# zenithfang/supervised_dispnet

Measured on AMD Instinct MI355X. Metric: images/sec fwd+bwd Disp_vgg_BN 128x416 b32 @1/2/4/8 GPU, higher is better.
Workload: dtype f32 (Winograd forward / input gradient / weight gradient form each f32 product from three exact bf16 pieces per operand on the bf16 matrix cores, six partial products, f32 accumulate; error vs fp64 at or below the f32 matrix instruction's)

## Files before the change

include/dispnet_hip.h:

```cpp
#ifndef DISPNET_HIP_H_
#define DISPNET_HIP_H_

#include <stddef.h>
#include <stdint.h>

#ifdef __cplusplus
extern "C" {
#endif

typedef void* dn_stream_t;

enum dn_status {
  DN_OK = 0,
  DN_ERR_BAD_ARG = -1,
  DN_ERR_UNSUPPORTED = -2,
  DN_ERR_WORKSPACE = -3,
  DN_ERR_LAUNCH = -4
};

void dn_reload_knobs(void);
int dn_version(void);
const char* dn_last_error(void);
const char* dn_last_kernel(void);
int dn_device_arch_ok(void);
// ... 49 lines not shown
  int32_t pad_mode;
  int32_t compute;
  int32_t dilation;
  const float* bnb_y;
  const float* bnb_scale;
  const float* bnb_shift;
  const float* bnb_mean;
  const float* bnb_invstd;
  float* bnb_partial;
  void* splitk_ws;
  int64_t splitk_ws_bytes;
  float* recip_out;
  const float* bnf_gamma;
  const float* bnf_beta;
  float* bnf_running_mean;
  float* bnf_running_var;
  int64_t* bnf_num_batches_tracked;
  float bnf_momentum, bnf_eps;
  float* bnf_mean;
  float* bnf_invstd;
  float* bnf_scale;
  float* bnf_shift;
  float* bnb_dgamma;
  float* bnb_dbeta;
} dn_conv_desc;

enum { DN_COMPUTE_DEFAULT = 0, DN_COMPUTE_BF16 = 1, DN_COMPUTE_F32X3 = 2, DN_COMPUTE_F32 = 3 };

int64_t dn_conv_packed_weight_elems(const dn_conv_desc* d);
int dn_conv_pack_weights(const dn_conv_desc* d, const float* w, float* w_packed, dn_stream_t stream);
int64_t dn_pack_entry_bytes(void);
int dn_pack_entry_fill(const dn_conv_desc* d, const float* w, float* w_packed, void* entry_host);
int dn_pack_many(const void* entries_dev, int32_t n_direct, int32_t n_wino, int32_t n_wino_bf16, int32_t n_wino_x3, dn_stream_t stream);
int32_t dn_conv_weight_layout(const dn_conv_desc* d);
int32_t dn_conv_bn_partial_rows(const dn_conv_desc* d);
int64_t dn_conv_splitk_workspace_bytes(const dn_conv_desc* d);
int32_t dn_conv_fwd_folds_bn_finalize(const dn_conv_desc* d);
int32_t dn_conv_dgrad_folds_bn_sums(const dn_conv_desc* d);
int32_t dn_conv_dgrad_fuses_bn_sums(const dn_conv_desc* d);
int32_t dn_conv_fwd_fuses_reciprocal(const dn_conv_desc* d);
int dn_conv2d_fwd(const dn_conv_desc* d, dn_stream_t stream);
int dn_conv2d_dgrad(const dn_conv_desc* d, dn_stream_t stream);
int dn_convT2d_fwd(const dn_conv_desc* d, dn_stream_t stream);
int dn_convT2d_dgrad(const dn_conv_desc* d, dn_stream_t stream);

size_t dn_conv_wgrad_workspace_bytes(const dn_conv_desc* fwd);
int dn_conv2d_wgrad(const dn_conv_desc* fwd, const float* dy, float* dw, void* workspace, size_t workspace_bytes,
                    dn_stream_t stream);

int dn_bn_finalize(const float* partial, int32_t rows, int32_t C, int64_t count, const float* conv_bias,
                   const float* gamma, const float* beta, float* running_mean, float* running_var, float momentum,
                   float eps, float* mean, float* invstd, float* scale, float* shift, int64_t* num_batches_tracked,
                   dn_stream_t stream);
int dn_bn_eval_affine(int32_t C, const float* gamma, const float* beta, const float* running_mean,
                      const float* running_var, float eps, float* scale, float* shift, dn_stream_t stream);
int dn_bn_relu_pool_fwd(const float* y, const float* scale, const float* shift, int32_t N, int32_t H, int32_t W,
                        int32_t C, float* pooled, uint8_t* idx, dn_stream_t stream);
int dn_bn_relu_pool_bwd(const float* dpooled, const uint8_t* idx, const float* y, const float* mean,
                        const float* invstd, int32_t N, int32_t H, int32_t W, int32_t C, float* dz, float* partial,
                        dn_stream_t stream);
int dn_maxpool2_bwd(const float* dpooled, const uint8_t* idx, int32_t N, int32_t H, int32_t W, int32_t C, float* dx, int32_t accumulate,
                    dn_stream_t stream);
int dn_bn_relu_bwd_reduce(float* da_dz, const float* y, const float* scale, const float* shift, const float* mean,
                          const float* invstd, int64_t rows, int32_t C, float* partial, dn_stream_t stream);
int dn_bn_bwd_apply(float* dz_dy, const float* y, const float* mean, const float* invstd, const float* gamma,
                    const float* partial, int32_t partial_rows, int32_t partial_stride, int32_t partial_offset, int64_t rows,
                    int32_t C, float* dgamma, float* dbeta, dn_stream_t stream);
int dn_bn_relu_bwd_sums(const float* da, const float* y, const float* scale, const float* shift, const float* mean, const float* invstd,
                        int64_t rows, int32_t C, float* partial, dn_stream_t stream);
int dn_bn_relu_pool_bwd_sums(const float* dpooled, const uint8_t* idx, const float* y, const float* mean, const float* invstd, int32_t N,
                             int32_t H, int32_t W, int32_t C, float* partial, dn_stream_t stream);
int dn_bn_bwd_apply_relu(float* da_dy, const float* y, const float* scale, const float* shift, const float* mean, const float* invstd,
                         const float* gamma, const float* partial, int32_t partial_rows, int32_t partial_stride, int32_t partial_offset,
                         int64_t rows, int32_t C, float* dgamma, float* dbeta, dn_stream_t stream);
int dn_bn_bwd_apply_pool(const float* dpooled, const uint8_t* idx, const float* y, const float* mean, const float* invstd, const float* gamma,
                         const float* partial, int32_t partial_rows, int32_t partial_stride, int32_t partial_offset, int32_t N, int32_t H,
                         int32_t W, int32_t C, float* dy, float* dgamma, float* dbeta, dn_stream_t stream);
int32_t dn_reduce_blocks(int64_t rows, int32_t C);

int dn_bn_frozen_affine(int32_t C, const float* gamma, const float* beta, const float* running_mean, const float* running_var, float eps,
                        float* scale, float* shift, float* invstd, dn_stream_t stream);
int dn_bn_frozen_bwd(float* dz_dy, const float* y, const float* mean, const float* invstd, const float* gamma, int64_t rows, int32_t C,
                     float* partial, dn_stream_t stream);
int dn_bn_frozen_bwd_relu(float* da_dy, const float* y, const float* scale, const float* shift, const float* mean, const float* invstd,
                          const float* gamma, int64_t rows, int32_t C, float* partial, dn_stream_t stream);
int dn_bn_frozen_bwd_pool(const float* dpooled, const uint8_t* idx, const float* y, const float* mean, const float* invstd, const float* gamma,
                          int32_t N, int32_t H, int32_t W, int32_t C, float* dy, float* partial, dn_stream_t stream);
int dn_bn_frozen_add_relu_bwd(const float* gout, const float* out, const float* y, const float* mean, const float* invstd, const float* gamma,
                              const float* r, const float* r_mean, const float* r_invstd, const float* r_gamma, int64_t rows, int32_t C,
                              float* dy, float* dr, int32_t dr_accumulate, float* partial, dn_stream_t stream);
int dn_bn_frozen_finalize(const float* partial, int32_t partial_rows, int32_t partial_stride, int32_t partial_offset, int32_t C,
                          const float* gamma, const float* invstd, float* dgamma, float* dbeta, float* dbias, dn_stream_t stream);

int dn_act_bwd_reduce_from(const float* g_in, float* g_out, const float* y_post, int32_t act, float p0, float p1, int64_t rows, int32_t C,
                           float* partial, dn_stream_t stream);
int dn_act_bwd_reduce(float* g, const float* y_post, int32_t act, float p0, float p1, int64_t rows, int32_t C,
                      float* partial, dn_stream_t stream);
int dn_colsum_finalize(const float* partial, int32_t rows, int32_t C, int32_t stride, int32_t offset, float* out,
                       dn_stream_t stream);
int dn_upsample2x_nearest_bwd(const float* dfull, int32_t N, int32_t h, int32_t w, float* dlow, int32_t accumulate,
                              dn_stream_t stream);
int dn_upsample2x_nearest_bwd_nhwc(const float* dfull, int32_t N, int32_t h, int32_t w, int32_t C, float* dlow, int32_t accumulate,
                                   dn_stream_t stream);
int dn_reflect_fold(const float* dxp, int32_t N, int32_t H, int32_t W, int32_t C, int32_t pad, float* dx, int32_t accumulate,
                    dn_stream_t stream);
int dn_bn_add_relu_fwd(const float* y, const float* scale, const float* shift, const float* r, const float* r_scale, const float* r_shift,
                       int64_t rows, int32_t C, float* out, dn_stream_t stream);
int dn_bn_add_relu_bwd(const float* gout, const float* out, const float* y, const float* mean, const float* invstd, const float* r,
                       const float* r_mean, const float* r_invstd, int64_t rows, int32_t C, float* dz_y, float* dr, int32_t dr_accumulate,
                       float* partial, dn_stream_t stream);
int32_t dn_maxpool3s2_out(int32_t H, int32_t ceil_mode);
int dn_maxpool3s2_fwd(const float* x, int32_t N, int32_t H, int32_t W, int32_t C, int32_t ceil_mode, float* out, uint8_t* idx, dn_stream_t stream);
int dn_maxpool3s2_bwd(const float* dout, const uint8_t* idx, int32_t N, int32_t H, int32_t W, int32_t C, int32_t ceil_mode, float* dx,
                      int32_t accumulate, dn_stream_t stream);
int dn_sub_div(const float* x, int64_t n, float sub, float div, float* out, dn_stream_t stream);
int dn_upsample2x_bilinear_fwd(const float* low, int32_t N, int32_t h, int32_t w, int32_t OH, int32_t OW, float* out,
                               dn_stream_t stream);
int dn_upsample2x_bilinear_bwd(const float* dout, int32_t N, int32_t h, int32_t w, int32_t OH, int32_t OW, float* dlow,
                               int32_t accumulate, dn_stream_t stream);
int32_t dn_bn_stats_rows(int64_t rows);
int dn_bn_stats_partial(const float* x, int64_t rows, int32_t C, float* partial, dn_stream_t stream);
int dn_bn_apply_fwd(const float* y, const float* scale, const float* shift, int64_t rows, int32_t C, float* out, dn_stream_t stream);
int dn_phase_bias_add(float* x, int32_t N, int32_t H2, int32_t W2, int32_t C, const float* bias4, dn_stream_t stream);
size_t dn_phase_colsum_workspace_bytes(int32_t C);
int dn_phase_colsum(const float* g, int32_t N, int32_t H, int32_t W, int32_t C, float* workspace, float* out4, dn_stream_t stream);
int dn_act_fwd(const float* x, int64_t n, int32_t act, float p0, float p1, float* out, dn_stream_t stream);
int dn_resize_bilinear_fwd(const float* in, int32_t N, int32_t IH, int32_t IW, int32_t OH, int32_t OW, int32_t align_corners, float* out,
                           dn_stream_t stream);
int dn_resize_bilinear_bwd(const float* dout, int32_t N, int32_t IH, int32_t IW, int32_t OH, int32_t OW, int32_t align_corners, float* din,
                           int32_t accumulate, dn_stream_t stream);
int dn_spatial_mean_fwd(const float* x, int32_t N, int64_t HW, int32_t C, float scale, float* out, dn_stream_t stream);
// ... 189 lines not shown
```

supervised_dispnet_amd/_lib.py:

```python
import ctypes as C
import os
import pathlib

_PKG = pathlib.Path(__file__).resolve().parent
LIB_PATH = pathlib.Path(os.environ.get("DISPNET_HIP_LIB", _PKG / "libdispnet_hip.so"))

EXPECTED_ABI = 23

DN_MAX_OPERANDS = 3
ACT_NONE, ACT_RELU, ACT_LEAKY, ACT_ELU, ACT_SIGMOID_AFFINE = 0, 1, 2, 3, 4
COMPUTE_DEFAULT, COMPUTE_BF16, COMPUTE_F32X3, COMPUTE_F32 = 0, 1, 2, 3
CONV_FWD, CONV_DGRAD, CONVT_FWD, CONVT_DGRAD = 0, 1, 2, 3
LOSS_L1, LOSS_L2, LOSS_BERHU, LOSS_SCALE_INV = 0, 1, 2, 3
LOSS_STATS = 8

_f32p = C.c_void_p


class Operand(C.Structure):
    _fields_ = [("data", _f32p), ("C", C.c_int32), ("up_shift", C.c_int32),
                ("stride_n", C.c_int64), ("stride_h", C.c_int64), ("stride_w", C.c_int64), ("stride_c", C.c_int64),
                ("scale", _f32p), ("shift", _f32p)]


class Result(C.Structure):
    _fields_ = [("data", _f32p), ("C", C.c_int32), ("accumulate", C.c_int32),
                ("stride_n", C.c_int64), ("stride_h", C.c_int64), ("stride_w", C.c_int64)]


class ConvDesc(C.Structure):
    _fields_ = [("kind", C.c_int32), ("N", C.c_int32), ("IH", C.c_int32), ("IW", C.c_int32), ("OH", C.c_int32),
                ("OW", C.c_int32), ("R", C.c_int32), ("S", C.c_int32), ("stride", C.c_int32), ("pad", C.c_int32),
                ("n_in", C.c_int32), ("in_", Operand * DN_MAX_OPERANDS),
                ("n_out", C.c_int32), ("out", Result * DN_MAX_OPERANDS),
                ("w_packed", _f32p), ("bias", _f32p), ("act", C.c_int32), ("act_p0", C.c_float), ("act_p1", C.c_float),
                ("bn_partial", _f32p), ("pad_mode", C.c_int32), ("compute", C.c_int32), ("dilation", C.c_int32),
                ("bnb_y", _f32p), ("bnb_scale", _f32p), ("bnb_shift", _f32p), ("bnb_mean", _f32p), ("bnb_invstd", _f32p), ("bnb_partial", _f32p),
                ("splitk_ws", _f32p), ("splitk_ws_bytes", C.c_int64), ("recip_out", _f32p),
                ("bnf_gamma", _f32p), ("bnf_beta", _f32p), ("bnf_running_mean", _f32p), ("bnf_running_var", _f32p),
                ("bnf_num_batches_tracked", C.c_void_p), ("bnf_momentum", C.c_float), ("bnf_eps", C.c_float),
                ("bnf_mean", _f32p), ("bnf_invstd", _f32p), ("bnf_scale", _f32p), ("bnf_shift", _f32p),
                ("bnb_dgamma", _f32p), ("bnb_dbeta", _f32p)]


_P = C.POINTER
_i32, _u32, _i64, _f, _d, _vp, _sz = C.c_int32, C.c_uint32, C.c_int64, C.c_float, C.c_double, C.c_void_p, C.c_size_t

SIGNATURES = {
    "dn_version": (C.c_int, []),
    "dn_reload_knobs": (None, []),
    "dn_last_error": (C.c_char_p, []),
    "dn_last_kernel": (C.c_char_p, []),
    "dn_device_arch_ok": (C.c_int, []),
    "dn_conv_packed_weight_elems": (_i64, [_P(ConvDesc)]),
    "dn_conv_pack_weights": (C.c_int, [_P(ConvDesc), _vp, _vp, _vp]),
    "dn_pack_entry_bytes": (_i64, []),
    "dn_pack_entry_fill": (C.c_int, [_P(ConvDesc), _vp, _vp, _vp]),
    "dn_pack_many": (C.c_int, [_vp, _i32, _i32, _i32, _i32, _vp]),
    "dn_conv_weight_layout": (_i32, [_P(ConvDesc)]),
    "dn_conv_bn_partial_rows": (_i32, [_P(ConvDesc)]),
    "dn_conv_dgrad_fuses_bn_sums": (_i32, [_P(ConvDesc)]),
    "dn_conv_fwd_fuses_reciprocal": (_i32, [_P(ConvDesc)]),
    "dn_conv_splitk_workspace_bytes": (_i64, [_P(ConvDesc)]),
    "dn_conv_fwd_folds_bn_finalize": (_i32, [_P(ConvDesc)]),
    "dn_conv_dgrad_folds_bn_sums": (_i32, [_P(ConvDesc)]),
    "dn_conv2d_fwd": (C.c_int, [_P(ConvDesc), _vp]),
    "dn_conv2d_dgrad": (C.c_int, [_P(ConvDesc), _vp]),
    "dn_convT2d_fwd": (C.c_int, [_P(ConvDesc), _vp]),
    "dn_convT2d_dgrad": (C.c_int, [_P(ConvDesc), _vp]),
    "dn_conv_wgrad_workspace_bytes": (_sz, [_P(ConvDesc)]),
    "dn_conv2d_wgrad": (C.c_int, [_P(ConvDesc), _vp, _vp, _vp, _sz, _vp]),
    "dn_bn_finalize": (C.c_int, [_vp, _i32, _i32, _i64, _vp, _vp, _vp, _vp, _vp, _f, _f, _vp, _vp, _vp, _vp, _vp, _vp]),
    "dn_bn_eval_affine": (C.c_int, [_i32, _vp, _vp, _vp, _vp, _f, _vp, _vp, _vp]),
    "dn_bn_relu_pool_fwd": (C.c_int, [_vp, _vp, _vp, _i32, _i32, _i32, _i32, _vp, _vp, _vp]),
    "dn_bn_relu_bwd_sums": (C.c_int, [_vp, _vp, _vp, _vp, _vp, _vp, _i64, _i32, _vp, _vp]),
    "dn_bn_relu_pool_bwd_sums": (C.c_int, [_vp, _vp, _vp, _vp, _vp, _i32, _i32, _i32, _i32, _vp, _vp]),
    "dn_bn_bwd_apply_relu": (C.c_int, [_vp, _vp, _vp, _vp, _vp, _vp, _vp, _vp, _i32, _i32, _i32, _i64, _i32, _vp, _vp, _vp]),
    "dn_bn_bwd_apply_pool": (C.c_int, [_vp, _vp, _vp, _vp, _vp, _vp, _vp, _i32, _i32, _i32, _i32, _i32, _i32, _i32, _vp, _vp, _vp, _vp]),
    "dn_maxpool2_bwd": (C.c_int, [_vp, _vp, _i32, _i32, _i32, _i32, _vp, _i32, _vp]),
    "dn_bn_relu_pool_bwd": (C.c_int, [_vp, _vp, _vp, _vp, _vp, _i32, _i32, _i32, _i32, _vp, _vp, _vp]),
    "dn_bn_relu_bwd_reduce": (C.c_int, [_vp, _vp, _vp, _vp, _vp, _vp, _i64, _i32, _vp, _vp]),
    "dn_bn_bwd_apply": (C.c_int, [_vp, _vp, _vp, _vp, _vp, _vp, _i32, _i32, _i32, _i64, _i32, _vp, _vp, _vp]),
    "dn_reduce_blocks": (_i32, [_i64, _i32]),
    "dn_bn_frozen_affine": (C.c_int, [_i32, _vp, _vp, _vp, _vp, _f, _vp, _vp, _vp, _vp]),
    "dn_bn_frozen_bwd": (C.c_int, [_vp, _vp, _vp, _vp, _vp, _i64, _i32, _vp, _vp]),
    "dn_bn_frozen_bwd_relu": (C.c_int, [_vp, _vp, _vp, _vp, _vp, _vp, _vp, _i64, _i32, _vp, _vp]),
    "dn_bn_frozen_bwd_pool": (C.c_int, [_vp, _vp, _vp, _vp, _vp, _vp, _i32, _i32, _i32, _i32, _vp, _vp, _vp]),
    "dn_bn_frozen_add_relu_bwd": (C.c_int, [_vp, _vp, _vp, _vp, _vp, _vp, _vp, _vp, _vp, _vp, _i64, _i32, _vp, _vp, _i32, _vp, _vp]),
    "dn_bn_frozen_finalize": (C.c_int, [_vp, _i32, _i32, _i32, _i32, _vp, _vp, _vp, _vp, _vp, _vp]),
    "dn_act_bwd_reduce": (C.c_int, [_vp, _vp, _i32, _f, _f, _i64, _i32, _vp, _vp]),
    "dn_act_bwd_reduce_from": (C.c_int, [_vp, _vp, _vp, _i32, _f, _f, _i64, _i32, _vp, _vp]),
    "dn_colsum_finalize": (C.c_int, [_vp, _i32, _i32, _i32, _i32, _vp, _vp]),
    "dn_upsample2x_nearest_bwd": (C.c_int, [_vp, _i32, _i32, _i32, _vp, _i32, _vp]),
    "dn_upsample2x_nearest_bwd_nhwc": (C.c_int, [_vp, _i32, _i32, _i32, _i32, _vp, _i32, _vp]),
    "dn_reflect_fold": (C.c_int, [_vp, _i32, _i32, _i32, _i32, _i32, _vp, _i32, _vp]),
    "dn_bn_add_relu_fwd": (C.c_int, [_vp, _vp, _vp, _vp, _vp, _vp, _i64, _i32, _vp, _vp]),
    "dn_bn_add_relu_bwd": (C.c_int, [_vp, _vp, _vp, _vp, _vp, _vp, _vp, _vp, _i64, _i32, _vp, _vp, _i32, _vp, _vp]),
    "dn_maxpool3s2_out": (_i32, [_i32, _i32]),
    "dn_maxpool3s2_fwd": (C.c_int, [_vp, _i32, _i32, _i32, _i32, _i32, _vp, _vp, _vp]),
    "dn_maxpool3s2_bwd": (C.c_int, [_vp, _vp, _i32, _i32, _i32, _i32, _i32, _vp, _i32, _vp]),
    "dn_bn_stats_rows": (_i32, [_i64]),
    "dn_bn_stats_partial": (C.c_int, [_vp, _i64, _i32, _vp, _vp]),
    "dn_bn_apply_fwd": (C.c_int, [_vp, _vp, _vp, _i64, _i32, _vp, _vp]),
    "dn_act_fwd": (C.c_int, [_vp, _i64, _i32, _f, _f, _vp, _vp]),
    "dn_phase_bias_add": (C.c_int, [_vp, _i32, _i32, _i32, _i32, _vp, _vp]),
    "dn_phase_colsum_workspace_bytes": (_sz, [_i32]),
    "dn_phase_colsum": (C.c_int, [_vp, _i32, _i32, _i32, _i32, _vp, _vp, _vp]),
    "dn_resize_bilinear_fwd": (C.c_int, [_vp, _i32, _i32, _i32, _i32, _i32, _i32, _vp, _vp]),
    "dn_resize_bilinear_bwd": (C.c_int, [_vp, _i32, _i32, _i32, _i32, _i32, _i32, _vp, _i32, _vp]),
    "dn_sub_div": (C.c_int, [_vp, _i64, _f, _f, _vp, _vp]),
    "dn_spatial_mean_fwd": (C.c_int, [_vp, _i32, _i64, _i32, _f, _vp, _vp]),
    "dn_spatial_mean_bwd": (C.c_int, [_vp, _i32, _i64, _i32, _f, _vp, _vp]),
    "dn_upsample2x_bilinear_fwd": (C.c_int, [_vp, _i32, _i32, _i32, _i32, _i32, _vp, _vp]),
    "dn_upsample2x_bilinear_bwd": (C.c_int, [_vp, _i32, _i32, _i32, _i32, _i32, _vp, _i32, _vp]),
    "dn_reciprocal_fwd": (C.c_int, [_vp, _vp, _i64, _vp]),
    "dn_reciprocal_bwd": (C.c_int, [_vp, _vp, _vp, _i64, _vp]),
    "dn_masked_loss_workspace_bytes": (_sz, [_i32, _i64]),
    "dn_masked_loss_fwd": (C.c_int, [_vp, _vp, _i32, _i64, _f, _i32, _f, _i32, _vp, _vp, _sz, _vp, _vp]),
    "dn_masked_loss_fwd_fused": (C.c_int, [_vp, _vp, _i32, _i64, _f, _i32, _f, _i32, _vp, _vp, _sz, _vp, _vp, _vp]),
    "dn_masked_loss_stats": (C.c_int, [_vp, _vp, _i32, _i64, _f, _i32, _i32, _vp, _vp, _sz, _vp]),
    "dn_masked_loss_finalize": (C.c_int, [_vp, _i32, _i32, _f, _i32, _vp, _vp]),
    "dn_masked_loss_bwd": (C.c_int, [_vp, _vp, _vp, _vp, _i32, _i64, _f, _i32, _f, _vp, _vp]),
    "dn_pyramid_down2": (C.c_int, [_vp, _i32, _i32, _i32, _i32, _vp, _vp]),
    "dn_upsample_int_fwd": (C.c_int, [_vp, _i32, _i32, _i32, _i32, _i32, _vp, _vp]),
    "dn_upsample_int_bwd": (C.c_int, [_vp, _i32, _i32, _i32, _i32, _i32, _vp, _vp]),
# ... 149 lines not shown
```

supervised_dispnet_amd/csrc/dn_bn.hip:

```cpp
#include "dn_colreduce.h"
#include "dn_fold.h"

namespace dn {

constexpr int kBnTileRows = 128;
__global__ void __launch_bounds__(kThreads) bn_finalize_kernel(const float* __restrict__ partial, int rows, int C, double count,
                                                               const float* __restrict__ conv_bias, const float* __restrict__ gamma,
                                                               const float* __restrict__ beta, float* running_mean, float* running_var,
                                                               float momentum, float eps, float* mean_out, float* invstd_out, float* scale,
                                                               float* shift, long long* num_batches_tracked) {
  const int c = blockIdx.x;
  if (num_batches_tracked != nullptr && c == 0 && threadIdx.x == 0) num_batches_tracked[0] += 1;
  __shared__ double red[3][4];
  double s1 = 0.0, q = 0.0, pp = 0.0;
  const double n0 = count < (double)kBnTileRows ? count : (double)kBnTileRows;
  const double pivot = (double)partial[(long long)c * 2] / n0;
#pragma unroll 8
  for (int r = threadIdx.x; r < rows; r += kThreads) {
    const float2 v = *reinterpret_cast<const float2*>(partial + ((long long)r * C + c) * 2);
    const double left = count - (double)r * kBnTileRows;
    const double nt = left < (double)kBnTileRows ? left : (double)kBnTileRows;
    const double dm = (double)v.x / nt - pivot;
    s1 += (double)v.x;
    q += (double)v.y;
    pp += nt * dm * dm;
  }
#pragma unroll
  for (int o = 32; o > 0; o >>= 1) {
    s1 += __shfl_xor(s1, o);
    q += __shfl_xor(q, o);
    pp += __shfl_xor(pp, o);
  }
  if ((threadIdx.x & 63) == 0) {
    red[0][threadIdx.x >> 6] = s1;
    red[1][threadIdx.x >> 6] = q;
    red[2][threadIdx.x >> 6] = pp;
  }
  __syncthreads();
  double macc = 0.0, m2tot = 0.0;
  if (threadIdx.x == 0) {
    const double S = (red[0][0] + red[0][1]) + (red[0][2] + red[0][3]);
    const double Q = (red[1][0] + red[1][1]) + (red[1][2] + red[1][3]);
    const double P = (red[2][0] + red[2][1]) + (red[2][2] + red[2][3]);
    macc = S / count;
    m2tot = Q + (P - count * (macc - pivot) * (macc - pivot));
  }
  if (threadIdx.x == 0) {
    double var = m2tot / count;
    if (var < 0.0) var = 0.0;
    const float mean = (float)(macc + (conv_bias ? (double)conv_bias[c] : 0.0));
    const float invstd = (float)(1.0 / sqrt(var + (double)eps));
    const float sc = gamma[c] * invstd;
    mean_out[c] = mean;
    invstd_out[c] = invstd;
    scale[c] = sc;
    shift[c] = beta[c] - mean * sc;
    if (running_mean) {
      const double unbiased = count > 1.0 ? var * count / (count - 1.0) : var;
      running_mean[c] = (1.f - momentum) * running_mean[c] + momentum * mean;
      running_var[c] = (1.f - momentum) * running_var[c] + momentum * (float)unbiased;
    }
  }
}

__global__ void __launch_bounds__(256) bn_finalize_sliced_kernel(const float* __restrict__ partial, int rows, int C, double count, BnFinalizeArgs a) {
  __shared__ double red[3 * kFoldSlices * 64];
  const int c0 = blockIdx.x * 64;
  bn_finalize_sliced<false>(partial, rows, C, c0, C - c0 < 64 ? C - c0 : 64, count, a, red, threadIdx.x);
}

__global__ void __launch_bounds__(256) colsum2_sliced_kernel(const float* __restrict__ partial, int rows, int C, int stride, int offset,
                                                             float* __restrict__ out0, float* __restrict__ out1) {
  __shared__ double red[2 * kFoldSlices * 64];
  const int c0 = blockIdx.x * 64;
  colsum2_sliced<false>(partial, rows, C, stride, offset, c0, C - c0 < 64 ? C - c0 : 64, out0, out1, red, threadIdx.x);
}

__global__ void bn_eval_affine_kernel(int C, const float* gamma, const float* beta, const float* rm, const float* rv, float eps,
                                      float* scale, float* shift, float* invstd_out) {
  int c = blockIdx.x * blockDim.x + threadIdx.x;
  if (c < C) {
    float invstd = 1.f / sqrtf(rv[c] + eps);
    float sc = gamma[c] * invstd;
    scale[c] = sc;
    shift[c] = beta[c] - rm[c] * sc;
    if (invstd_out != nullptr) invstd_out[c] = invstd;
  }
}

__global__ void __launch_bounds__(kThreads) bn_stats_partial_kernel(const float* __restrict__ x, long long rows, int C, float* __restrict__ partial) {
  __shared__ float red[4][64];
  __shared__ float mean_s[64];
  const int c = blockIdx.y * 64 + (threadIdx.x & 63), q = threadIdx.x >> 6;
  const long long r0 = (long long)blockIdx.x * kBnTileRows;
  const long long left = rows - r0;
  const int n = left < kBnTileRows ? (int)left : kBnTileRows;
  float s = 0.f;
  if (c < C)
    for (int r = q; r < n; r += 4) s += x[(r0 + r) * C + c];
  red[q][threadIdx.x & 63] = s;
  __syncthreads();
  float tot = 0.f;
  if (q == 0) {
    tot = red[0][threadIdx.x] + red[1][threadIdx.x] + red[2][threadIdx.x] + red[3][threadIdx.x];
    mean_s[threadIdx.x] = tot / (float)n;
  }
  __syncthreads();
  const float mu = mean_s[threadIdx.x & 63];
  float m2 = 0.f;
  if (c < C)
    for (int r = q; r < n; r += 4) {
      const float d = x[(r0 + r) * C + c] - mu;
      m2 += d * d;
    }
  __syncthreads();
  red[q][threadIdx.x & 63] = m2;
  __syncthreads();
  if (q == 0 && c < C) {
    float* dst = partial + ((long long)blockIdx.x * C + c) * 2;
    dst[0] = tot;
    dst[1] = red[0][threadIdx.x] + red[1][threadIdx.x] + red[2][threadIdx.x] + red[3][threadIdx.x];
  }
}

__global__ void __launch_bounds__(kThreads) bn_apply_kernel(const float* __restrict__ y, const float* __restrict__ scale, const float* __restrict__ shift,
                                                            long long rows, int C, float* __restrict__ out) {
  const int G = C / 4;
  const long long total = rows * G;
// ... 443 lines not shown
  float* dr;
  int dr_accumulate;
  int C;
  template <int V>
  __device__ __forceinline__ void apply(long long row, int c0, float (&acc)[V][4]) const {
    const long long o = row * C + c0;
    const Vec<V> g = ldv<V>(gout + o), ov = ldv<V>(out + o), yv = ldv_stream<V>(y + o);
    const Vec<V> mu = ldv<V>(mean + c0), is = ldv<V>(invstd + c0), ga = ldv<V>(gamma + c0);
    Vec<V> m, d;
#pragma unroll
    for (int e = 0; e < V; ++e) {
      m.v[e] = ov.v[e] > 0.f ? g.v[e] : 0.f;
      float term;
      d.v[e] = bn_frozen_bwd_value(m.v[e], yv.v[e], mu.v[e], is.v[e], ga.v[e], term);
      acc[e][0] += m.v[e];
      acc[e][1] += term;
    }
    stv<V>(dy + o, d);
    if (r_mean != nullptr) {
      const Vec<V> rv = ldv_stream<V>(r + o), rm = ldv<V>(r_mean + c0), ri = ldv<V>(r_invstd + c0), rg = ldv<V>(r_gamma + c0);
#pragma unroll
      for (int e = 0; e < V; ++e) {
        float term;
        d.v[e] = bn_frozen_bwd_value(m.v[e], rv.v[e], rm.v[e], ri.v[e], rg.v[e], term);
        acc[e][2] += m.v[e];
        acc[e][3] += term;
      }
      stv<V>(dr + o, d);
    } else if (dr != nullptr) {
      if (dr_accumulate) {
        Vec<V> a = ldv<V>(dr + o);
#pragma unroll
        for (int e = 0; e < V; ++e) a.v[e] += m.v[e];
        stv<V>(dr + o, a);
      } else {
        stv<V>(dr + o, m);
      }
    }
  }
};

__device__ __forceinline__ float bn_frozen_dbias(float ga, float is, float db) {
#pragma clang fp contract(off)
  return (ga * is) * db;
}

__global__ void __launch_bounds__(256) bn_frozen_finalize_sliced_kernel(const float* __restrict__ partial, int rows, int C, int stride, int offset,
                                                                        const float* __restrict__ gamma, const float* __restrict__ invstd,
                                                                        float* __restrict__ dgamma, float* __restrict__ dbeta,
                                                                        float* __restrict__ dbias) {
  __shared__ double red[2 * kFoldSlices * 64];
  const int c0 = blockIdx.x * 64;
  const int nlive = C - c0 < 64 ? C - c0 : 64;
  colsum2_sliced<false>(partial, rows, C, stride, offset, c0, nlive, dbeta, dgamma, red, threadIdx.x);
  const int cl = threadIdx.x & 63;
  if (dbias != nullptr && (threadIdx.x >> 6) == 0 && cl < nlive) dbias[c0 + cl] = bn_frozen_dbias(gamma[c0 + cl], invstd[c0 + cl], dbeta[c0 + cl]);
}

__global__ void __launch_bounds__(256) bn_frozen_finalize_kernel(const float* __restrict__ partial, int rows, int C, int stride, int offset,
                                                                 const float* __restrict__ gamma, const float* __restrict__ invstd,
                                                                 float* __restrict__ dgamma, float* __restrict__ dbeta, float* __restrict__ dbias) {
  const int c = blockIdx.x;
  double s0 = 0.0, s1 = 0.0;
#pragma unroll 4
  for (int r = threadIdx.x; r < rows; r += 256) {
    const float* q = partial + ((long long)r * C + c) * stride + offset;
    s0 += (double)q[0];
    s1 += (double)q[1];
  }
#pragma unroll
  for (int o = 32; o > 0; o >>= 1) {
    s0 += __shfl_xor(s0, o);
    s1 += __shfl_xor(s1, o);
  }
  __shared__ double red[2][4];
  if ((threadIdx.x & 63) == 0) {
    red[0][threadIdx.x >> 6] = s0;
    red[1][threadIdx.x >> 6] = s1;
  }
  __syncthreads();
  if (threadIdx.x == 0) {
    const float db = (float)((red[0][0] + red[0][1]) + (red[0][2] + red[0][3]));
    dbeta[c] = db;
    dgamma[c] = (float)((red[1][0] + red[1][1]) + (red[1][2] + red[1][3]));
    if (dbias != nullptr) dbias[c] = bn_frozen_dbias(gamma[c], invstd[c], db);
  }
}

template <bool RELU>
static int launch_bn_bwd_apply(float* g_dy, const float* y, const float* scale, const float* shift, const float* mean, const float* invstd,
                               const float* gamma, const float* dgamma, const float* dbeta, int64_t rows, int32_t C, hipStream_t s,
                               const char* what) {
  const int G = C / 4;
  int blocks = ew_blocks((rows * (long long)G + 3) / 4);
  int ga = G, gb = kThreads;
  while (gb != 0) {
    const int t = ga % gb;
    ga = gb;
    gb = t;
  }
  const int per = G / ga;
  if (per <= 64) {
    blocks = (blocks + per - 1) / per * per;
    set_last_kernel(RELU ? "dn::bn_bwd_apply_hoisted_kernel<true>" : "dn::bn_bwd_apply_hoisted_kernel<false>");
    DN_LAUNCH(bn_bwd_apply_hoisted_kernel<RELU>, dim3(blocks), dim3(kThreads), 0, s, g_dy, y, scale, shift, mean, invstd, gamma, dgamma, dbeta,
              (long long)rows, C, (float)(1.0 / (double)rows));
  } else {
    set_last_kernel(RELU ? "dn::bn_bwd_apply_kernel<true>" : "dn::bn_bwd_apply_kernel<false>");
    DN_LAUNCH(bn_bwd_apply_kernel<RELU>, dim3(ew_blocks(rows * (C / 4))), dim3(kThreads), 0, s, g_dy, y, scale, shift, mean, invstd, gamma, dgamma,
              dbeta, (long long)rows, C, (float)(1.0 / (double)rows));
  }
  return check_launch(what);
}

}

using namespace dn;

extern "C" {

int dn_bn_finalize(const float* partial, int32_t rows, int32_t C, int64_t count, const float* conv_bias, const float* gamma,
                   const float* beta, float* running_mean, float* running_var, float momentum, float eps, float* mean, float* invstd,
                   float* scale, float* shift, int64_t* num_batches_tracked, dn_stream_t stream) {
  DN_REQUIRE(partial && gamma && beta && mean && invstd && scale && shift && rows > 0 && C > 0 && count > 0, DN_ERR_BAD_ARG,
             "dn_bn_finalize: bad argument");
  if (rows <= kFoldMaxRows) {
    const BnFinalizeArgs a{conv_bias, gamma, beta, running_mean, running_var, reinterpret_cast<long long*>(num_batches_tracked), momentum, eps,
                           mean, invstd, scale, shift};
    DN_LAUNCH(bn_finalize_sliced_kernel, dim3((C + 63) / 64), dim3(256), 0, as_stream(stream), partial, rows, C, (double)count, a);
    return check_launch("bn_finalize_sliced_kernel");
  }
  DN_LAUNCH(bn_finalize_kernel, dim3(C), dim3(kThreads), 0, as_stream(stream), partial, rows, C, (double)count, conv_bias, gamma,
                     beta, running_mean, running_var, momentum, eps, mean, invstd, scale, shift,
                     reinterpret_cast<long long*>(num_batches_tracked));
  return check_launch("bn_finalize_kernel");
}

int dn_bn_eval_affine(int32_t C, const float* gamma, const float* beta, const float* running_mean, const float* running_var, float eps,
                      float* scale, float* shift, dn_stream_t stream) {
  DN_REQUIRE(C > 0 && gamma && beta && running_mean && running_var && scale && shift, DN_ERR_BAD_ARG, "dn_bn_eval_affine: bad argument");
  DN_LAUNCH(bn_eval_affine_kernel, dim3((C + 255) / 256), dim3(256), 0, as_stream(stream), C, gamma, beta, running_mean,
                     running_var, eps, scale, shift, (float*)nullptr);
  return check_launch("bn_eval_affine_kernel");
}

int dn_bn_frozen_affine(int32_t C, const float* gamma, const float* beta, const float* running_mean, const float* running_var, float eps,
                        float* scale, float* shift, float* invstd, dn_stream_t stream) {
  DN_REQUIRE(C > 0 && gamma && beta && running_mean && running_var && scale && shift && invstd, DN_ERR_BAD_ARG,
             "dn_bn_frozen_affine: bad argument");
  DN_LAUNCH(bn_eval_affine_kernel, dim3((C + 255) / 256), dim3(256), 0, as_stream(stream), C, gamma, beta, running_mean,
                     running_var, eps, scale, shift, invstd);
  return check_launch("bn_eval_affine_kernel");
}

int dn_bn_frozen_bwd(float* dz_dy, const float* y, const float* mean, const float* invstd, const float* gamma, int64_t rows, int32_t C,
                     float* partial, dn_stream_t stream) {
  DN_REQUIRE(dz_dy && y && mean && invstd && gamma && partial && rows > 0 && C > 0, DN_ERR_BAD_ARG, "dn_bn_frozen_bwd: bad argument");
  DN_REQUIRE(C % 4 == 0, DN_ERR_UNSUPPORTED, "dn_bn_frozen_bwd: need C%%4==0");
  BnFrozenBwdOp<false> op{dz_dy, y, nullptr, nullptr, mean, invstd, gamma, C};
  return launch_colreduce(op, rows, C, partial, as_stream(stream), "bn_frozen_bwd");
}

int dn_bn_frozen_bwd_relu(float* da_dy, const float* y, const float* scale, const float* shift, const float* mean, const float* invstd,
                          const float* gamma, int64_t rows, int32_t C, float* partial, dn_stream_t stream) {
  DN_REQUIRE(da_dy && y && scale && shift && mean && invstd && gamma && partial && rows > 0 && C > 0, DN_ERR_BAD_ARG,
             "dn_bn_frozen_bwd_relu: bad argument");
  DN_REQUIRE(C % 4 == 0, DN_ERR_UNSUPPORTED, "dn_bn_frozen_bwd_relu: need C%%4==0");
  BnFrozenBwdOp<true> op{da_dy, y, scale, shift, mean, invstd, gamma, C};
  return launch_colreduce(op, rows, C, partial, as_stream(stream), "bn_frozen_bwd_relu");
}

int dn_bn_frozen_bwd_pool(const float* dpooled, const uint8_t* idx, const float* y, const float* mean, const float* invstd, const float* gamma,
                          int32_t N, int32_t H, int32_t W, int32_t C, float* dy, float* partial, dn_stream_t stream) {
  DN_REQUIRE(dpooled && idx && y && mean && invstd && gamma && dy && partial && N > 0 && H > 0 && W > 0 && C > 0, DN_ERR_BAD_ARG,
             "dn_bn_frozen_bwd_pool: bad argument");
  DN_REQUIRE(C % 4 == 0 && H % 2 == 0 && W % 2 == 0, DN_ERR_UNSUPPORTED, "dn_bn_frozen_bwd_pool: need C%%4==0 and even H,W");
  BnFrozenPoolBwdOp op{dpooled, idx, y, mean, invstd, gamma, dy, H / 2, W / 2, H, W, C};
  return launch_colreduce(op, (long long)N * (H / 2) * (W / 2), C, partial, as_stream(stream), "bn_frozen_bwd_pool");
}

int dn_bn_frozen_add_relu_bwd(const float* gout, const float* out, const float* y, const float* mean, const float* invstd, const float* gamma,
                              const float* r, const float* r_mean, const float* r_invstd, const float* r_gamma, int64_t rows, int32_t C,
                              float* dy, float* dr, int32_t dr_accumulate, float* partial, dn_stream_t stream) {
  DN_REQUIRE(gout && out && y && mean && invstd && gamma && dy && partial && rows > 0 && C > 0, DN_ERR_BAD_ARG,
             "dn_bn_frozen_add_relu_bwd: bad argument");
  DN_REQUIRE(C % 4 == 0, DN_ERR_UNSUPPORTED, "dn_bn_frozen_add_relu_bwd: need C%%4==0");
  DN_REQUIRE((r_mean == nullptr) == (r_invstd == nullptr) && (r_mean == nullptr) == (r_gamma == nullptr), DN_ERR_BAD_ARG,
             "dn_bn_frozen_add_relu_bwd: r_mean / r_invstd / r_gamma go together");
// ... 11 lines not shown
  hipStream_t s = as_stream(stream);
  if (partial_rows <= kFoldMaxRows && (partial_stride & 1) == 0 && (partial_offset & 1) == 0 && (reinterpret_cast<uintptr_t>(partial) & 7) == 0)
    DN_LAUNCH(bn_frozen_finalize_sliced_kernel, dim3((C + 63) / 64), dim3(256), 0, s, partial, partial_rows, C, partial_stride, partial_offset, gamma,
              invstd, dgamma, dbeta, dbias);
  else
    DN_LAUNCH(bn_frozen_finalize_kernel, dim3(C), dim3(256), 0, s, partial, partial_rows, C, partial_stride, partial_offset, gamma, invstd, dgamma,
              dbeta, dbias);
  return check_launch("bn_frozen_finalize");
}

int32_t dn_bn_stats_rows(int64_t rows) { return (int32_t)((rows + kBnTileRows - 1) / kBnTileRows); }

int dn_bn_stats_partial(const float* x, int64_t rows, int32_t C, float* partial, dn_stream_t stream) {
  DN_REQUIRE(x && partial && rows > 0 && C > 0, DN_ERR_BAD_ARG, "dn_bn_stats_partial: bad argument");
  DN_REQUIRE((rows + kBnTileRows - 1) / kBnTileRows < 65536ll * 32768ll, DN_ERR_UNSUPPORTED, "dn_bn_stats_partial: too many rows");
  DN_LAUNCH(bn_stats_partial_kernel, dim3((unsigned)((rows + kBnTileRows - 1) / kBnTileRows), (C + 63) / 64), dim3(kThreads), 0, as_stream(stream), x,
                     (long long)rows, C, partial);
  return check_launch("bn_stats_partial_kernel");
}

int dn_bn_apply_fwd(const float* y, const float* scale, const float* shift, int64_t rows, int32_t C, float* out, dn_stream_t stream) {
  DN_REQUIRE(y && scale && shift && out && rows > 0 && C > 0, DN_ERR_BAD_ARG, "dn_bn_apply_fwd: bad argument");
  DN_REQUIRE(C % 4 == 0, DN_ERR_UNSUPPORTED, "dn_bn_apply_fwd: need C%%4==0");
  DN_LAUNCH(bn_apply_kernel, dim3(ew_blocks(rows * (C / 4))), dim3(kThreads), 0, as_stream(stream), y, scale, shift, (long long)rows, C, out);
  return check_launch("bn_apply_kernel");
}

int dn_bn_relu_pool_fwd(const float* y, const float* scale, const float* shift, int32_t N, int32_t H, int32_t W, int32_t C, float* pooled,
                        uint8_t* idx, dn_stream_t stream) {
  DN_REQUIRE(y && pooled && idx && ((scale == nullptr) == (shift == nullptr)), DN_ERR_BAD_ARG, "dn_bn_relu_pool_fwd: null pointer");
  DN_REQUIRE(C % 4 == 0 && H % 2 == 0 && W % 2 == 0 && N > 0, DN_ERR_UNSUPPORTED, "dn_bn_relu_pool_fwd: need C%%4==0 and even H,W");
  const long long total = (long long)N * (H / 2) * (W / 2) * (C / 4);
  DN_LAUNCH(bn_relu_pool_fwd_kernel, dim3(ew_blocks(total)), dim3(kThreads), 0, as_stream(stream), y, scale, shift, N, H, W, C,
                     pooled, idx);
  return check_launch("bn_relu_pool_fwd_kernel");
}

int dn_bn_relu_pool_bwd(const float* dpooled, const uint8_t* idx, const float* y, const float* mean, const float* invstd, int32_t N,
                        int32_t H, int32_t W, int32_t C, float* dz, float* partial, dn_stream_t stream) {
  DN_REQUIRE(dpooled && idx && y && mean && invstd && dz && partial, DN_ERR_BAD_ARG, "dn_bn_relu_pool_bwd: null pointer");
  DN_REQUIRE(C % 4 == 0 && H % 2 == 0 && W % 2 == 0, DN_ERR_UNSUPPORTED, "dn_bn_relu_pool_bwd: need C%%4==0 and even H,W");
  PoolBwdOp op{dpooled, idx, y, mean, invstd, dz, H / 2, W / 2, H, W, C};
  return launch_colreduce(op, (long long)N * (H / 2) * (W / 2), C, partial, as_stream(stream), "bn_relu_pool_bwd");
}

int dn_bn_relu_pool_bwd_sums(const float* dpooled, const uint8_t* idx, const float* y, const float* mean, const float* invstd, int32_t N,
                             int32_t H, int32_t W, int32_t C, float* partial, dn_stream_t stream) {
  DN_REQUIRE(dpooled && idx && y && mean && invstd && partial, DN_ERR_BAD_ARG, "dn_bn_relu_pool_bwd_sums: null pointer");
  DN_REQUIRE(C % 4 == 0 && H % 2 == 0 && W % 2 == 0, DN_ERR_UNSUPPORTED, "dn_bn_relu_pool_bwd_sums: need C%%4==0 and even H,W");
  PoolBwdOp op{dpooled, idx, y, mean, invstd, nullptr, H / 2, W / 2, H, W, C};
  return launch_colreduce(op, (long long)N * (H / 2) * (W / 2), C, partial, as_stream(stream), "bn_relu_pool_bwd_sums");
}

int dn_bn_relu_bwd_reduce(float* da_dz, const float* y, const float* scale, const float* shift, const float* mean, const float* invstd,
                          int64_t rows, int32_t C, float* partial, dn_stream_t stream) {
  DN_REQUIRE(da_dz && y && scale && shift && mean && invstd && partial && rows > 0 && C > 0, DN_ERR_BAD_ARG,
             "dn_bn_relu_bwd_reduce: bad argument");
  BnReluBwdOp op{1, da_dz, y, scale, shift, mean, invstd, C};
  return launch_colreduce(op, rows, C, partial, as_stream(stream), "bn_relu_bwd_reduce");
}

int dn_bn_relu_bwd_sums(const float* da, const float* y, const float* scale, const float* shift, const float* mean, const float* invstd,
                        int64_t rows, int32_t C, float* partial, dn_stream_t stream) {
  DN_REQUIRE(da && y && scale && shift && mean && invstd && partial && rows > 0 && C > 0, DN_ERR_BAD_ARG, "dn_bn_relu_bwd_sums: bad argument");
  BnReluBwdOp op{0, const_cast<float*>(da), y, scale, shift, mean, invstd, C};
  return launch_colreduce(op, rows, C, partial, as_stream(stream), "bn_relu_bwd_sums");
}

static void launch_colsum2(const float* partial, int32_t partial_rows, int32_t C, int32_t partial_stride, int32_t partial_offset, float* out0,
                           float* out1, hipStream_t s) {
  if (partial_rows <= kFoldMaxRows && (partial_stride & 1) == 0 && (partial_offset & 1) == 0 && (reinterpret_cast<uintptr_t>(partial) & 7) == 0)
    DN_LAUNCH(colsum2_sliced_kernel, dim3((C + 63) / 64), dim3(256), 0, s, partial, partial_rows, C, partial_stride, partial_offset, out0, out1);
  else
    DN_LAUNCH(colsum2_finalize_kernel, dim3(C), dim3(256), 0, s, partial, partial_rows, C, partial_stride, partial_offset, out0, out1);
}

static int bn_bwd_sums_to_params(const float* partial, int32_t partial_rows, int32_t partial_stride, int32_t partial_offset, int32_t C,
                                 float* dgamma, float* dbeta, hipStream_t s, const char* who) {
  DN_REQUIRE(dgamma && dbeta, DN_ERR_BAD_ARG, "%s: bad argument", who);
  DN_REQUIRE(C % 4 == 0, DN_ERR_UNSUPPORTED, "%s: need C%%4==0", who);
  if (partial == nullptr) return DN_OK;
  DN_REQUIRE(partial_rows > 0, DN_ERR_BAD_ARG, "%s: bad argument", who);
  DN_REQUIRE(partial_stride >= 2 && partial_offset >= 0 && partial_offset + 1 < partial_stride, DN_ERR_BAD_ARG, "%s: partial layout", who);
  launch_colsum2(partial, partial_rows, C, partial_stride, partial_offset, dbeta, dgamma, s);
  return DN_OK;
}

int dn_bn_bwd_apply_relu(float* da_dy, const float* y, const float* scale, const float* shift, const float* mean, const float* invstd,
                         const float* gamma, const float* partial, int32_t partial_rows, int32_t partial_stride, int32_t partial_offset,
                         int64_t rows, int32_t C, float* dgamma, float* dbeta, dn_stream_t stream) {
  DN_REQUIRE(da_dy && y && scale && shift && mean && invstd && gamma && rows > 0, DN_ERR_BAD_ARG, "dn_bn_bwd_apply_relu: bad argument");
  hipStream_t s = as_stream(stream);
  int rc = bn_bwd_sums_to_params(partial, partial_rows, partial_stride, partial_offset, C, dgamma, dbeta, s, "dn_bn_bwd_apply_relu");
  if (rc != DN_OK) return rc;
  return launch_bn_bwd_apply<true>(da_dy, y, scale, shift, mean, invstd, gamma, dgamma, dbeta, rows, C, s, "bn_bwd_apply_relu");
}

int dn_bn_bwd_apply_pool(const float* dpooled, const uint8_t* idx, const float* y, const float* mean, const float* invstd, const float* gamma,
                         const float* partial, int32_t partial_rows, int32_t partial_stride, int32_t partial_offset, int32_t N, int32_t H,
                         int32_t W, int32_t C, float* dy, float* dgamma, float* dbeta, dn_stream_t stream) {
  DN_REQUIRE(dpooled && idx && y && mean && invstd && gamma && dy && N > 0, DN_ERR_BAD_ARG, "dn_bn_bwd_apply_pool: bad argument");
  DN_REQUIRE(H % 2 == 0 && W % 2 == 0, DN_ERR_UNSUPPORTED, "dn_bn_bwd_apply_pool: need even H, W");
  hipStream_t s = as_stream(stream);
  int rc = bn_bwd_sums_to_params(partial, partial_rows, partial_stride, partial_offset, C, dgamma, dbeta, s, "dn_bn_bwd_apply_pool");
  if (rc != DN_OK) return rc;
  const long long total = (long long)N * (H / 2) * (W / 2) * (C / 4);
  DN_LAUNCH(bn_bwd_apply_pool_kernel, dim3(ew_blocks(total)), dim3(kThreads), 0, s, dpooled, idx, y, mean, invstd, gamma, dgamma, dbeta, N,
                     H, W, C, (float)(1.0 / ((double)N * H * W)), dy);
  return check_launch("bn_bwd_apply_pool");
}

int dn_bn_bwd_apply(float* dz_dy, const float* y, const float* mean, const float* invstd, const float* gamma, const float* partial,
                    int32_t partial_rows, int32_t partial_stride, int32_t partial_offset, int64_t rows, int32_t C, float* dgamma,
                    float* dbeta, dn_stream_t stream) {
  DN_REQUIRE(dz_dy && y && mean && invstd && gamma && partial && dgamma && dbeta && rows > 0, DN_ERR_BAD_ARG, "dn_bn_bwd_apply: bad argument");
  DN_REQUIRE(C % 4 == 0, DN_ERR_UNSUPPORTED, "dn_bn_bwd_apply: need C%%4==0");
  DN_REQUIRE(partial_stride >= 2 && partial_offset >= 0 && partial_offset + 1 < partial_stride, DN_ERR_BAD_ARG, "dn_bn_bwd_apply: partial layout");
  hipStream_t s = as_stream(stream);
  launch_colsum2(partial, partial_rows, C, partial_stride, partial_offset, dbeta, dgamma, s);
  return launch_bn_bwd_apply<false>(dz_dy, y, nullptr, nullptr, mean, invstd, gamma, dgamma, dbeta, rows, C, s, "bn_bwd_apply");
}

int dn_bn_add_relu_fwd(const float* y, const float* scale, const float* shift, const float* r, const float* r_scale, const float* r_shift,
                       int64_t rows, int32_t C, float* out, dn_stream_t stream) {
  DN_REQUIRE(y && scale && shift && out && rows > 0 && C > 0 && ((r_scale == nullptr) == (r_shift == nullptr)) && (r || !r_scale),
             DN_ERR_BAD_ARG, "dn_bn_add_relu_fwd: bad argument");
  DN_REQUIRE(C % 4 == 0, DN_ERR_UNSUPPORTED, "dn_bn_add_relu_fwd: need C%%4==0");
  DN_LAUNCH(bn_add_relu_fwd_kernel, dim3(ew_blocks(rows * (C / 4))), dim3(kThreads), 0, as_stream(stream), y, scale, shift, r, r_scale,
                     r_shift, (long long)rows, C, out);
  return check_launch("bn_add_relu_fwd_kernel");
}

int dn_bn_add_relu_bwd(const float* gout, const float* out, const float* y, const float* mean, const float* invstd, const float* r,
                       const float* r_mean, const float* r_invstd, int64_t rows, int32_t C, float* dz_y, float* dr, int32_t dr_accumulate,
                       float* partial, dn_stream_t stream) {
  DN_REQUIRE(gout && out && y && mean && invstd && dz_y && partial && rows > 0 && C > 0, DN_ERR_BAD_ARG, "dn_bn_add_relu_bwd: bad argument");
  DN_REQUIRE((r_mean == nullptr) == (r_invstd == nullptr), DN_ERR_BAD_ARG, "dn_bn_add_relu_bwd: r_mean / r_invstd go together");
  DN_REQUIRE(r_mean == nullptr || (r && dr), DN_ERR_BAD_ARG, "dn_bn_add_relu_bwd: the downsample branch needs r and dr");
  AddReluBwdOp op{gout, out, y, mean, invstd, r, r_mean, r_invstd, dz_y, dr, dr_accumulate, C};
  return launch_colreduce(op, rows, C, partial, as_stream(stream), "bn_add_relu_bwd");
}

}
```

supervised_dispnet_amd/csrc/dn_colreduce.h:

```cpp
#pragma once
#include "dn_device.h"

namespace dn {

constexpr int kThreads = 256;
constexpr int kMaxReduceBlocks = 4096;

static inline int ew_blocks(long long n_items) {
  long long b = (n_items + kThreads - 1) / kThreads;
  if (b > 4096) b = 4096;
  if (b < 1) b = 1;
  return (int)b;
}

static inline int reduce_blocks(long long rows, int C) {
  int V = (C % 4 == 0) ? 4 : 1;
  int groups = C / V;
  int tpr = 1;
  while (tpr < groups && tpr < kThreads) tpr <<= 1;
  int rpi = kThreads / tpr;
  const int rpt = 2;
  long long b = (rows + (long long)rpi * rpt - 1) / ((long long)rpi * rpt);
  const int cap = 1024 < kMaxReduceBlocks ? 1024 : kMaxReduceBlocks;
  if (b > cap) b = cap;
  if (b < 1) b = 1;
  return (int)b;
}

template <class Op, int V>
__global__ void __launch_bounds__(kThreads) colreduce_kernel(Op op, long long rows, int C, float* __restrict__ partial) {
  constexpr int NACC = Op::NACC;
  const int groups = C / V;
  int tpr = 1;
  while (tpr < groups && tpr < kThreads) tpr <<= 1;
  const int rpi = kThreads / tpr;
  const int rl = threadIdx.x / tpr, gi = threadIdx.x % tpr;
  const long long per = (rows + gridDim.x - 1) / gridDim.x;
  const long long rbeg = blockIdx.x * per;
  const long long rend = (rbeg + per < rows) ? rbeg + per : rows;
  __shared__ float red[kThreads * V * NACC];
  for (int g0 = 0; g0 < groups; g0 += tpr) {
    const int grp = g0 + gi;
    float acc[V][NACC];
#pragma unroll
    for (int v = 0; v < V; ++v)
#pragma unroll
      for (int a = 0; a < NACC; ++a) acc[v][a] = 0.f;
    if (grp < groups)
      for (long long r = rbeg + rl; r < rend; r += rpi) op.template apply<V>(r, grp * V, acc);
#pragma unroll
    for (int v = 0; v < V; ++v)
#pragma unroll
      for (int a = 0; a < NACC; ++a) red[(threadIdx.x * V + v) * NACC + a] = acc[v][a];
    __syncthreads();
    if (rl == 0 && grp < groups) {
#pragma unroll
      for (int v = 0; v < V; ++v)
#pragma unroll
        for (int a = 0; a < NACC; ++a) {
          float s = 0.f;
          for (int q = 0; q < rpi; ++q) s += red[((q * tpr + gi) * V + v) * NACC + a];
          partial[((long long)blockIdx.x * C + grp * V + v) * NACC + a] = s;
        }
    }
    __syncthreads();
  }
}

template <class Op>
static int launch_colreduce(const Op& op, long long rows, int C, float* partial, hipStream_t s, const char* what) {
  const int blocks = reduce_blocks(rows, C);
  if (C % 4 == 0)
    DN_LAUNCH((colreduce_kernel<Op, 4>), dim3(blocks), dim3(kThreads), 0, s, op, rows, C, partial);
  else
    DN_LAUNCH((colreduce_kernel<Op, 1>), dim3(blocks), dim3(kThreads), 0, s, op, rows, C, partial);
  return check_launch(what);
}

template <int V>
struct Vec {
  float v[V];
};
template <int V>
__device__ __forceinline__ Vec<V> ldv(const float* p) {
  Vec<V> r;
  if constexpr (V == 4) {
    f32x4 t = *reinterpret_cast<const f32x4*>(p);
#pragma unroll
    for (int i = 0; i < 4; ++i) r.v[i] = t[i];
  } else {
#pragma unroll
    for (int i = 0; i < V; ++i) r.v[i] = p[i];
  }
  return r;
}
template <int V>
__device__ __forceinline__ void stv(float* p, const Vec<V>& r) {
  if constexpr (V == 4) {
    *reinterpret_cast<f32x4*>(p) = f32x4{r.v[0], r.v[1], r.v[2], r.v[3]};
  } else {
#pragma unroll
    for (int i = 0; i < V; ++i) p[i] = r.v[i];
  }
}

}
```

supervised_dispnet_amd/csrc/dn_conv.hip:

```cpp
#include <stdlib.h>

#include "dn_internal.h"

namespace dn {

template <auto Launch> static int plan_only(const dn_conv_desc*, IgemmParams& p, hipStream_t s) { return Launch(p, s); }
template <auto Launch> static int with_desc(const dn_conv_desc* d, IgemmParams& p, hipStream_t s) { return Launch(d, p, s); }
static bool heads_off() { return knobs().no_direct; }
constexpr auto x3_upper = conv_x3_splitk_workspace_upper_bytes;
static const ConvFamily kConvFamilies[] = {
    {"head_fwd", head_fwd_eligible, heads_off, plan_only<launch_head_fwd>, nullptr, x3_upper, head_fwd_fuses_reciprocal},
    {"head_dgrad", head_dgrad_eligible, heads_off, plan_only<launch_head_dgrad>, nullptr, x3_upper},
    {"winograd", wino_eligible, nullptr, plan_only<launch_wino_conv>, wino_layout,
     [](const IgemmParams& p) { return wino_layout(p) == 3 ? wino_splitk_workspace_bytes(p) : (size_t)0; }, nullptr,
     [](const dn_conv_desc* d) {
       const dn_result& r = d->out[0];
       return d->kind == DN_CONV_DGRAD && d->n_out == 1 && !r.accumulate && (r.C & 3) == 0 && r.stride_w == r.C &&
              r.stride_h == (int64_t)d->OW * r.C && r.stride_n == (int64_t)d->OH * d->OW * r.C && d->bias == nullptr && d->act == DN_ACT_NONE;
     },
     [](IgemmParams& p) { wino_prepare(p); return wino_folds_bn_finalize(p); }, [](IgemmParams& p) { wino_prepare(p); return wino_folds_bn_sums(p); }},
    {"stem3", stem3_conv_eligible, nullptr, plan_only<launch_stem3_conv>, nullptr, x3_upper},
    {"stemk", stemk_conv_eligible, nullptr, with_desc<launch_stemk_conv>, nullptr, x3_upper},
    {"stem", stem_eligible, nullptr, plan_only<launch_stem>, nullptr, x3_upper},
    {"lds3", lds3_conv_eligible, nullptr, with_desc<launch_lds3_conv>, nullptr, x3_upper},
    {"lds3k", lds3k_conv_eligible, nullptr, with_desc<launch_lds3k_conv>, nullptr, x3_upper},
    {"thin", thin_conv_eligible, nullptr, plan_only<launch_thin_conv>, nullptr, x3_upper},
    {"tiled", [](const dn_conv_desc*, const IgemmParams&) { return true; }, nullptr, plan_only<launch_tiled_conv>, nullptr, x3_upper},
};

const ConvFamily* conv_route(const dn_conv_desc* d, const IgemmParams& p) {
  const ConvFamily* f = kConvFamilies;
  while (!f->eligible(d, p) || (f->switched_off && f->switched_off())) ++f;
  return f;
}

static int run_conv(const dn_conv_desc* d, int expect_kind, dn_stream_t stream) {
  DN_REQUIRE(d != nullptr && d->kind == expect_kind, DN_ERR_BAD_ARG, "descriptor kind mismatch (want %d)", expect_kind);
  IgemmParams p;
  int rc = build_plan(d, false, &p);
  if (rc != DN_OK) return rc;
  DN_REQUIRE(p.w != nullptr, DN_ERR_BAD_ARG, "w_packed is null");
  for (int i = 0; i < p.n_in; ++i) DN_REQUIRE(p.in[i].p != nullptr, DN_ERR_BAD_ARG, "operand %d has no data", i);
  for (int i = 0; i < p.n_out; ++i) {
    const dn_result& o = d->out[i];
    DN_REQUIRE(o.stride_h == (int64_t)d->OW * o.stride_w && o.stride_n == (int64_t)d->OH * o.stride_h, DN_ERR_UNSUPPORTED,
               "result %d must be pixel-dense (NHWC with a channel stride)", i);
  }
  return conv_route(d, p)->launch(d, p, as_stream(stream));
}

}

using namespace dn;

static bool wgrad_split_plans(const dn_conv_desc* fwd, dn_conv_desc* d1, dn_conv_desc* d2, IgemmParams* p1, IgemmParams* p2, size_t* w1,
                              size_t* w2) {
  if (fwd->kind != DN_CONV_FWD || fwd->n_in < 2 || fwd->in[fwd->n_in - 1].C != 1) return false;
  *d1 = *fwd;
  d1->n_in = fwd->n_in - 1;
  *d2 = *fwd;
  d2->n_in = 1;
  d2->in[0] = fwd->in[fwd->n_in - 1];
  if (build_plan(d1, true, p1) != DN_OK || build_plan(d2, true, p2) != DN_OK) return false;
  int cin_total = 0;
  for (int i = 0; i < fwd->n_in; ++i) cin_total += fwd->in[i].C;
  if (wino_wgrad_eligible(d1, *p1)) {
    p1->dw_cin_total = cin_total;
    *w1 = (wino_wgrad_workspace_bytes(*p1) + 255) / 256 * 256;
  } else {
    return false;
  }
  p2->in[0].ch_off = cin_total - 1;
  p2->D1 = cin_total;
  choose_splits(p2);
// ... 185 lines not shown
```

supervised_dispnet_amd/csrc/dn_fold.h:

```cpp
#pragma once
#if defined(__HIP_DEVICE_COMPILE__) && !defined(__gfx950__)
#error "dn_fold.h relies on gfx950 behaviour (write-through sc1 stores + s_waitcnt vmcnt(0), relaxed agent-scope atomics served by the L2): probe before porting (dn_last_arrival_probe)"
#endif
#include "dn_internal.h"

namespace dn {

constexpr int kFoldMaxRows = 128;
constexpr int kFoldSlices = 4;
constexpr int kFoldCounters = 64;

__device__ __forceinline__ void fold_store(float* p, float v) { __hip_atomic_store(p, v, __ATOMIC_RELAXED, __HIP_MEMORY_SCOPE_AGENT); }

template <bool AGENT>
__device__ __forceinline__ float2 fold_load2(const float* p) {
  float2 r;
  if constexpr (AGENT) {
    const unsigned long long u = __hip_atomic_load(reinterpret_cast<const unsigned long long*>(p), __ATOMIC_RELAXED, __HIP_MEMORY_SCOPE_AGENT);
    r.x = __builtin_bit_cast(float, (unsigned)(u & 0xffffffffull));
    r.y = __builtin_bit_cast(float, (unsigned)(u >> 32));
  } else {
    r = *reinterpret_cast<const float2*>(p);
  }
  return r;
}

__device__ __forceinline__ bool fold_last_arrival(int* counter, int expected, int* flag) {
  asm volatile("s_waitcnt vmcnt(0)" ::: "memory");
  __syncthreads();
  if (threadIdx.x == 0) {
    const int prev = __hip_atomic_fetch_add(counter, 1, __ATOMIC_RELAXED, __HIP_MEMORY_SCOPE_AGENT);
    *flag = (prev == expected - 1) ? 1 : 0;
    if (prev == expected - 1) __hip_atomic_store(counter, 0, __ATOMIC_RELAXED, __HIP_MEMORY_SCOPE_AGENT);
  }
  __syncthreads();
  return *flag != 0;
}

template <bool AGENT>
__device__ __forceinline__ void bn_finalize_sliced(const float* partial, int rows, int C, int c0, int nlive, double count, const BnFinalizeArgs& a,
                                                   double* red, int tid) {
  constexpr double kTile = 128.0;
  const int cl = tid & 63, sl = tid >> 6;
  const int c = c0 + cl;
  const bool live = tid < 64 * kFoldSlices && cl < nlive;
  double pivot = 0.0;
  if (live) {
    double s1 = 0.0, q = 0.0, pp = 0.0;
    const double n0 = count < kTile ? count : kTile;
    pivot = (double)fold_load2<AGENT>(partial + (long long)c * 2).x / n0;
#pragma unroll 8
    for (int r = sl; r < rows; r += kFoldSlices) {
      const float2 v = fold_load2<AGENT>(partial + ((long long)r * C + c) * 2);
      const double left = count - (double)r * kTile;
      const double nt = left < kTile ? left : kTile;
      const double dm = (double)v.x / nt - pivot;
      s1 += (double)v.x;
      q += (double)v.y;
      pp += nt * dm * dm;
    }
    red[(0 * kFoldSlices + sl) * 64 + cl] = s1;
    red[(1 * kFoldSlices + sl) * 64 + cl] = q;
    red[(2 * kFoldSlices + sl) * 64 + cl] = pp;
  }
  __syncthreads();
  if (live && sl == 0) {
    double t[3];
#pragma unroll
    for (int k = 0; k < 3; ++k)
      t[k] = ((red[(k * kFoldSlices + 0) * 64 + cl] + red[(k * kFoldSlices + 1) * 64 + cl]) + red[(k * kFoldSlices + 2) * 64 + cl]) +
             red[(k * kFoldSlices + 3) * 64 + cl];
    const double macc = t[0] / count;
    const double m2tot = t[1] + (t[2] - count * (macc - pivot) * (macc - pivot));
    double var = m2tot / count;
    if (var < 0.0) var = 0.0;
    const float mean = (float)(macc + (a.conv_bias ? (double)a.conv_bias[c] : 0.0));
    const float invstd = (float)(1.0 / sqrt(var + (double)a.eps));
    const float sc = a.gamma[c] * invstd;
    a.mean[c] = mean;
    a.invstd[c] = invstd;
    a.scale[c] = sc;
    a.shift[c] = a.beta[c] - mean * sc;
    if (a.running_mean) {
      const double unbiased = count > 1.0 ? var * count / (count - 1.0) : var;
      a.running_mean[c] = (1.f - a.momentum) * a.running_mean[c] + a.momentum * mean;
      a.running_var[c] = (1.f - a.momentum) * a.running_var[c] + a.momentum * (float)unbiased;
    }
  }
  if (tid == 0 && c0 == 0 && a.num_batches_tracked != nullptr) a.num_batches_tracked[0] += 1;
}

template <bool AGENT>
__device__ __forceinline__ void colsum2_sliced(const float* partial, int rows, int C, int stride, int offset, int c0, int nlive, float* out0,
                                               float* out1, double* red, int tid) {
  const int cl = tid & 63, sl = tid >> 6;
  const int c = c0 + cl;
  const bool live = tid < 64 * kFoldSlices && cl < nlive;
  if (live) {
    double s0 = 0.0, s1 = 0.0;
#pragma unroll 8
    for (int r = sl; r < rows; r += kFoldSlices) {
      const float2 v = fold_load2<AGENT>(partial + ((long long)r * C + c) * stride + offset);
      s0 += (double)v.x;
      s1 += (double)v.y;
    }
    red[(0 * kFoldSlices + sl) * 64 + cl] = s0;
    red[(1 * kFoldSlices + sl) * 64 + cl] = s1;
  }
  __syncthreads();
  if (live && sl == 0) {
    out0[c] = (float)(((red[(0 * kFoldSlices + 0) * 64 + cl] + red[(0 * kFoldSlices + 1) * 64 + cl]) + red[(0 * kFoldSlices + 2) * 64 + cl]) +
                      red[(0 * kFoldSlices + 3) * 64 + cl]);
    out1[c] = (float)(((red[(1 * kFoldSlices + 0) * 64 + cl] + red[(1 * kFoldSlices + 1) * 64 + cl]) + red[(1 * kFoldSlices + 2) * 64 + cl]) +
                      red[(1 * kFoldSlices + 3) * 64 + cl]);
  }
}

}
```

supervised_dispnet_amd/csrc/dn_internal.h:

```cpp
#pragma once
#include <hip/hip_runtime.h>
#include <hip/hip_ext.h>
#include <stdint.h>
#include <stdio.h>

#include <atomic>
#include <functional>
#include <tuple>
#include <type_traits>

#include "dispnet_hip.h"

namespace dn {

void set_error(const char* fmt, ...);
void set_last_kernel(const char* fmt, ...);
int check_launch(const char* what);

static inline hipStream_t as_stream(dn_stream_t s) { return reinterpret_cast<hipStream_t>(s); }

struct LaunchTape;
extern std::atomic<LaunchTape*> g_tape_rec;
void tape_push(LaunchTape* t, std::function<void(hipEvent_t)>&& op, const void* kernel, hipStream_t stream);

// ... 33 lines not shown
  int wino_splitk_target, wino_splitk_maxblocks;
  int pack_blocks;
  bool no_riding_fences;
  int wino_nmajor;
  int wino_wg_target;
  int wino8;
};
const Knobs& knobs();

inline int norm_compute(int c) {
  return c == DN_COMPUTE_BF16 ? DN_COMPUTE_BF16 : ((c == DN_COMPUTE_F32X3 || c == DN_COMPUTE_DEFAULT) ? DN_COMPUTE_F32X3 : DN_COMPUTE_F32);
}

#define DN_REQUIRE(cond, code, ...)      \
  do {                                   \
    if (!(cond)) {                       \
      ::dn::set_error(__VA_ARGS__);      \
      return (code);                     \
    }                                    \
  } while (0)

constexpr int kMaxTaps = 64;
constexpr int kMaxPhases = 4;
constexpr int kChunk = 32;

struct KOperand {
  const float* p;
  const float* scale;
  const float* shift;
  long long sn, sh, sw, sc;
  int C;
  int up;
  int vec;
  int ch_off;
  unsigned mC;
  int small;
};

struct KResult {
  float* p;
  long long sn, sh, sw;
  int C;
  int n_begin;
  int accumulate;
  int linear;
};

struct KPhase {
  int ntaps;
  int tap0;
  int ooy, oox;
  int nchunks;
  long long w_off;
};

struct BnFinalizeArgs {
  const float* conv_bias;
  const float* gamma;
  const float* beta;
  float* running_mean;
  float* running_var;
  long long* num_batches_tracked;
  float momentum, eps;
  float* mean;
  float* invstd;
  float* scale;
  float* shift;
};

struct IgemmParams {
  KOperand in[DN_MAX_OPERANDS];
  KResult out[DN_MAX_OPERANDS];
  KPhase ph[kMaxPhases];
  int8_t tdy[kMaxTaps], tdx[kMaxTaps], tr[kMaxTaps], ts[kMaxTaps];
  int n_in, n_out, nphases;
  int N, GH, GW, M;
  int sy, sx;
  int osy, osx;
  int IH, IW, OH, OW;
  int Ntot, Npad;
  int BN;
  int R, S;
  int n_is_dim0;
  int D0, D1;
  const float* w;
  const float* bias;
  float* bn_partial;
  int act;
  float act_p0, act_p1;
  const float* g;
  float* ws;
  int splits, m_per_split;
  unsigned mGW, mGH;
  int allvec;
  int uni32;
  int wg_uniform;
  int any_affine;
  int reflect;
  int compute;
  int tile_store;
  const float *bnb_y, *bnb_scale, *bnb_shift, *bnb_mean, *bnb_invstd;
  float* bnb_partial;
  int ksplit, ks_chunks, ks_cnt_floats;
  int dw_cin_total;
  int ks_reg, ks_tail;
  float* recip_out;
  float* ks_ws;
  size_t ks_ws_bytes;
  int T, TH, TW;
  unsigned mTW, mTH;
  BnFinalizeArgs bnf;
  float *bnb_dgamma, *bnb_dbeta;
  int* fold_cnt;
  int fold_bn, fold_bnb;
  int nmajor;
};

static inline unsigned fastdiv_magic(unsigned d) { return d <= 1 ? 0xFFFFFFFFu : (unsigned)(0x100000000ull / d); }

int build_plan(const dn_conv_desc* d, bool for_wgrad, IgemmParams* p);

inline long long direct_packed_elems(const IgemmParams& p) {
  const KPhase& last = p.ph[p.nphases - 1];
  return last.w_off + (long long)p.Npad * last.nchunks * kChunk;
}

struct PackEntry {
  IgemmParams p;
  const float* w;
  float* wp;
  long long total;
  int wino;
  int NS;
};
int launch_wino_pack_many(const PackEntry* tab_dev, int first, int n, hipStream_t stream);
int launch_wino_pack16_many(const PackEntry* tab_dev, int first, int n, int pieces, hipStream_t stream);
int launch_wino_pack16(const IgemmParams& p, const float* w, float* wp, int pieces, hipStream_t stream);
long long wino_packed_floats(const IgemmParams& p, int layout);
int wino_layout(const IgemmParams& p);

struct ConvFamily {
  const char* name;
  bool (*eligible)(const dn_conv_desc* d, const IgemmParams& p);
  bool (*switched_off)();
  int (*launch)(const dn_conv_desc* d, IgemmParams& p, hipStream_t s);
  int (*weight_layout)(const IgemmParams& p);
  size_t (*splitk_workspace_bytes)(const IgemmParams& p);
  bool (*fuses_reciprocal)(const IgemmParams& p);
  bool (*takes_bn_sums)(const dn_conv_desc* d);
  bool (*folds_bn_finalize)(IgemmParams& p);
  bool (*folds_bn_sums)(IgemmParams& p);
};
const ConvFamily* conv_route(const dn_conv_desc* d, const IgemmParams& p);

bool stem_eligible(const dn_conv_desc* d, const IgemmParams& p);
int launch_stem(const IgemmParams& p, hipStream_t stream);
int launch_tiled_conv(const IgemmParams& p, hipStream_t stream);
void choose_splits(IgemmParams* p);
size_t generic_wgrad_workspace_bytes(const IgemmParams& p);
int generic_wgrad(const dn_conv_desc* fwd, IgemmParams& p, const float* dy, float* dw, void* workspace, size_t workspace_bytes, hipStream_t s);
int launch_direct_pack(const IgemmParams& p, const float* w, float* wp, hipStream_t stream);
int launch_direct_pack_many(const PackEntry* tab_dev, int n, hipStream_t stream);

bool head_fwd_eligible(const dn_conv_desc* d, const IgemmParams& p);
int launch_head_fwd(const IgemmParams& p, hipStream_t stream);
bool head_fwd_fuses_reciprocal(const IgemmParams& p);
bool head_dgrad_eligible(const dn_conv_desc* d, const IgemmParams& p);
int launch_head_dgrad(const IgemmParams& p, hipStream_t stream);
bool head_wgrad_eligible(const dn_conv_desc* fwd, const IgemmParams& p);
size_t head_wgrad_workspace_bytes(const IgemmParams& p);
int launch_head_wgrad(const IgemmParams& p, float* dw, float* workspace, hipStream_t stream);

bool wino_eligible(const dn_conv_desc* d, const IgemmParams& p);
long long wino_packed_elems(const IgemmParams& p);
int launch_wino_pack(const IgemmParams& p, const float* w, float* wp, hipStream_t stream);
int launch_wino_conv(IgemmParams& p, hipStream_t stream);
void wino_prepare(IgemmParams& p);
bool wino_folds_bn_finalize(const IgemmParams& p);
bool wino_folds_bn_sums(const IgemmParams& p);
int wino_splitk_choice(const IgemmParams& p);
size_t conv_x3_splitk_workspace_upper_bytes(const IgemmParams& p);
size_t wino_splitk_workspace_bytes(const IgemmParams& p);
bool wino_wgrad_eligible(const dn_conv_desc* fwd, const IgemmParams& p);
size_t wino_wgrad_workspace_bytes(const IgemmParams& p);
int launch_wino_wgrad(IgemmParams& p, float* dw, hipStream_t stream);

bool thin_wgrad_eligible(const dn_conv_desc* fwd, const IgemmParams& p);
size_t thin_wgrad_workspace_bytes(const IgemmParams& p);
int launch_thin_wgrad(IgemmParams& p, float* dw, hipStream_t stream);
bool thin_conv_eligible(const dn_conv_desc* d, const IgemmParams& p);
int launch_thin_conv(const IgemmParams& p, hipStream_t stream);

bool lds3_conv_eligible(const dn_conv_desc* d, const IgemmParams& p);
int launch_lds3_conv(const dn_conv_desc* d, const IgemmParams& p, hipStream_t stream);
bool lds3_wgrad_eligible(const dn_conv_desc* fwd, const IgemmParams& p);
size_t lds3_wgrad_workspace_bytes(const IgemmParams& p);
int launch_lds3_wgrad(const dn_conv_desc* fwd, IgemmParams& p, float* dw, hipStream_t stream);
bool lds3k_wgrad_eligible(const dn_conv_desc* fwd, const IgemmParams& p);
size_t lds3k_wgrad_workspace_bytes(const IgemmParams& p);
int launch_lds3k_wgrad(const dn_conv_desc* fwd, IgemmParams& p, float* dw, hipStream_t stream);
int launch_wgrad_reduce(const IgemmParams& p, float* dw, hipStream_t stream);
bool wgrad_x3_eligible(const IgemmParams& p);
int launch_wgrad_x3(const IgemmParams& p, hipStream_t stream);
bool lds3k_conv_eligible(const dn_conv_desc* d, const IgemmParams& p);
int launch_lds3k_conv(const dn_conv_desc* d, const IgemmParams& p, hipStream_t stream);
bool stem3_conv_eligible(const dn_conv_desc* d, const IgemmParams& p);
bool stemk_conv_eligible(const dn_conv_desc* d, const IgemmParams& p);
int launch_stemk_conv(const dn_conv_desc* d, const IgemmParams& p, hipStream_t stream);
bool stemk_wgrad_eligible(const dn_conv_desc* d, const IgemmParams& p);
size_t stemk_wgrad_workspace_bytes(const dn_conv_desc* d, const IgemmParams& p);
int launch_stemk_wgrad(const dn_conv_desc* d, IgemmParams& p, float* dw, hipStream_t stream);
int launch_stem3_conv(const IgemmParams& p, hipStream_t stream);

}
```

supervised_dispnet_amd/csrc/dn_lds3.hip:

```cpp
#include <stdlib.h>

#include "dn_device.h"

namespace dn {

struct Lds3Geo {
  int tilesX, tilesY, ntiles;
  int dy0, dx0;
  int per_xcd;
};

template <int CG, int NKS, bool HAS1, int ROLES, int STRIDE, int TH, int TW, int ROWS, int COLS>
struct Lds3Cfg {
  static constexpr int HALFC = (COLS + 1) / 2;
  static constexpr int COLSP = STRIDE == 2 ? 2 * HALFC : COLS;
  static constexpr int PLANE = ROWS * COLSP * 16;
  static constexpr int CGSTRIDE = ((PLANE + 255) / 256) * 256 + 256 / CG;
  static constexpr int PSTRIDE = CG * CGSTRIDE;
  static constexpr int DPLANE = HAS1 ? ROWS * COLS * 4 : 0;
  static constexpr size_t LDS = (size_t)3 * PSTRIDE + DPLANE;
  static constexpr int PTB = TH * TW / 16;
  static constexpr int WAVES_PER_ROLE = 4 / ROLES;
  static constexpr int PT_PER_WAVE = PTB / WAVES_PER_ROLE;
  static_assert(TW % 16 == 0 && PT_PER_WAVE % 2 == 0, "pixel tiles are processed in pairs");
};

template <int CG, int NKS, bool HAS1, int ROLES, int STRIDE, int TH, int TW, int ROWS, int COLS, int PIPE>
__global__ void __launch_bounds__(256, 2) lds3_conv_kernel(const IgemmParams p, const Lds3Geo geo) {
  using Cfg = Lds3Cfg<CG, NKS, HAS1, ROLES, STRIDE, TH, TW, ROWS, COLS>;
  constexpr int C = 8 * CG;
  extern __shared__ __align__(16) char lds[];
  const int tid = threadIdx.x, lane = tid & 63, wave = tid >> 6;
  const int j = lane & 15, g = lane >> 4;
  const int role = ROLES == 1 ? 0 : (ROLES == 2 ? (wave >> 1) : wave);
  const int sub = ROLES == 1 ? wave : (ROLES == 2 ? (wave & 1) : 0);
  const int z = ROLES == 4 ? role : 0;
  const int mt = ROLES == 2 ? role : 0;
  const KPhase ph = p.ph[z];
  const int ntaps = ph.ntaps, Kp = ph.nchunks * kChunk;
  const int nslots = ntaps * CG;
  const int kbase1 = ((ntaps * C + kChunk - 1) / kChunk) * kChunk;

  bf16x8 wa[NKS][3];
  int boff[NKS];
  {
    const int n = 16 * mt + j;
    const float* wrow = p.w + ph.w_off + (long long)n * Kp;
#pragma unroll
    for (int ks = 0; ks < NKS; ++ks) {
      const int s = 4 * ks + g;
      float v[8];
#pragma unroll
      for (int e = 0; e < 8; ++e) v[e] = 0.f;
      int off = 0;
      if (s < nslots) {
// ... 341 lines not shown
        for (int u = 0; u < 2; ++u)
#pragma unroll
          for (int m = 0; m < 4; ++m) acc[u][m] = __builtin_amdgcn_mfma_f32_16x16x32_bf16(wa[m][AS[q]], b[u][BS[q]], acc[u][m], 0, 0, 0);
      if (p.bn_partial != nullptr) {
        if (i == 0) {
#pragma unroll
          for (int m = 0; m < 4; ++m)
#pragma unroll
            for (int e = 0; e < 4; ++e) {
              pv[m][e] = __shfl(acc[0][m][e], lane & 48);
              sv[m][e] = 0.f;
              qv[m][e] = 0.f;
            }
        }
#pragma unroll
        for (int u = 0; u < 2; ++u)
#pragma unroll
          for (int m = 0; m < 4; ++m)
#pragma unroll
            for (int e = 0; e < 4; ++e) {
              const float dlt = acc[u][m][e] - pv[m][e];
              sv[m][e] += dlt;
              qv[m][e] = fmaf(dlt, dlt, qv[m][e]);
            }
      }
#pragma unroll
      for (int u = 0; u < 2; ++u) {
        const int pt = i + u;
        const int gy = gy0 + 2 * wave + (pt >> 1), gx = gx0 + (pt & 1) * 16 + j;
        float* o = R.p + (long long)n * R.sn + (long long)gy * R.sh + (long long)gx * R.sw + 4 * g;
#pragma unroll
        for (int m = 0; m < 4; ++m) {
          f32x4 w4;
#pragma unroll
          for (int e = 0; e < 4; ++e) w4[e] = apply_act(acc[u][m][e] + bias[m][e], p.act, p.act_p0, p.act_p1);
          *reinterpret_cast<f32x4*>(o + 16 * m) = w4;
        }
      }
    }
    if (p.bn_partial != nullptr) {
#pragma unroll
      for (int m = 0; m < 4; ++m)
#pragma unroll
        for (int e = 0; e < 4; ++e) {
          const float s1 = row16_sum(sv[m][e]), q1 = row16_sum(qv[m][e]);
          if (j == 0) *reinterpret_cast<f32x2*>(&wstat[wave][16 * m + 4 * g + e][0]) = f32x2{fmaf(64.f, pv[m][e], s1), q1 - s1 * s1 * (1.f / 64.f)};
        }
    }
    __syncthreads();
    if (p.bn_partial != nullptr && tid < 128) {
      const int h = tid >> 6, c = tid & 63;
      const f32x2 a = *reinterpret_cast<const f32x2*>(&wstat[2 * h][c][0]), b2 = *reinterpret_cast<const f32x2*>(&wstat[2 * h + 1][c][0]);
      const float dm = (b2[0] - a[0]) * (1.f / 64.f);
      *reinterpret_cast<f32x2*>(p.bn_partial + ((long long)(2 * t + h) * p.Ntot + c) * 2) = f32x2{a[0] + b2[0], a[1] + b2[1] + dm * dm * 32.f};
    }
  }
}

static bool stem3_eligible(const dn_conv_desc* d, const IgemmParams& p) {
  if (knobs().no_lds3 || p.compute != DN_COMPUTE_F32X3) return false;
  if (d->kind != DN_CONV_FWD || d->R != 3 || d->S != 3 || d->stride != 1 || d->pad != 1 || d->pad_mode != 0 || d->dilation > 1) return false;
  if (p.n_in != 1 || p.n_out != 1 || p.Ntot != 64 || p.nphases != 1) return false;
  const KOperand& o = p.in[0];
  const KResult& r = p.out[0];
  if (!(o.C >= 1 && o.C <= 3 && o.up == 0 && o.scale == nullptr && o.small)) return false;
  if (!(r.linear && !r.accumulate && (r.sw & 3) == 0 && (reinterpret_cast<uintptr_t>(r.p) & 15) == 0)) return false;
  return p.GH % STEM_TH == 0 && p.GW % STEM_TW == 0;
}

bool stem3_conv_eligible(const dn_conv_desc* d, const IgemmParams& p) { return stem3_eligible(d, p); }

int launch_stem3_conv(const IgemmParams& p, hipStream_t stream) {
  Lds3Geo geo;
  geo.tilesX = p.GW / STEM_TW;
  geo.tilesY = p.GH / STEM_TH;
  geo.ntiles = p.N * geo.tilesX * geo.tilesY;
  geo.dy0 = -1;
  geo.dx0 = -1;
  geo.per_xcd = (geo.ntiles + 7) / 8;
  int blocks = geo.ntiles < 512 ? geo.ntiles : 512;
  blocks = (blocks + 7) / 8 * 8;
  DN_LAUNCH(stem3_conv_kernel, dim3(blocks), dim3(256), 0, stream, p, geo);
  set_last_kernel("dn::stem3_conv_kernel");
  return check_launch("stem3_conv_kernel");
}

struct Lds3Pick {
  int cfg;
  Lds3Geo geo;
};

static Lds3Pick lds3_pick(const dn_conv_desc* d, const IgemmParams& p) {
  Lds3Pick r;
  r.cfg = 0;
  if (knobs().no_lds3 || p.compute != DN_COMPUTE_F32X3) return r;
  if (p.reflect || p.bn_partial != nullptr || p.bnb_y != nullptr || p.Ntot > 32 || p.n_in > 2 || p.n_out < 1) return r;
  if (d->dilation > 1) return r;
  if (!(p.nphases == 1 || (p.nphases == 4 && p.Ntot <= 16))) return r;
  const KOperand& a = p.in[0];
  if (!(a.vec && a.small && a.up == 0 && a.scale == nullptr && (a.C == 16 || a.C == 32))) return r;
  const bool has1 = p.n_in == 2;
  if (has1) {
    const KOperand& b = p.in[1];
    if (!(b.C == 1 && b.small && b.scale == nullptr)) return r;
  }
  if (p.sy != p.sx || (p.sy != 1 && p.sy != 2)) return r;
  if (has1 && (p.sy != 1 || p.nphases != 1 || p.Ntot > 16)) return r;
  for (int i = 0; i < p.n_out; ++i)
    if (p.out[i].C < 1) return r;
  int dy0 = 127, dy1 = -127, dx0 = 127, dx1 = -127, maxtaps = 0;
  for (int z = 0; z < p.nphases; ++z) {
    const KPhase& ph = p.ph[z];
    if (ph.ntaps < 1) return r;
    if (ph.ntaps > maxtaps) maxtaps = ph.ntaps;
    for (int t = 0; t < ph.ntaps; ++t) {
      const int dy = p.tdy[ph.tap0 + t], dx = p.tdx[ph.tap0 + t];
      dy0 = dy < dy0 ? dy : dy0; dy1 = dy > dy1 ? dy : dy1;
      dx0 = dx < dx0 ? dx : dx0; dx1 = dx > dx1 ? dx : dx1;
    }
  }
  const int spanY = dy1 - dy0 + 1, spanX = dx1 - dx0 + 1;
  const int cg = a.C / 8, slots = maxtaps * cg + (has1 ? 2 : 0);
  if (has1 && maxtaps > 16) return r;
  const int roles = p.nphases == 4 ? 4 : (p.Ntot > 16 ? 2 : 1);
  int cfg = 0, TH = 8, TW = 32;
// ... 52 lines not shown
```

supervised_dispnet_amd/csrc/dn_plan.hip:

```cpp
#include <stdarg.h>
#include <stdlib.h>
#include <string.h>

#include <atomic>
#include <mutex>

#include "dn_internal.h"

namespace dn {

static thread_local char g_err[512] = "";

void set_error(const char* fmt, ...) {
  va_list ap;
  va_start(ap, fmt);
  vsnprintf(g_err, sizeof(g_err), fmt, ap);
  va_end(ap);
}

static thread_local char g_kernel[160] = "";

void set_last_kernel(const char* fmt, ...) {
  va_list ap;
  va_start(ap, fmt);
  vsnprintf(g_kernel, sizeof(g_kernel), fmt, ap);
  va_end(ap);
}

int check_launch(const char* what) {
  hipError_t e = hipGetLastError();
  if (e != hipSuccess) {
    set_error("%s: %s", what, hipGetErrorString(e));
    return DN_ERR_LAUNCH;
  }
  return DN_OK;
}

static int pick_bn(int ntot) { return ntot <= 32 ? 32 : (ntot <= 64 ? 64 : 128); }

static int ceil_div(int a, int b) { return (a + b - 1) / b; }

static int floor_div(int a, int b) {
  int q = a / b, r = a % b;
  return (r != 0 && ((r < 0) != (b < 0))) ? q - 1 : q;
}

static void fill_operand(KOperand* k, const dn_operand* o, int ch_off) {
  k->p = o->data;
  k->scale = o->scale;
  k->shift = o->shift;
  k->sn = o->stride_n;
  k->sh = o->stride_h;
  k->sw = o->stride_w;
  k->sc = o->stride_c;
  k->C = o->C;
  k->up = o->up_shift;
  bool aligned = ((reinterpret_cast<uintptr_t>(o->data) & 15) == 0) && (o->stride_n % 4 == 0) &&
                 (o->stride_h % 4 == 0) && (o->stride_w % 4 == 0);
  k->vec = (o->C % 4 == 0 && o->stride_c == 1 && aligned) ? 1 : 0;
// ... 35 lines not shown
  k->no_tap_windows = on("DN_NO_TAP_WINDOWS");
  k->wino_wg_target = num("DN_WINO_WG_TARGET", 0);
  k->wino_nmajor = num("DN_WINO_NMAJOR", 1);
  k->no_riding_fences = on("DN_NO_RIDING_FENCES");
  k->wino8 = num("DN_WINO8", -1);
}

const Knobs& knobs() {
  if (g_knobs_state.load(std::memory_order_acquire) == 0) {
    std::lock_guard<std::mutex> lock(g_knobs_mu);
    if (g_knobs_state.load(std::memory_order_relaxed) == 0) {
      read_knobs(&g_knobs);
      g_knobs_state.store(1, std::memory_order_release);
    }
  }
  return g_knobs;
}

int build_plan(const dn_conv_desc* d, bool for_wgrad, IgemmParams* p) {
  memset(p, 0, sizeof(*p));
  DN_REQUIRE(d != nullptr, DN_ERR_BAD_ARG, "null conv descriptor");
  DN_REQUIRE(d->kind >= DN_CONV_FWD && d->kind <= DN_CONVT_DGRAD, DN_ERR_BAD_ARG, "bad conv kind %d", d->kind);
  DN_REQUIRE(d->R >= 1 && d->S >= 1 && d->R * d->S <= 49, DN_ERR_UNSUPPORTED, "kernel %dx%d unsupported", d->R, d->S);
  DN_REQUIRE(d->stride >= 1 && d->stride <= 2, DN_ERR_UNSUPPORTED, "stride %d unsupported", d->stride);
  DN_REQUIRE(d->n_in >= 1 && d->n_in <= DN_MAX_OPERANDS, DN_ERR_BAD_ARG, "n_in %d", d->n_in);
  DN_REQUIRE(d->N > 0 && d->IH > 0 && d->IW > 0 && d->OH > 0 && d->OW > 0, DN_ERR_BAD_ARG, "bad sizes");
  int cin_total = 0;
  for (int i = 0; i < d->n_in; ++i) {
    DN_REQUIRE(d->in[i].C > 0 && (d->in[i].up_shift == 0 || d->in[i].up_shift == 1), DN_ERR_BAD_ARG, "operand %d", i);
    cin_total += d->in[i].C;
  }
  p->N = d->N;
  p->R = d->R;
  p->S = d->S;
  p->act = d->act;
  p->act_p0 = d->act_p0;
  p->act_p1 = d->act_p1;
  p->bias = d->bias;
  p->w = d->w_packed;
  p->bn_partial = d->bn_partial;
  if (d->kind == DN_CONV_DGRAD && !for_wgrad && d->bnb_y != nullptr && d->bnb_partial != nullptr) {
    DN_REQUIRE(d->bnb_scale && d->bnb_shift && d->bnb_mean && d->bnb_invstd, DN_ERR_BAD_ARG, "bnb_y needs scale / shift / mean / invstd");
    p->bnb_y = d->bnb_y;
    p->bnb_scale = d->bnb_scale;
    p->bnb_shift = d->bnb_shift;
    p->bnb_mean = d->bnb_mean;
    p->bnb_invstd = d->bnb_invstd;
    p->bnb_partial = d->bnb_partial;
  }
  if (!for_wgrad && d->kind == DN_CONV_FWD) p->recip_out = d->recip_out;
  if (!for_wgrad && d->splitk_ws != nullptr && d->splitk_ws_bytes > 0) {
    p->ks_ws = reinterpret_cast<float*>(d->splitk_ws);
    p->ks_ws_bytes = (size_t)d->splitk_ws_bytes;
    if (d->splitk_ws_bytes >= 8192 && (d->splitk_ws_bytes & 3) == 0) {
      p->ks_ws_bytes -= 256;
      p->fold_cnt = reinterpret_cast<int*>(reinterpret_cast<char*>(d->splitk_ws) + d->splitk_ws_bytes - 256);
    }
  }
  if (!for_wgrad && d->kind == DN_CONV_FWD && d->bn_partial != nullptr && d->bnf_scale != nullptr) {
    DN_REQUIRE(d->bnf_gamma && d->bnf_beta && d->bnf_mean && d->bnf_invstd && d->bnf_shift, DN_ERR_BAD_ARG,
               "bnf_scale needs gamma / beta / mean / invstd / shift");
    DN_REQUIRE((d->bnf_running_mean == nullptr) == (d->bnf_running_var == nullptr), DN_ERR_BAD_ARG, "bnf_running_mean and bnf_running_var go together");
    p->bnf.conv_bias = d->bias;
    p->bnf.gamma = d->bnf_gamma;
    p->bnf.beta = d->bnf_beta;
    p->bnf.running_mean = d->bnf_running_mean;
    p->bnf.running_var = d->bnf_running_var;
    p->bnf.num_batches_tracked = reinterpret_cast<long long*>(d->bnf_num_batches_tracked);
    p->bnf.momentum = d->bnf_momentum;
    p->bnf.eps = d->bnf_eps;
    p->bnf.mean = d->bnf_mean;
    p->bnf.invstd = d->bnf_invstd;
    p->bnf.scale = d->bnf_scale;
    p->bnf.shift = d->bnf_shift;
  }
  if (!for_wgrad && d->kind == DN_CONV_DGRAD && p->bnb_y != nullptr && d->bnb_dgamma != nullptr && d->bnb_dbeta != nullptr) {
    p->bnb_dgamma = d->bnb_dgamma;
    p->bnb_dbeta = d->bnb_dbeta;
  }
  const int st = d->stride, pad = d->pad;
  const int dil = d->dilation > 1 ? d->dilation : 1;
  DN_REQUIRE(d->pad_mode == 0 || d->pad_mode == 1, DN_ERR_BAD_ARG, "bad pad_mode %d", d->pad_mode);
  if (dil > 1) {
    DN_REQUIRE(st == 1 && d->pad_mode == 0 && (d->kind == DN_CONV_FWD || d->kind == DN_CONV_DGRAD), DN_ERR_UNSUPPORTED,
               "dilation %d: stride-1 zero-padded conv forward / input gradient / weight gradient only", dil);
    DN_REQUIRE((d->R - 1) * dil - pad <= 127 && (d->S - 1) * dil - pad <= 127 && pad <= 127, DN_ERR_UNSUPPORTED, "dilation %d: tap offsets beyond +-127", dil);
  }
  if (d->pad_mode == 1) {
    DN_REQUIRE(for_wgrad ? d->kind == DN_CONV_FWD : d->kind == DN_CONV_FWD, DN_ERR_UNSUPPORTED,
               "reflection padding is supported by the conv forward and its weight gradient only");
    DN_REQUIRE(pad < d->IH && pad < d->IW, DN_ERR_BAD_ARG, "reflection pad %d needs a larger input than %dx%d", pad, d->IH, d->IW);
    p->reflect = 1;
  }

  if (for_wgrad) {
    DN_REQUIRE(d->kind == DN_CONV_FWD || d->kind == DN_CONVT_FWD, DN_ERR_BAD_ARG, "wgrad needs a forward descriptor");
    p->nphases = 1;
    p->osy = p->osx = 1;
    p->sy = p->sx = st;
    p->n_is_dim0 = 1;
    int nt = 0;
    for (int r = 0; r < d->R; ++r)
      for (int s = 0; s < d->S; ++s) {
        p->tdy[nt] = (int8_t)(r * dil - pad);
        p->tdx[nt] = (int8_t)(s * dil - pad);
        p->tr[nt] = (int8_t)r;
        p->ts[nt] = (int8_t)s;
        ++nt;
      }
    p->ph[0].ntaps = nt;
// ... 116 lines not shown
  }
  long long m = (long long)p->N * p->GH * p->GW;
  DN_REQUIRE(m > 0 && m < (1ll << 31), DN_ERR_UNSUPPORTED, "grid too large");
  p->M = (int)m;
  p->mGW = fastdiv_magic((unsigned)p->GW);
  p->mGH = fastdiv_magic((unsigned)p->GH);
  p->allvec = 1;
  p->uni32 = 1;
  p->any_affine = 0;
  for (int z = 0; z < p->nphases; ++z)
    if (p->ph[z].ntaps > 32) p->uni32 = 0;
  int n_fast = 0, n_uniform = 0;
  for (int i = 0; i < p->n_in; ++i) {
    const KOperand& o = p->in[i];
    if (o.scale != nullptr) p->any_affine = 1;
    p->in[i].small = offsets_fit_int32(p->in[i], p->N, p->IH, p->IW) && ((long long)p->N * (o.sn < 0 ? -o.sn : o.sn) + 16) * 4 < (1ll << 31) ? 1 : 0;
    if (!(p->in[i].vec && p->in[i].small)) p->allvec = 0;
    if (p->in[i].vec && p->in[i].small && o.up == 0 && (o.C % 32 == 0 || o.C == 4 || o.C == 8 || o.C == 16)) ++n_fast;
    if (p->in[i].vec && p->in[i].small && o.up == 0 && o.C % 32 == 0) ++n_uniform;
  }
  (void)n_fast;
  if (p->reflect) p->uni32 = 0;
  for (int i = 0; i < p->n_in; ++i)
    if (!p->in[i].small) p->uni32 = 0;
  p->wg_uniform = (!p->reflect && p->ph[0].ntaps <= 32) ? 1 : 0;
  for (int i = 0; i < p->n_in; ++i) {
    const KOperand& o = p->in[i];
    if (!o.small || (!o.vec && o.scale != nullptr) || o.C >= 32768) p->wg_uniform = 0;
  }
  (void)n_uniform;
  p->tile_store = false ? 0 : (false ? 1 : 2);
  p->compute = norm_compute(d->compute);
  p->BN = pick_bn(p->Ntot);
  p->Npad = ceil_div(p->Ntot, p->BN) * p->BN;
  long long woff = 0;
  for (int z = 0; z < p->nphases; ++z) {
    int nch = 0;
    for (int i = 0; i < p->n_in; ++i) nch += ceil_div(p->ph[z].ntaps * p->in[i].C, kChunk);
    p->ph[z].nchunks = nch;
    p->ph[z].w_off = woff;
    woff += (long long)p->Npad * nch * kChunk;
  }
  return DN_OK;
}

static const ConvFamily* plan_route(const dn_conv_desc* d, IgemmParams* p) {
  return build_plan(d, false, p) == DN_OK ? conv_route(d, *p) : nullptr;
}

}

extern "C" {

int dn_version(void) { return 23; }

void dn_reload_knobs(void) {
  std::lock_guard<std::mutex> lock(dn::g_knobs_mu);
  dn::read_knobs(&dn::g_knobs);
  dn::g_knobs_state.store(1, std::memory_order_release);
}

const char* dn_last_error(void) { return dn::g_err; }

const char* dn_last_kernel(void) { return dn::g_kernel; }

int dn_device_arch_ok(void) {
  int dev = 0;
  if (hipGetDevice(&dev) != hipSuccess) {
    dn::set_error("hipGetDevice failed (no HIP device?)");
    return DN_ERR_LAUNCH;
  }
  hipDeviceProp_t prop;
  if (hipGetDeviceProperties(&prop, dev) != hipSuccess) {
    dn::set_error("hipGetDeviceProperties failed");
    return DN_ERR_LAUNCH;
  }
  return strncmp(prop.gcnArchName, "gfx950", 6) == 0 ? 1 : 0;
}

int64_t dn_conv_packed_weight_elems(const dn_conv_desc* d) {
  dn::IgemmParams p;
  const dn::ConvFamily* f = dn::plan_route(d, &p);
  if (f == nullptr) return -1;
  return f->weight_layout ? dn::wino_packed_floats(p, f->weight_layout(p)) : dn::direct_packed_elems(p);
}

int32_t dn_conv_weight_layout(const dn_conv_desc* d) {
  dn::IgemmParams p;
  const dn::ConvFamily* f = dn::plan_route(d, &p);
  return f == nullptr ? -1 : (f->weight_layout ? f->weight_layout(p) : 0);
}

int32_t dn_conv_bn_partial_rows(const dn_conv_desc* d) {
  dn::IgemmParams p;
  if (dn::build_plan(d, false, &p) != DN_OK) return -1;
  return (p.M + 127) / 128;
}

int32_t dn_conv_fwd_fuses_reciprocal(const dn_conv_desc* d) {
  dn::IgemmParams p;
  const dn::ConvFamily* f = dn::plan_route(d, &p);
  return (f != nullptr && f->fuses_reciprocal && f->fuses_reciprocal(p)) ? 1 : 0;
}

int32_t dn_conv_dgrad_fuses_bn_sums(const dn_conv_desc* d) {
  dn::IgemmParams p;
  const dn::ConvFamily* f = dn::plan_route(d, &p);
// ... 50 lines not shown
```

supervised_dispnet_amd/csrc/dn_wino_common.h:

```cpp
#pragma once
#include "dn_device.h"
#include "dn_fold.h"

namespace dn {

constexpr int WBT = 64;
constexpr int WBN = 64;
constexpr int WKC = 16;
constexpr int WZLD = 72;

template <int MTW>
struct WinoCfg {
  static constexpr int BT = 32 * MTW;
  static constexpr int HALFB = BT * 16 + 32;
  static constexpr int POSB = 2 * HALFB;
  static constexpr int SUBB = 16 * POSB + 64;
  static constexpr int BUFB = 2 * SUBB;
  static constexpr size_t LDS = (size_t)2 * BUFB;
};

constexpr int W16_ROWB = 48;

template <int NK, int TSTEP, int NWAVES, int GROUPS>
__device__ __forceinline__ void wino_bn_bwd_sums(const IgemmParams& p, const f32x4 (&Y)[NK][2][2], int mb, int tg, int c4, int wave, int lane, int tid,
// ... 15 lines not shown
        const int n = (int)fastdiv_dev(r, (unsigned)p.TH, p.mTH, &ty);
        const float* y00 = p.bnb_y + (((long long)n * p.OH + 2 * (int)ty) * p.OW + 2 * (int)tx) * C + n_first;
        const f32x4 yv[2][2] = {{*reinterpret_cast<const f32x4*>(y00), *reinterpret_cast<const f32x4*>(y00 + C)},
                                {*reinterpret_cast<const f32x4*>(y00 + rowB), *reinterpret_cast<const f32x4*>(y00 + rowB + C)}};
#pragma unroll
        for (int a = 0; a < 2; ++a)
#pragma unroll
          for (int b = 0; b < 2; ++b)
#pragma unroll
            for (int e = 0; e < 4; ++e) {
              const float yy = yv[a][b][e];
              const float dz = (yy * sc[e] + sh[e] > 0.f) ? Y[k][a][b][e] : 0.f;
              s1[(k * TSTEP) / 32][e] += dz;
              s2[(k * TSTEP) / 32][e] += dz * (yy - mu[e]) * is[e];
            }
      }
    }
  }
#pragma unroll
  for (int g = 0; g < GROUPS; ++g)
#pragma unroll
    for (int e = 0; e < 4; ++e) {
      s1[g][e] += __shfl_xor(s1[g][e], 16);
      s1[g][e] += __shfl_xor(s1[g][e], 32);
      s2[g][e] += __shfl_xor(s2[g][e], 16);
      s2[g][e] += __shfl_xor(s2[g][e], 32);
    }
  __syncthreads();
  if (lane < 16) {
#pragma unroll
    for (int g = 0; g < GROUPS; ++g) {
      *reinterpret_cast<f32x4*>(red + ((g * NWAVES + wave) * 2 + 0) * 64 + 4 * c4) = s1[g];
      *reinterpret_cast<f32x4*>(red + ((g * NWAVES + wave) * 2 + 1) * 64 + 4 * c4) = s2[g];
    }
  }
  __syncthreads();
  if (tid < 64 * GROUPS) {
    const int g = tid >> 6, col = tid & 63;
    float a1 = 0.f, a2 = 0.f;
#pragma unroll
    for (int w = 0; w < NWAVES; ++w) {
      a1 += red[((g * NWAVES + w) * 2 + 0) * 64 + col];
      a2 += red[((g * NWAVES + w) * 2 + 1) * 64 + col];
    }
    const int n = (n_first - 4 * c4) + col;
    if (n < p.Ntot && mb * BT + 32 * g < p.T) {
      float* dst = p.bnb_partial + ((long long)(GROUPS * mb + g) * p.Ntot + n) * 2;
      fold_store(dst, a1);
      fold_store(dst + 1, a2);
    }
  }
}

__device__ __forceinline__ void wino_fold_tail(const IgemmParams& p, int nb, int mblocks, float* lds, int tid) {
  if (!(p.fold_bn | p.fold_bnb)) return;
  __shared__ int fold_flag;
  if (!fold_last_arrival(p.fold_cnt + nb, mblocks, &fold_flag)) return;
  const int rows = (p.T + 31) / 32, c0 = nb * WBN;
  const int nlive = p.Ntot - c0 < WBN ? p.Ntot - c0 : WBN;
  double* red = reinterpret_cast<double*>(lds);
  if (p.fold_bn) bn_finalize_sliced<true>(p.bn_partial, rows, p.Ntot, c0, nlive, (double)p.M, p.bnf, red, tid);
  if (p.fold_bnb) colsum2_sliced<true>(p.bnb_partial, rows, p.Ntot, 2, 0, c0, nlive, p.bnb_dbeta, p.bnb_dgamma, red, tid);
}

bool wino8_wanted(const IgemmParams& p);
int launch_wino_conv8(const IgemmParams& p, hipStream_t stream);

}
```

supervised_dispnet_amd/csrc/dn_winograd.hip:

```cpp
#include <stdlib.h>
#include <type_traits>
#include <utility>

#include "dn_device.h"
#include "dn_wino_common.h"

namespace dn {

bool wino_eligible(const dn_conv_desc* d, const IgemmParams& p) {
  if (knobs().no_winograd) return false;
  if (!(d->kind == DN_CONV_FWD || d->kind == DN_CONV_DGRAD)) return false;
  if (d->R != 3 || d->S != 3 || d->stride != 1 || d->pad != 1 || d->pad_mode != 0 || d->dilation > 1) return false;
  if (d->IH != d->OH || d->IW != d->OW || (d->OH & 1) || (d->OW & 1)) return false;
  if (p.nphases != 1 || p.ph[0].ntaps != 9) return false;
  if (p.Ntot < 64) return false;
  if ((long long)p.M * 4 >= (1ll << 31)) return false;
  {
    const long long T = p.M / 4, Tpad = (T + 31) / 32 * 32, Npad = (p.Ntot + WBN - 1) / WBN * WBN;
    if (T * p.Ntot * 100 < Tpad * Npad * 60) return false;
    if (T < knobs().wino_min_tiles) return false;
  }
  for (int i = 0; i < p.n_in; ++i) {
    const KOperand& o = p.in[i];
    const bool scalar1 = o.C == 1 && o.small && o.scale == nullptr;
// ... 826 lines not shown
          if (accumulate) {
            const f32x4 g00 = *reinterpret_cast<const f32x4*>(o00), g01 = *reinterpret_cast<const f32x4*>(o00 + sw);
            const f32x4 g10 = *reinterpret_cast<const f32x4*>(o00 + rowB), g11 = *reinterpret_cast<const f32x4*>(o00 + rowB + sw);
            v[0][0] += g00;
            v[0][1] += g01;
            v[1][0] += g10;
            v[1][1] += g11;
          }
          *reinterpret_cast<f32x4*>(o00) = v[0][0];
          *reinterpret_cast<f32x4*>(o00 + sw) = v[0][1];
          *reinterpret_cast<f32x4*>(o00 + rowB) = v[1][0];
          *reinterpret_cast<f32x4*>(o00 + rowB + sw) = v[1][1];
        }
      }
    } else {
#pragma unroll
      for (int k = 0; k < NK; ++k) {
        const int t = mb * BT + tg + 16 * k;
        if (t < p.T) {
          unsigned tx, ty;
          const unsigned r = fastdiv_dev((unsigned)t, (unsigned)p.TW, p.mTW, &tx);
          const int n = (int)fastdiv_dev(r, (unsigned)p.TH, p.mTH, &ty);
          const long long pix0 = ((long long)n * p.OH + 2 * (int)ty) * p.OW + 2 * (int)tx;
#pragma unroll
          for (int a = 0; a < 2; ++a)
#pragma unroll
            for (int b = 0; b < 2; ++b) {
              const long long pix = pix0 + (long long)a * p.OW + b;
#pragma unroll
              for (int e = 0; e < 4; ++e) {
                const int col = n_first + e;
                if (col < p.Ntot) {
                  const float val = apply_act(Y[k][a][b][e] + bias[e], p.act, p.act_p0, p.act_p1);
                  int sg = 0;
                  if (p.n_out > 1 && col >= p.out[1].n_begin) sg = 1;
                  if (p.n_out > 2 && col >= p.out[2].n_begin) sg = 2;
                  const KResult& Q = p.out[sg];
                  float* o = Q.p + pix * Q.sw + (col - Q.n_begin);
                  *o = Q.accumulate ? *o + val : val;
                }
              }
            }
        }
      }
    }
  }
  if (p.fold_bn | p.fold_bnb) {
    __syncthreads();
    unsigned bx = blockIdx.x;
    asm volatile("" : "+s"(bx));
    const int MT2 = (p.T + BT - 1) / BT, NT2 = p.Npad / WBN;
    const int per2 = (MT2 * NT2 + 7) >> 3;
    const int q2 = (int)(bx & 7u) * per2 + (int)(bx >> 3);
    wino_fold_tail(p, p.nmajor ? q2 / MT2 : q2 % NT2, MT2, smem, (int)threadIdx.x);
  }
}

bool wino_folds_bn_finalize(const IgemmParams& p) {
  return p.bnf.scale != nullptr && p.bn_partial != nullptr && p.fold_cnt != nullptr && (p.T + 31) / 32 <= kFoldMaxRows &&
         wino_npad(p) / WBN <= kFoldCounters;
}
bool wino_folds_bn_sums(const IgemmParams& p) {
  return p.bnb_dgamma != nullptr && p.bnb_dbeta != nullptr && p.bnb_partial != nullptr && p.fold_cnt != nullptr && (p.T + 31) / 32 <= kFoldMaxRows &&
         wino_npad(p) / WBN <= kFoldCounters;
}

template <int MTW, bool HA, int PREC = 0>
static int launch_wino_variant(const IgemmParams& p, hipStream_t stream) {
  using Cfg = WinoCfg<MTW>;
  auto kernel = wino_conv_kernel<MTW, HA, PREC>;
  constexpr size_t lds16a = (size_t)2 * 16 * Cfg::BT * W16_ROWB;
  constexpr size_t lds16b = (size_t)(4 * Cfg::BT * WZLD + MTW * 8 * 64) * sizeof(float);
  constexpr size_t lds = PREC == 1 ? (lds16a > lds16b ? lds16a : lds16b) : Cfg::LDS;
  hipError_t e = hipFuncSetAttribute(reinterpret_cast<const void*>(kernel), hipFuncAttributeMaxDynamicSharedMemorySize, (int)lds);
  if (e != hipSuccess) {
    set_error("hipFuncSetAttribute(wino_conv_kernel, %zu): %s", lds, hipGetErrorString(e));
    return DN_ERR_LAUNCH;
  }
  const int tiles = ((p.T + Cfg::BT - 1) / Cfg::BT) * (p.Npad / WBN);
  dim3 grid((tiles + 7) / 8 * 8, (PREC == 3 && MTW == 1 && p.ksplit > 1) ? p.ksplit : 1);
  DN_LAUNCH(kernel, grid, dim3(256), lds, stream, p);
  set_last_kernel("dn::wino_conv_kernel<%d, %s, %d>", MTW, HA ? "true" : "false", PREC);
  return check_launch("wino_conv_kernel");
}

void wino_prepare(IgemmParams& p) {
  const int wl = wino_layout(p);
  p.compute = wl == 2 ? DN_COMPUTE_BF16 : (wl == 3 ? DN_COMPUTE_F32X3 : DN_COMPUTE_F32);
  p.Npad = wino_npad(p);
  p.T = p.M / 4;
  p.TH = p.OH / 2;
  p.TW = p.OW / 2;
  p.mTW = fastdiv_magic((unsigned)p.TW);
  p.mTH = fastdiv_magic((unsigned)p.TH);
}

int launch_wino_conv(IgemmParams& p, hipStream_t stream) {
  wino_prepare(p);
  {
    const int nm = knobs().wino_nmajor, nt = p.Npad / WBN;
    p.nmajor = p.compute == DN_COMPUTE_F32X3 && (nm == 1 || (nm == 2 && nt >= 4) || (nm == 3 && nt >= 8));
  }
  p.fold_bn = wino_folds_bn_finalize(p) ? 1 : 0;
  p.fold_bnb = wino_folds_bn_sums(p) ? 1 : 0;
  if (p.compute == DN_COMPUTE_BF16)
    return p.any_affine ? launch_wino_variant<1, true, 1>(p, stream) : launch_wino_variant<1, false, 1>(p, stream);
  p.ksplit = 1;
  if (p.compute == DN_COMPUTE_F32X3) {
    if (wino8_wanted(p)) return launch_wino_conv8(p, stream);
    const int ks = wino_splitk_choice(p);
    if (ks > 1 && p.ks_ws != nullptr && p.ks_ws_bytes >= wino_splitk_workspace_bytes(p)) {
      p.ksplit = ks;
      p.ks_chunks = wino_ktot(p) / WKC;
      p.ks_cnt_floats = kSplitKCounterBytes / 4;
    }
    return p.any_affine ? launch_wino_variant<1, true, 3>(p, stream) : launch_wino_variant<1, false, 3>(p, stream);
  }
// ... 5 lines not shown
```

supervised_dispnet_amd/csrc/dn_winograd8.hip:

```cpp
#include <stdlib.h>

#include "dn_device.h"
#include "dn_wino_common.h"

namespace dn {

namespace {
constexpr int BT8 = 64;
constexpr size_t kXchgBytes = (size_t)8 * BT8 * WZLD * sizeof(float);
constexpr size_t kStatBytes = (size_t)(2 * 8 * 2 * 64) * sizeof(float);
constexpr size_t kLds8 = kXchgBytes + kStatBytes;
static_assert(kLds8 >= WinoCfg<2>::LDS, "the epilogue's exchange area must cover the main loop's two chunk buffers");
static_assert(kLds8 <= 160 * 1024, "one CU has 160 KB of LDS");
}

template <bool HA>
__global__ void __launch_bounds__(512, 1) wino_conv8_kernel(const IgemmParams p) {
  using Cfg = WinoCfg<2>;
  constexpr int BT = BT8, HALFB = Cfg::HALFB, POSB = Cfg::POSB, SUBB = Cfg::SUBB, BUFB = Cfg::BUFB;
  extern __shared__ __align__(16) float smem[];
  char* smemB = reinterpret_cast<char*>(smem);
  const int tid = threadIdx.x, lane = tid & 63, wave = __builtin_amdgcn_readfirstlane(tid >> 6);
  const int wi = wave >> 1, jh = wave & 1;
  const int MT = (p.T + BT - 1) / BT, NT = p.Npad / WBN;
// ... 455 lines not shown
              v[a][b] = Y[k][a][b] + bias;
              if (!plain) {
#pragma unroll
                for (int e = 0; e < 4; ++e) v[a][b][e] = apply_act(v[a][b][e], p.act, p.act_p0, p.act_p1);
              }
            }
          if (accumulate) {
            const f32x4 g00 = *reinterpret_cast<const f32x4*>(o00), g01 = *reinterpret_cast<const f32x4*>(o00 + sw);
            const f32x4 g10 = *reinterpret_cast<const f32x4*>(o00 + rowB), g11 = *reinterpret_cast<const f32x4*>(o00 + rowB + sw);
            v[0][0] += g00;
            v[0][1] += g01;
            v[1][0] += g10;
            v[1][1] += g11;
          }
          *reinterpret_cast<f32x4*>(o00) = v[0][0];
          *reinterpret_cast<f32x4*>(o00 + sw) = v[0][1];
          *reinterpret_cast<f32x4*>(o00 + rowB) = v[1][0];
          *reinterpret_cast<f32x4*>(o00 + rowB + sw) = v[1][1];
        }
      }
    } else {
#pragma unroll
      for (int k = 0; k < NK; ++k) {
        const int t = mb * BT + tg + 32 * k;
        if (t < p.T) {
          unsigned tx, ty;
          const unsigned r = fastdiv_dev((unsigned)t, (unsigned)p.TW, p.mTW, &tx);
          const int n = (int)fastdiv_dev(r, (unsigned)p.TH, p.mTH, &ty);
          const long long pix0 = ((long long)n * p.OH + 2 * (int)ty) * p.OW + 2 * (int)tx;
#pragma unroll
          for (int a = 0; a < 2; ++a)
#pragma unroll
            for (int b = 0; b < 2; ++b) {
              const long long pix = pix0 + (long long)a * p.OW + b;
#pragma unroll
              for (int e = 0; e < 4; ++e) {
                const int col = n_first + e;
                if (col < p.Ntot) {
                  const float val = apply_act(Y[k][a][b][e] + bias[e], p.act, p.act_p0, p.act_p1);
                  int sg = 0;
                  if (p.n_out > 1 && col >= p.out[1].n_begin) sg = 1;
                  if (p.n_out > 2 && col >= p.out[2].n_begin) sg = 2;
                  const KResult& Q = p.out[sg];
                  float* o = Q.p + pix * Q.sw + (col - Q.n_begin);
                  *o = Q.accumulate ? *o + val : val;
                }
              }
            }
        }
      }
    }
  }
  __syncthreads();
  wino_fold_tail(p, nb, MT, smem, tid);
}

template <bool HA>
static int launch_wino8(const IgemmParams& p, hipStream_t stream) {
  auto kernel = wino_conv8_kernel<HA>;
  hipError_t e = hipFuncSetAttribute(reinterpret_cast<const void*>(kernel), hipFuncAttributeMaxDynamicSharedMemorySize, (int)kLds8);
  if (e != hipSuccess) {
    set_error("hipFuncSetAttribute(wino_conv8_kernel, %zu): %s", kLds8, hipGetErrorString(e));
    return DN_ERR_LAUNCH;
  }
  const int tiles = ((p.T + BT8 - 1) / BT8) * (p.Npad / WBN);
  IgemmParams q = p;
  q.ksplit = 1;
  int blocks = (tiles + 7) / 8 * 8;
  if (!knobs().no_wino8_tail && p.ks_ws != nullptr) {
    const int cus = 256, reg = tiles / cus * cus, tail = tiles - reg;
    int chunks = 0;
    for (int i = 0; i < p.n_in; ++i) chunks += (p.in[i].C + WKC - 1) / WKC;
    int ks = tail > 0 ? cus / tail : 1;
    if (ks > chunks / 8) ks = chunks / 8;
    if (ks > 8) ks = 8;
    const size_t need = 4096 + (size_t)tail * ks * 32 * 512 * 16;
    if (reg > 0 && reg <= 3 * cus && tail > 0 && tail % 8 == 0 && tail <= 64 && ks >= 2 && p.ks_ws_bytes >= need) {
      q.ksplit = ks;
      q.ks_chunks = chunks;
      q.ks_cnt_floats = 4096 / 4;
      q.ks_reg = reg;
      q.ks_tail = tail;
      blocks = reg + tail * ks;
    }
  }
  dim3 grid(blocks);
  DN_LAUNCH(kernel, grid, dim3(512), kLds8, stream, q);
  set_last_kernel("dn::wino_conv8_kernel<%s>", HA ? "true" : "false");
  return check_launch("wino_conv8_kernel");
}

bool wino8_wanted(const IgemmParams& p) {
  if (p.compute != DN_COMPUTE_F32X3) return false;
  const int mode = knobs().wino8;
  if (mode == 0) return false;
  if (mode == 1) return true;
  int k = 0;
  for (int i = 0; i < p.n_in; ++i) k += (p.in[i].C + WKC - 1) / WKC * WKC;
  const long long blocks = (long long)((p.M / 4 + BT8 - 1) / BT8) * ((p.Ntot + WBN - 1) / WBN);
  return k >= 128 && blocks >= 192;
}

int launch_wino_conv8(const IgemmParams& p, hipStream_t stream) {
  return p.any_affine ? launch_wino8<true>(p, stream) : launch_wino8<false>(p, stream);
}

}
// ... 1 lines not shown
```

supervised_dispnet_amd/engine.py:

```python
import ctypes as C
import math
import os
import threading
import weakref

import torch

from . import _lib
from ._lib import (ACT_LEAKY, ACT_NONE, ACT_RELU, ACT_SIGMOID_AFFINE, CONV_DGRAD, CONV_FWD, CONVT_DGRAD, CONVT_FWD,
                   ConvDesc)

BN_EPS = 1e-5
BN_MOMENTUM = 0.1

PARAM_EPOCH = 0


PROFILE = None

SPLITK = True
PACK_ON_SIDE_STREAM = True
PACK_LATE_MIN_ELEMS = 400000
BN_SUMS_FUSION = True
FOLD_FINALIZE = True
# ... 146 lines not shown
    if pause:
        _lib.call("dn_tape_pause", TAPE["handle"], 1)
        TAPE["paused"] = True
    try:
        with torch.cuda.device(device), outside_tape_pool():
            props = torch.cuda.get_device_properties(device)
            if "gfx950" not in getattr(props, "gcnArchName", "gfx950") or props.multi_processor_count % 8:
                ok = False
            shapes = ((8, 16, 1), (104, 4, 1), (32, 2, 4))
            side = side_stream()["sides"][0]
            outs = []
            for st in (torch.cuda.current_stream(device), side):
                for gx, gy, gz in shapes:
                    o = torch.full((gx * gy * gz,), -1, dtype=torch.int32, device=device)
                    side.wait_stream(torch.cuda.current_stream(device))
                    _lib.call("dn_xcd_probe", o.data_ptr(), gx, gy, gz, st.cuda_stream)
                    outs.append((o, gx))
            torch.cuda.synchronize(device)
            for o, gx in outs:
                ids = o.cpu().view(-1, gx)
                if int(ids.min()) < 0 or int(ids.max()) > 7 or not bool((ids == ids[0:1]).all()):
                    ok = False
    except Exception:
        ok = False
    finally:
        if pause:
            TAPE["paused"] = False
            _lib.call("dn_tape_pause", TAPE["handle"], 0)
    if not ok:
        import warnings
        warnings.warn("supervised_dispnet_amd: block -> XCD placement on this device is not blockIdx.x % 8; K split of small grids disabled")
    _XCD_OK[device.index] = ok
    return ok


def _splitk_workspace(d, device):
    if not SPLITK or device.type != "cuda" or not xcd_placement_ok(device):
        return
    h = _stream()
    cur = _SPLITK.get((device.index, h))
    if cur is None:
        with torch.cuda.device(device):
            sides = side_stream()["handles"]
        if h in sides:
            _SPLITK[(device.index, h)] = cur = (None, 0, None, None)
        else:
            with outside_tape_pool():
                buf = torch.zeros(_SPLITK_BYTES // 4, dtype=torch.float32, device=device)
            cur = _SPLITK[(device.index, h)] = (buf, _SPLITK_BYTES, None, buf.data_ptr())
    if cur[0] is None:
        return
    d.splitk_ws = cur[3]
    d.splitk_ws_bytes = cur[1]


def _pick_bn(ntot):
    return 32 if ntot <= 32 else (64 if ntot <= 64 else 128)


class _Timed(object):

    def __init__(self, name, flops, tag="", abytes=0):
        self.name, self.flops, self.tag, self.abytes = name, flops, tag, abytes

    def __enter__(self):
        if PROFILE is not None:
            self.e0 = torch.cuda.Event(enable_timing=True)
            self.e1 = torch.cuda.Event(enable_timing=True)
            self.e0.record()
        return self

    def __exit__(self, *exc):
        if PROFILE is not None:
            self.e1.record()
            launched = _lib.load().dn_last_kernel().decode(errors="replace")
            PROFILE.append((launched or self.name, self.flops, self.e0, self.e1, self.tag, 0, int(self.abytes)))
        return False


def hbm_call(kernel, nbytes, entry, *args):
    if PROFILE is None:
        return _lib.call(entry, *args)
    e0 = torch.cuda.Event(enable_timing=True)
    e1 = torch.cuda.Event(enable_timing=True)
    e0.record()
    _lib.call(entry, *args)
    e1.record()
    if kernel is None:
        kernel = _lib.load().dn_last_kernel().decode(errors="replace")
    PROFILE.append((kernel, 0, e0, e1, entry, int(nbytes), int(nbytes)))


def bump_param_epoch():
    global PARAM_EPOCH
    PARAM_EPOCH += 1


_TLS = threading.local()


def _stream():
    h = getattr(_TLS, "handle", None)
    return h if h is not None else torch.cuda.current_stream().cuda_stream


class stream_scope(object):
# ... 643 lines not shown
                         y.t.data_ptr(), y.scale.data_ptr(), y.shift.data_ptr(), mean.data_ptr(), invstd.data_ptr(), gamma, y.rows, Cn,
                         sums.partial.data_ptr(), _stream())
    y.bn_sums = None
    dgamma, dbeta = sink.dest_or_new(bn.weight), sink.dest_or_new(bn.bias)
    dbias = sink.dest_or_new(conv_bias) if conv_bias is not None else None
    home = _stream()

    def finish():
        h = _stream()
        _lib.call("dn_bn_frozen_finalize", sums.partial.data_ptr(), sums.rows, sums.stride, sums.offset, Cn, bn.weight.data_ptr(),
                  invstd.data_ptr(), dgamma.data_ptr(), dbeta.data_ptr(), _ptr(dbias), h)
        if h != home:
            cur = torch.cuda.current_stream()
            cross_stream_use(invstd, cur)
            for prm, t in ((bn.weight, dgamma), (bn.bias, dbeta), (conv_bias, dbias)):
                if t is not None and sink.dest(prm) is None:
                    cross_stream_use(t, cur)
        sink.put(bn.weight, dgamma)
        sink.put(bn.bias, dbeta)
        if dbias is not None:
            sink.put(conv_bias, dbias)

    if defer is not None:
        defer.append((finish, sums.partial))
    else:
        finish()
    return g


def bn_backward(y, bn, sink, conv_bias=None, defer=None):
    g, y_t, Cn, dev = y.grad, y.t, y.C, y.t.device
    if y.frozen is not None:
        return _bn_backward_frozen(y, bn, sink, conv_bias, defer)
    if y.mean is None:
        raise RuntimeError("bn_backward: the forward of this BatchNorm was not recorded (neither batch statistics nor a frozen state on it)")
    relu_pending = not y.grad_is_dz
    sums = y.bn_sums
    if relu_pending and (sums is None or BN_MATERIALIZE_DZ):
        if y.no_relu:
            raise RuntimeError("a ReLU-less BatchNorm output must be consumed by block_bn_add_relu / block_bn_plain")
        nblk = _lib.load().dn_reduce_blocks(y.rows, Cn)
        sums = BnSums(torch.empty((nblk, Cn, 2), dtype=torch.float32, device=dev), nblk)
        if BN_MATERIALIZE_DZ:
            hbm_call("dn::colreduce_kernel<dn::BnReluBwdOp, 4>", y.rows * Cn * 12, "dn_bn_relu_bwd_reduce", g.data_ptr(),
                     y_t.data_ptr(), y.scale.data_ptr(), y.shift.data_ptr(), y.mean.data_ptr(), y.invstd.data_ptr(), y.rows, Cn,
                     sums.partial.data_ptr(), _stream())
        else:
            hbm_call("dn::colreduce_kernel<dn::BnReluBwdOp, 4>", y.rows * Cn * 8, "dn_bn_relu_bwd_sums", g.data_ptr(),
                     y_t.data_ptr(), y.scale.data_ptr(), y.shift.data_ptr(), y.mean.data_ptr(), y.invstd.data_ptr(), y.rows, Cn,
                     sums.partial.data_ptr(), _stream())
    elif sums is None:
        raise RuntimeError("bn_backward: the column sums of this dz are gone (a second consumer added to the gradient after they were taken)")
    dgamma, dbeta = sums.final if sums.final is not None else (sink.dest_or_new(bn.weight), sink.dest_or_new(bn.bias))
    if y.pool_src is not None:
        dpooled, pidx = y.pool_src
        hbm_call("dn::bn_bwd_apply_pool_kernel", y.rows * Cn * 8 + y.rows * Cn * 5 // 4, "dn_bn_bwd_apply_pool", dpooled.data_ptr(),
                 pidx.data_ptr(), y_t.data_ptr(), y.mean.data_ptr(), y.invstd.data_ptr(), bn.weight.data_ptr(), sums.partial.data_ptr(),
                 sums.rows, sums.stride, sums.offset, y.N, y.H, y.W, Cn, g.data_ptr(), dgamma.data_ptr(),
                 dbeta.data_ptr(), _stream())
        y.pool_src = None
    elif relu_pending and not BN_MATERIALIZE_DZ:
        hbm_call(None, y.rows * Cn * 12, "dn_bn_bwd_apply_relu", g.data_ptr(), y_t.data_ptr(),
                 y.scale.data_ptr(), y.shift.data_ptr(), y.mean.data_ptr(), y.invstd.data_ptr(), bn.weight.data_ptr(),
                 None if sums.final is not None else sums.partial.data_ptr(), sums.rows, sums.stride, sums.offset, y.rows, Cn,
                 dgamma.data_ptr(), dbeta.data_ptr(), _stream())
    else:
        hbm_call(None, y.rows * Cn * 12, "dn_bn_bwd_apply", g.data_ptr(), y_t.data_ptr(), y.mean.data_ptr(),
                 y.invstd.data_ptr(), bn.weight.data_ptr(), sums.partial.data_ptr(), sums.rows, sums.stride,
                 sums.offset, y.rows, Cn, dgamma.data_ptr(), dbeta.data_ptr(), _stream())
    y.bn_sums = None
    sink.put(bn.weight, dgamma)
    sink.put(bn.bias, dbeta)
    return g


def _bn_finalize(bn, partial, prow, count, conv_bias, mean, invstd, scale, shift, nbt):
    _lib.call("dn_bn_finalize", partial.data_ptr(), prow, scale.numel(), count, _ptr(conv_bias.detach()) if conv_bias is not None else None,
              bn.weight.data_ptr(), bn.bias.data_ptr(), bn.running_mean.data_ptr(), bn.running_var.data_ptr(),
              bn.momentum if bn.momentum is not None else BN_MOMENTUM, bn.eps, mean.data_ptr(), invstd.data_ptr(),
              scale.data_ptr(), shift.data_ptr(), nbt, _stream())


def _bn_pending(y, bn, partial, prow, training, conv_bias=None, record=False):
    Cn, dev = y.C, y.t.device
    if not training:
        _bn_frozen_affine(y, bn, record)
        return
    y.scale = torch.empty(Cn, dtype=torch.float32, device=dev)
    y.shift = torch.empty(Cn, dtype=torch.float32, device=dev)
    y.mean = torch.empty(Cn, dtype=torch.float32, device=dev)
    y.invstd = torch.empty(Cn, dtype=torch.float32, device=dev)
    _bn_finalize(bn, partial, prow, y.rows, conv_bias, y.mean, y.invstd, y.scale, y.shift, _nbt_ptr(bn))


def block_conv_bn(tape, sink, x_piece, layer, bn, training, relu=True):
    xa = x_piece.act
    dev = xa.t.device
    Cn = layer.Cout
    if not bn.training:
        y_t, _, _ = conv_forward(layer, [x_piece], ACT_NONE)
        OH, OW = y_t.shape[1], y_t.shape[2]
        y = Act(y_t, xa.N, OH, OW, Cn)
        y.no_relu = not relu
        _bn_frozen_affine(y, bn, tape.recording)

        def backward_frozen():
            if y.grad is None:
                return
            fin = []
            g = bn_backward(y, bn, sink, conv_bias=layer.m.bias, defer=fin)
            conv_wgrad(layer, [x_piece], g, (OH, OW), out=sink.dest(layer.m.weight), sink=sink, first=fin[0])
            conv_dgrad(layer, g, xa.N, OH, OW, [x_piece], (xa.H, xa.W))
            y.grad = None

        tape.push(backward_frozen)
        return y
    scale = torch.empty(Cn, dtype=torch.float32, device=dev)
    shift = torch.empty(Cn, dtype=torch.float32, device=dev)
    mean = torch.empty(Cn, dtype=torch.float32, device=dev)
    invstd = torch.empty(Cn, dtype=torch.float32, device=dev)
    nbt = _nbt_ptr(bn)
    fold = [bn, mean, invstd, scale, shift, nbt]
    y_t, partial, prow = conv_forward(layer, [x_piece], ACT_NONE, bn_stats=True, bn_fold=fold)
    OH, OW = y_t.shape[1], y_t.shape[2]
    y = Act(y_t, xa.N, OH, OW, Cn)
    y.no_relu = not relu
    y.scale, y.shift, y.mean, y.invstd = scale, shift, mean, invstd
    y.bn_owner = (bn, sink)
    if fold[0] is not True:
        _bn_finalize(bn, partial, prow, y.rows, layer.m.bias, mean, invstd, scale, shift, nbt)

    def backward():
        if y.grad is None:
            return
        g = bn_backward(y, bn, sink)
        if layer.m.bias is not None:
            sink.put_zero(layer.m.bias)
        conv_wgrad(layer, [x_piece], g, (OH, OW), out=sink.dest(layer.m.weight), sink=sink)
        conv_dgrad(layer, g, xa.N, OH, OW, [x_piece], (xa.H, xa.W))
        y.grad = None

    tape.push(backward)
    return y


def block_pool(tape, y):
    dev = y.t.device
    p_t = torch.empty((y.N, y.H // 2, y.W // 2, y.C), dtype=torch.float32, device=dev)
    idx = torch.empty((y.N, y.H // 2, y.W // 2, y.C), dtype=torch.uint8, device=dev)
    hbm_call("dn::bn_relu_pool_fwd_kernel", y.rows * y.C * 4 * 1.25 + y.rows * y.C // 4, "dn_bn_relu_pool_fwd", y.t.data_ptr(),
             y.scale.data_ptr(), y.shift.data_ptr(), y.N, y.H, y.W, y.C, p_t.data_ptr(), idx.data_ptr(), _stream())
    p = Act(p_t, y.N, y.H // 2, y.W // 2, y.C)

    def backward():
        if p.grad is None:
            return
        if y.frozen is not None:
            y.grad = y.new_like()
            y.grad_is_dz = True
            y.pool_src = (p.grad, idx)
            p.grad = None
            return
        nblk = _lib.load().dn_reduce_blocks(p.rows, y.C)
        sums = y.bn_sums = BnSums(torch.empty((nblk, y.C, 2), dtype=torch.float32, device=dev), nblk)
        y.grad = y.new_like()
        y.grad_is_dz = True
        if BN_MATERIALIZE_DZ:
            hbm_call("dn::colreduce_kernel<dn::PoolBwdOp, 4>", y.rows * y.C * 4 * 2.25 + y.rows * y.C // 4, "dn_bn_relu_pool_bwd",
                     p.grad.data_ptr(), idx.data_ptr(), y.t.data_ptr(), y.mean.data_ptr(), y.invstd.data_ptr(), y.N, y.H, y.W, y.C,
                     y.grad.data_ptr(), sums.partial.data_ptr(), _stream())
        else:
            hbm_call("dn::colreduce_kernel<dn::PoolBwdOp, 4>", y.rows * y.C * 4 * 1.25 + y.rows * y.C // 4, "dn_bn_relu_pool_bwd_sums",
                     p.grad.data_ptr(), idx.data_ptr(), y.t.data_ptr(), y.mean.data_ptr(), y.invstd.data_ptr(), y.N, y.H, y.W, y.C,
                     sums.partial.data_ptr(), _stream())
            y.pool_src = (p.grad, idx)
        p.grad = None

    tape.push(backward)
    return p


def block_conv_act(tape, sink, pieces, layer, act, p0=0.0, p1=0.0, out_hw=None, stat_bn=None):
    if stat_bn is not None and not stat_bn.training:
        stat_bn = None
    a0 = pieces[0].act
    in_hw = (a0.H * (2 if pieces[0].up else 1), a0.W * (2 if pieces[0].up else 1))
    want_recip = [] if (FUSE_RECIP and act == ACT_SIGMOID_AFFINE and layer.Cout == 1 and stat_bn is None and p1 > 0) else None
    y_t, partial, prow = conv_forward(layer, pieces, act, p0, p1, out_hw=out_hw, bn_stats=stat_bn is not None, recip=want_recip)
    OH, OW = y_t.shape[1], y_t.shape[2]
    y = Act(y_t, a0.N, OH, OW, layer.Cout)
    if want_recip:
        y.recip_t = want_recip[0]
    if stat_bn is not None:
        scratch = torch.empty((4, layer.Cout), dtype=torch.float32, device=y_t.device)
        _bn_finalize(stat_bn, partial, prow, y.rows, layer.m.bias, *scratch, _nbt_ptr(stat_bn))

    def backward():
        if y.grad is None:
            sink.put_none(layer.m.weight)
            if layer.m.bias is not None:
                sink.put_none(layer.m.bias)
            return
        g, g_src = y.grad, None
        if y.grad_borrowed:
            g_src, g, y.grad_borrowed = g, torch.empty_like(y.grad), False
        finish_db, db_partial = act_bwd(g, y_t, act, p0, p1, y.rows, layer.Cout,
                                        out=sink.dest(layer.m.bias) if layer.m.bias is not None else None, defer=True, src=g_src)

        def bias_grad():
            db = finish_db()
            if layer.m.bias is not None:
                sink.put(layer.m.bias, db)
            return db if (layer.m.bias is None or sink.dest(layer.m.bias) is None) else None

        conv_wgrad(layer, pieces, g, (OH, OW), out=sink.dest(layer.m.weight), sink=sink, first=(bias_grad, db_partial))
        conv_dgrad(layer, g, a0.N, OH, OW, pieces, in_hw)
        y.grad = None

    tape.push(backward, out=y)
    return y


def _not_on_tape(what):
    if TAPE is not None and not TAPE.get("paused"):
        raise RuntimeError("launch tape: %s runs outside libdispnet_hip and would be missing from the replay" % what)


# ... 403 lines not shown
```

Before: 2003.

## Fold BN column-sum finalize into producer kernels via multi-level group counters

Replaces the single-block-per-channel BN finalize and colsum kernels with a two-level fold. Row groups are reduced in parallel, and the last-arriving block merges the group records using workspace counters. The winograd fold tail and the pool-backward sums reduce are extended so that large row counts can also fold the finalize into the producing kernel, which drops the separate finalize launches and their serial reductions. This adds atomic counter and workspace complexity, and a serial fallback is kept for when the workspace is too small.

```diff
diff --git a/include/dispnet_hip.h b/include/dispnet_hip.h
--- a/include/dispnet_hip.h
+++ b/include/dispnet_hip.h
@@ -125,6 +125,10 @@
                    const float* gamma, const float* beta, float* running_mean, float* running_var, float momentum,
                    float eps, float* mean, float* invstd, float* scale, float* shift, int64_t* num_batches_tracked,
                    dn_stream_t stream);
+int dn_bn_finalize_ws(const float* partial, int32_t rows, int32_t C, int64_t count, const float* conv_bias,
+                      const float* gamma, const float* beta, float* running_mean, float* running_var, float momentum,
+                      float eps, float* mean, float* invstd, float* scale, float* shift, int64_t* num_batches_tracked,
+                      void* ws, int64_t ws_bytes, dn_stream_t stream);
 int dn_bn_eval_affine(int32_t C, const float* gamma, const float* beta, const float* running_mean,
                       const float* running_var, float eps, float* scale, float* shift, dn_stream_t stream);
 int dn_bn_relu_pool_fwd(const float* y, const float* scale, const float* shift, int32_t N, int32_t H, int32_t W,
@@ -150,6 +154,11 @@
                          const float* partial, int32_t partial_rows, int32_t partial_stride, int32_t partial_offset, int32_t N, int32_t H,
                          int32_t W, int32_t C, float* dy, float* dgamma, float* dbeta, dn_stream_t stream);
 int32_t dn_reduce_blocks(int64_t rows, int32_t C);
+int dn_bn_bwd_sums_finish(const float* partial, int32_t partial_rows, int32_t partial_stride, int32_t partial_offset, int32_t C,
+                          float* dgamma, float* dbeta, void* ws, int64_t ws_bytes, dn_stream_t stream);
+int dn_bn_relu_pool_bwd_sums_finish(const float* dpooled, const uint8_t* idx, const float* y, const float* mean, const float* invstd,
+                                    int32_t N, int32_t H, int32_t W, int32_t C, float* partial, float* dgamma, float* dbeta, void* ws,
+                                    int64_t ws_bytes, dn_stream_t stream);
 
 int dn_bn_frozen_affine(int32_t C, const float* gamma, const float* beta, const float* running_mean, const float* running_var, float eps,
                         float* scale, float* shift, float* invstd, dn_stream_t stream);
diff --git a/supervised_dispnet_amd/_lib.py b/supervised_dispnet_amd/_lib.py
--- a/supervised_dispnet_amd/_lib.py
+++ b/supervised_dispnet_amd/_lib.py
@@ -5,7 +5,7 @@
 _PKG = pathlib.Path(__file__).resolve().parent
 LIB_PATH = pathlib.Path(os.environ.get("DISPNET_HIP_LIB", _PKG / "libdispnet_hip.so"))
 
-EXPECTED_ABI = 23
+EXPECTED_ABI = 24
 
 DN_MAX_OPERANDS = 3
 ACT_NONE, ACT_RELU, ACT_LEAKY, ACT_ELU, ACT_SIGMOID_AFFINE = 0, 1, 2, 3, 4
@@ -71,6 +71,9 @@
     "dn_conv_wgrad_workspace_bytes": (_sz, [_P(ConvDesc)]),
     "dn_conv2d_wgrad": (C.c_int, [_P(ConvDesc), _vp, _vp, _vp, _sz, _vp]),
     "dn_bn_finalize": (C.c_int, [_vp, _i32, _i32, _i64, _vp, _vp, _vp, _vp, _vp, _f, _f, _vp, _vp, _vp, _vp, _vp, _vp]),
+    "dn_bn_finalize_ws": (C.c_int, [_vp, _i32, _i32, _i64, _vp, _vp, _vp, _vp, _vp, _f, _f, _vp, _vp, _vp, _vp, _vp, _vp, _i64, _vp]),
+    "dn_bn_bwd_sums_finish": (C.c_int, [_vp, _i32, _i32, _i32, _i32, _vp, _vp, _vp, _i64, _vp]),
+    "dn_bn_relu_pool_bwd_sums_finish": (C.c_int, [_vp, _vp, _vp, _vp, _vp, _i32, _i32, _i32, _i32, _vp, _vp, _vp, _vp, _i64, _vp]),
     "dn_bn_eval_affine": (C.c_int, [_i32, _vp, _vp, _vp, _vp, _f, _vp, _vp, _vp]),
     "dn_bn_relu_pool_fwd": (C.c_int, [_vp, _vp, _vp, _i32, _i32, _i32, _i32, _vp, _vp, _vp]),
     "dn_bn_relu_bwd_sums": (C.c_int, [_vp, _vp, _vp, _vp, _vp, _vp, _i64, _i32, _vp, _vp]),
diff --git a/supervised_dispnet_amd/csrc/dn_bn.hip b/supervised_dispnet_amd/csrc/dn_bn.hip
--- a/supervised_dispnet_amd/csrc/dn_bn.hip
+++ b/supervised_dispnet_amd/csrc/dn_bn.hip
@@ -4,76 +4,77 @@
 namespace dn {
 
 constexpr int kBnTileRows = 128;
-__global__ void __launch_bounds__(kThreads) bn_finalize_kernel(const float* __restrict__ partial, int rows, int C, double count,
-                                                               const float* __restrict__ conv_bias, const float* __restrict__ gamma,
-                                                               const float* __restrict__ beta, float* running_mean, float* running_var,
-                                                               float momentum, float eps, float* mean_out, float* invstd_out, float* scale,
-                                                               float* shift, long long* num_batches_tracked) {
-  const int c = blockIdx.x;
-  if (num_batches_tracked != nullptr && c == 0 && threadIdx.x == 0) num_batches_tracked[0] += 1;
-  __shared__ double red[3][4];
-  double s1 = 0.0, q = 0.0, pp = 0.0;
-  const double n0 = count < (double)kBnTileRows ? count : (double)kBnTileRows;
-  const double pivot = (double)partial[(long long)c * 2] / n0;
-#pragma unroll 8
-  for (int r = threadIdx.x; r < rows; r += kThreads) {
-    const float2 v = *reinterpret_cast<const float2*>(partial + ((long long)r * C + c) * 2);
-    const double left = count - (double)r * kBnTileRows;
-    const double nt = left < (double)kBnTileRows ? left : (double)kBnTileRows;
-    const double dm = (double)v.x / nt - pivot;
-    s1 += (double)v.x;
-    q += (double)v.y;
-    pp += nt * dm * dm;
-  }
-#pragma unroll
-  for (int o = 32; o > 0; o >>= 1) {
-    s1 += __shfl_xor(s1, o);
-    q += __shfl_xor(q, o);
-    pp += __shfl_xor(pp, o);
-  }
-  if ((threadIdx.x & 63) == 0) {
-    red[0][threadIdx.x >> 6] = s1;
-    red[1][threadIdx.x >> 6] = q;
-    red[2][threadIdx.x >> 6] = pp;
-  }
-  __syncthreads();
-  double macc = 0.0, m2tot = 0.0;
-  if (threadIdx.x == 0) {
-    const double S = (red[0][0] + red[0][1]) + (red[0][2] + red[0][3]);
-    const double Q = (red[1][0] + red[1][1]) + (red[1][2] + red[1][3]);
-    const double P = (red[2][0] + red[2][1]) + (red[2][2] + red[2][3]);
-    macc = S / count;
-    m2tot = Q + (P - count * (macc - pivot) * (macc - pivot));
-  }
-  if (threadIdx.x == 0) {
-    double var = m2tot / count;
-    if (var < 0.0) var = 0.0;
-    const float mean = (float)(macc + (conv_bias ? (double)conv_bias[c] : 0.0));
-    const float invstd = (float)(1.0 / sqrt(var + (double)eps));
-    const float sc = gamma[c] * invstd;
-    mean_out[c] = mean;
-    invstd_out[c] = invstd;
-    scale[c] = sc;
-    shift[c] = beta[c] - mean * sc;
-    if (running_mean) {
-      const double unbiased = count > 1.0 ? var * count / (count - 1.0) : var;
-      running_mean[c] = (1.f - momentum) * running_mean[c] + momentum * mean;
-      running_var[c] = (1.f - momentum) * running_var[c] + momentum * (float)unbiased;
-    }
-  }
-}
-
-__global__ void __launch_bounds__(256) bn_finalize_sliced_kernel(const float* __restrict__ partial, int rows, int C, double count, BnFinalizeArgs a) {
+
+__global__ void __launch_bounds__(256) bn_finalize_levels_kernel(const float* __restrict__ partial, int rows, int C, double count, BnFinalizeArgs a,
+                                                                 FoldWs ws) {
   __shared__ double red[3 * kFoldSlices * 64];
-  const int c0 = blockIdx.x * 64;
-  bn_finalize_sliced<false>(partial, rows, C, c0, C - c0 < 64 ? C - c0 : 64, count, a, red, threadIdx.x);
-}
-
-__global__ void __launch_bounds__(256) colsum2_sliced_kernel(const float* __restrict__ partial, int rows, int C, int stride, int offset,
+  __shared__ int flag;
+  fold_bn_levels<false>(partial, rows, C, (int)blockIdx.x, (int)blockIdx.y, count, a, ws.cnt, ws.rec, red, &flag, threadIdx.x);
+}
+
+__global__ void __launch_bounds__(256) bn_finalize_serial_kernel(const float* __restrict__ partial, int rows, int C, double count, BnFinalizeArgs a) {
+  __shared__ double red[3 * kFoldSlices * 64];
+  __shared__ double lrec[3][64];
+  const int tid = threadIdx.x, cl = tid & 63, sl = tid >> 6, c0 = blockIdx.x * 64;
+  const int nlive = C - c0 < 64 ? C - c0 : 64;
+  const bool live = cl < nlive;
+  const int groups = (rows + kFoldMaxRows - 1) / kFoldMaxRows;
+  double A[3] = {0.0, 0.0, 0.0}, rec[3];
+  for (int g = 0; g < groups; ++g) {
+    const int r0 = g * kFoldMaxRows;
+    bn_group_sliced<false>(partial, r0, r0 + kFoldMaxRows < rows ? r0 + kFoldMaxRows : rows, C, c0, nlive, count, red, tid, rec);
+    if (live && sl == 0) {
+      lrec[0][cl] = rec[0];
+      lrec[1][cl] = rec[1];
+      lrec[2][cl] = rec[2];
+    }
+    __syncthreads();
+    if (live && sl == (g & (kFoldSlices - 1))) {
+      const double B[3] = {lrec[0][cl], lrec[1][cl], lrec[2][cl]};
+      bn_chan_merge(A, B);
+    }
+    __syncthreads();
+  }
+  bn_merge_slices(A, live, red, tid);
+  if (live && sl == 0) bn_finalize_record(A, c0 + cl, count, a);
+  if (tid == 0 && c0 == 0 && a.num_batches_tracked != nullptr) a.num_batches_tracked[0] += 1;
+}
+
+__global__ void __launch_bounds__(256) colsum2_levels_kernel(const float* __restrict__ partial, int rows, int C, int stride, int offset,
+                                                             float* __restrict__ out0, float* __restrict__ out1, FoldWs ws) {
+  __shared__ double red[2 * kFoldSlices * 64];
+  __shared__ int flag;
+  fold_colsum2_levels<false>(partial, rows, C, stride, offset, (int)blockIdx.x, (int)blockIdx.y, out0, out1, ws.cnt, ws.rec, red, &flag, threadIdx.x);
+}
+
+__global__ void __launch_bounds__(256) colsum2_serial_kernel(const float* __restrict__ partial, int rows, int C, int stride, int offset,
                                                              float* __restrict__ out0, float* __restrict__ out1) {
   __shared__ double red[2 * kFoldSlices * 64];
-  const int c0 = blockIdx.x * 64;
-  colsum2_sliced<false>(partial, rows, C, stride, offset, c0, C - c0 < 64 ? C - c0 : 64, out0, out1, red, threadIdx.x);
+  __shared__ double lrec[2][64];
+  const int tid = threadIdx.x, cl = tid & 63, sl = tid >> 6, c0 = blockIdx.x * 64;
+  const int nlive = C - c0 < 64 ? C - c0 : 64;
+  const bool live = cl < nlive;
+  const int groups = (rows + kFoldMaxRows - 1) / kFoldMaxRows;
+  double A[2] = {0.0, 0.0}, s[2];
+  for (int g = 0; g < groups; ++g) {
+    const int r0 = g * kFoldMaxRows;
+    colsum2_group_sliced<false>(partial, r0, r0 + kFoldMaxRows < rows ? r0 + kFoldMaxRows : rows, C, stride, offset, c0, nlive, red, tid, s);
+    if (live && sl == 0) {
+      lrec[0][cl] = s[0];
+      lrec[1][cl] = s[1];
+    }
+    __syncthreads();
+    if (live && sl == (g & (kFoldSlices - 1))) {
+      A[0] += lrec[0][cl];
+      A[1] += lrec[1][cl];
+    }
+    __syncthreads();
+  }
+  colsum2_merge_slices(A, live, red, tid);
+  if (live && sl == 0) {
+    out0[c0 + cl] = (float)A[0];
+    out1[c0 + cl] = (float)A[1];
+  }
 }
 
 __global__ void bn_eval_affine_kernel(int C, const float* gamma, const float* beta, const float* rm, const float* rv, float eps,
@@ -623,9 +624,15 @@
   __shared__ double red[2 * kFoldSlices * 64];
   const int c0 = blockIdx.x * 64;
   const int nlive = C - c0 < 64 ? C - c0 : 64;
-  colsum2_sliced<false>(partial, rows, C, stride, offset, c0, nlive, dbeta, dgamma, red, threadIdx.x);
+  double s[2];
+  colsum2_group_sliced<false>(partial, 0, rows, C, stride, offset, c0, nlive, red, threadIdx.x, s);
   const int cl = threadIdx.x & 63;
-  if (dbias != nullptr && (threadIdx.x >> 6) == 0 && cl < nlive) dbias[c0 + cl] = bn_frozen_dbias(gamma[c0 + cl], invstd[c0 + cl], dbeta[c0 + cl]);
+  if ((threadIdx.x >> 6) == 0 && cl < nlive) {
+    const float db = (float)s[0];
+    dbeta[c0 + cl] = db;
+    dgamma[c0 + cl] = (float)s[1];
+    if (dbias != nullptr) dbias[c0 + cl] = bn_frozen_dbias(gamma[c0 + cl], invstd[c0 + cl], db);
+  }
 }
 
 __global__ void __launch_bounds__(256) bn_frozen_finalize_kernel(const float* __restrict__ partial, int rows, int C, int stride, int offset,
@@ -684,27 +691,49 @@
   return check_launch(what);
 }
 
+static void launch_colsum2(const float* partial, int32_t partial_rows, int32_t C, int32_t partial_stride, int32_t partial_offset, float* out0,
+                           float* out1, hipStream_t s, const FoldWs* ws = nullptr) {
+  const FoldWs none{nullptr, nullptr, nullptr};
+  const FoldWs& f = ws != nullptr ? *ws : none;
+  const int groups = (partial_rows + kFoldMaxRows - 1) / kFoldMaxRows;
+  if ((partial_stride & 1) != 0 || (partial_offset & 1) != 0 || (reinterpret_cast<uintptr_t>(partial) & 7) != 0)
+    DN_LAUNCH(colsum2_finalize_kernel, dim3(C), dim3(256), 0, s, partial, partial_rows, C, partial_stride, partial_offset, out0, out1);
+  else if (groups == 1 || fold_levels_fit(f, partial_rows, C))
+    DN_LAUNCH(colsum2_levels_kernel, dim3((C + 63) / 64, groups), dim3(256), 0, s, partial, partial_rows, C, partial_stride, partial_offset, out0,
+              out1, f);
+  else
+    DN_LAUNCH(colsum2_serial_kernel, dim3((C + 63) / 64), dim3(256), 0, s, partial, partial_rows, C, partial_stride, partial_offset, out0, out1);
+}
+
 }
 
 using namespace dn;
 
 extern "C" {
+
+int dn_bn_finalize_ws(const float* partial, int32_t rows, int32_t C, int64_t count, const float* conv_bias, const float* gamma,
+                      const float* beta, float* running_mean, float* running_var, float momentum, float eps, float* mean, float* invstd,
+                      float* scale, float* shift, int64_t* num_batches_tracked, void* ws, int64_t ws_bytes, dn_stream_t stream) {
+  DN_REQUIRE(partial && gamma && beta && mean && invstd && scale && shift && rows > 0 && C > 0 && count > 0, DN_ERR_BAD_ARG,
+             "dn_bn_finalize: bad argument");
+  const BnFinalizeArgs a{conv_bias, gamma, beta, running_mean, running_var, reinterpret_cast<long long*>(num_batches_tracked), momentum, eps,
+                         mean, invstd, scale, shift};
+  FoldWs f;
+  fold_ws_of(ws, ws_bytes, &f);
+  const int groups = (rows + kFoldMaxRows - 1) / kFoldMaxRows;
+  if (groups == 1 || fold_levels_fit(f, rows, C)) {
+    DN_LAUNCH(bn_finalize_levels_kernel, dim3((C + 63) / 64, groups), dim3(256), 0, as_stream(stream), partial, rows, C, (double)count, a, f);
+    return check_launch("bn_finalize_levels_kernel");
+  }
+  DN_LAUNCH(bn_finalize_serial_kernel, dim3((C + 63) / 64), dim3(256), 0, as_stream(stream), partial, rows, C, (double)count, a);
+  return check_launch("bn_finalize_serial_kernel");
+}
 
 int dn_bn_finalize(const float* partial, int32_t rows, int32_t C, int64_t count, const float* conv_bias, const float* gamma,
                    const float* beta, float* running_mean, float* running_var, float momentum, float eps, float* mean, float* invstd,
                    float* scale, float* shift, int64_t* num_batches_tracked, dn_stream_t stream) {
-  DN_REQUIRE(partial && gamma && beta && mean && invstd && scale && shift && rows > 0 && C > 0 && count > 0, DN_ERR_BAD_ARG,
-             "dn_bn_finalize: bad argument");
-  if (rows <= kFoldMaxRows) {
-    const BnFinalizeArgs a{conv_bias, gamma, beta, running_mean, running_var, reinterpret_cast<long long*>(num_batches_tracked), momentum, eps,
-                           mean, invstd, scale, shift};
-    DN_LAUNCH(bn_finalize_sliced_kernel, dim3((C + 63) / 64), dim3(256), 0, as_stream(stream), partial, rows, C, (double)count, a);
-    return check_launch("bn_finalize_sliced_kernel");
-  }
-  DN_LAUNCH(bn_finalize_kernel, dim3(C), dim3(kThreads), 0, as_stream(stream), partial, rows, C, (double)count, conv_bias, gamma,
-                     beta, running_mean, running_var, momentum, eps, mean, invstd, scale, shift,
-                     reinterpret_cast<long long*>(num_batches_tracked));
-  return check_launch("bn_finalize_kernel");
+  return dn_bn_finalize_ws(partial, rows, C, count, conv_bias, gamma, beta, running_mean, running_var, momentum, eps, mean, invstd, scale, shift,
+                           num_batches_tracked, nullptr, 0, stream);
 }
 
 int dn_bn_eval_affine(int32_t C, const float* gamma, const float* beta, const float* running_mean, const float* running_var, float eps,
@@ -822,6 +851,36 @@
   return launch_colreduce(op, (long long)N * (H / 2) * (W / 2), C, partial, as_stream(stream), "bn_relu_pool_bwd_sums");
 }
 
+int dn_bn_relu_pool_bwd_sums_finish(const float* dpooled, const uint8_t* idx, const float* y, const float* mean, const float* invstd, int32_t N,
+                                    int32_t H, int32_t W, int32_t C, float* partial, float* dgamma, float* dbeta, void* ws, int64_t ws_bytes,
+                                    dn_stream_t stream) {
+  DN_REQUIRE(dpooled && idx && y && mean && invstd && partial && dgamma && dbeta, DN_ERR_BAD_ARG, "dn_bn_relu_pool_bwd_sums_finish: null pointer");
+  DN_REQUIRE(C % 4 == 0 && H % 2 == 0 && W % 2 == 0, DN_ERR_UNSUPPORTED, "dn_bn_relu_pool_bwd_sums_finish: need C%%4==0 and even H,W");
+  PoolBwdOp op{dpooled, idx, y, mean, invstd, nullptr, H / 2, W / 2, H, W, C};
+  const long long rows = (long long)N * (H / 2) * (W / 2);
+  hipStream_t s = as_stream(stream);
+  FoldWs f;
+  fold_ws_of(ws, ws_bytes, &f);
+  if (launch_colreduce_finish(op, rows, C, partial, f, dbeta, dgamma, s)) {
+    set_last_kernel("dn::colreduce_finish_kernel<dn::PoolBwdOp, 4>");
+    return check_launch("bn_relu_pool_bwd_sums_finish");
+  }
+  int rc = launch_colreduce(op, rows, C, partial, s, "bn_relu_pool_bwd_sums");
+  if (rc != DN_OK) return rc;
+  launch_colsum2(partial, reduce_blocks(rows, C), C, 2, 0, dbeta, dgamma, s, &f);
+  return check_launch("bn_bwd_sums_finish");
+}
+
+int dn_bn_bwd_sums_finish(const float* partial, int32_t partial_rows, int32_t partial_stride, int32_t partial_offset, int32_t C, float* dgamma,
+                          float* dbeta, void* ws, int64_t ws_bytes, dn_stream_t stream) {
+  DN_REQUIRE(partial && dgamma && dbeta && partial_rows > 0 && C > 0, DN_ERR_BAD_ARG, "dn_bn_bwd_sums_finish: bad argument");
+  DN_REQUIRE(partial_stride >= 2 && partial_offset >= 0 && partial_offset + 1 < partial_stride, DN_ERR_BAD_ARG, "dn_bn_bwd_sums_finish: partial layout");
+  FoldWs f;
+  fold_ws_of(ws, ws_bytes, &f);
+  launch_colsum2(partial, partial_rows, C, partial_stride, partial_offset, dbeta, dgamma, as_stream(stream), &f);
+  return check_launch("bn_bwd_sums_finish");
+}
+
 int dn_bn_relu_bwd_reduce(float* da_dz, const float* y, const float* scale, const float* shift, const float* mean, const float* invstd,
                           int64_t rows, int32_t C, float* partial, dn_stream_t stream) {
   DN_REQUIRE(da_dz && y && scale && shift && mean && invstd && partial && rows > 0 && C > 0, DN_ERR_BAD_ARG,
@@ -835,14 +894,6 @@
   DN_REQUIRE(da && y && scale && shift && mean && invstd && partial && rows > 0 && C > 0, DN_ERR_BAD_ARG, "dn_bn_relu_bwd_sums: bad argument");
   BnReluBwdOp op{0, const_cast<float*>(da), y, scale, shift, mean, invstd, C};
   return launch_colreduce(op, rows, C, partial, as_stream(stream), "bn_relu_bwd_sums");
-}
-
-static void launch_colsum2(const float* partial, int32_t partial_rows, int32_t C, int32_t partial_stride, int32_t partial_offset, float* out0,
-                           float* out1, hipStream_t s) {
-  if (partial_rows <= kFoldMaxRows && (partial_stride & 1) == 0 && (partial_offset & 1) == 0 && (reinterpret_cast<uintptr_t>(partial) & 7) == 0)
-    DN_LAUNCH(colsum2_sliced_kernel, dim3((C + 63) / 64), dim3(256), 0, s, partial, partial_rows, C, partial_stride, partial_offset, out0, out1);
-  else
-    DN_LAUNCH(colsum2_finalize_kernel, dim3(C), dim3(256), 0, s, partial, partial_rows, C, partial_stride, partial_offset, out0, out1);
 }
 
 static int bn_bwd_sums_to_params(const float* partial, int32_t partial_rows, int32_t partial_stride, int32_t partial_offset, int32_t C,
@@ -883,11 +934,10 @@
 int dn_bn_bwd_apply(float* dz_dy, const float* y, const float* mean, const float* invstd, const float* gamma, const float* partial,
                     int32_t partial_rows, int32_t partial_stride, int32_t partial_offset, int64_t rows, int32_t C, float* dgamma,
                     float* dbeta, dn_stream_t stream) {
-  DN_REQUIRE(dz_dy && y && mean && invstd && gamma && partial && dgamma && dbeta && rows > 0, DN_ERR_BAD_ARG, "dn_bn_bwd_apply: bad argument");
-  DN_REQUIRE(C % 4 == 0, DN_ERR_UNSUPPORTED, "dn_bn_bwd_apply: need C%%4==0");
-  DN_REQUIRE(partial_stride >= 2 && partial_offset >= 0 && partial_offset + 1 < partial_stride, DN_ERR_BAD_ARG, "dn_bn_bwd_apply: partial layout");
+  DN_REQUIRE(dz_dy && y && mean && invstd && gamma && rows > 0, DN_ERR_BAD_ARG, "dn_bn_bwd_apply: bad argument");
   hipStream_t s = as_stream(stream);
-  launch_colsum2(partial, partial_rows, C, partial_stride, partial_offset, dbeta, dgamma, s);
+  int rc = bn_bwd_sums_to_params(partial, partial_rows, partial_stride, partial_offset, C, dgamma, dbeta, s, "dn_bn_bwd_apply");
+  if (rc != DN_OK) return rc;
   return launch_bn_bwd_apply<false>(dz_dy, y, nullptr, nullptr, mean, invstd, gamma, dgamma, dbeta, rows, C, s, "bn_bwd_apply");
 }
 
diff --git a/supervised_dispnet_amd/csrc/dn_colreduce.h b/supervised_dispnet_amd/csrc/dn_colreduce.h
--- a/supervised_dispnet_amd/csrc/dn_colreduce.h
+++ b/supervised_dispnet_amd/csrc/dn_colreduce.h
@@ -1,5 +1,6 @@
 #pragma once
 #include "dn_device.h"
+#include "dn_fold.h"
 
 namespace dn {
 
@@ -27,8 +28,8 @@
   return (int)b;
 }
 
-template <class Op, int V>
-__global__ void __launch_bounds__(kThreads) colreduce_kernel(Op op, long long rows, int C, float* __restrict__ partial) {
+template <class Op, int V, bool AGENT>
+__device__ __forceinline__ void colreduce_body(const Op& op, long long rows, int C, float* __restrict__ partial, float* red) {
   constexpr int NACC = Op::NACC;
   const int groups = C / V;
   int tpr = 1;
@@ -38,7 +39,6 @@
   const long long per = (rows + gridDim.x - 1) / gridDim.x;
   const long long rbeg = blockIdx.x * per;
   const long long rend = (rbeg + per < rows) ? rbeg + per : rows;
-  __shared__ float red[kThreads * V * NACC];
   for (int g0 = 0; g0 < groups; g0 += tpr) {
     const int grp = g0 + gi;
     float acc[V][NACC];
@@ -60,9 +60,46 @@
         for (int a = 0; a < NACC; ++a) {
           float s = 0.f;
           for (int q = 0; q < rpi; ++q) s += red[((q * tpr + gi) * V + v) * NACC + a];
-          partial[((long long)blockIdx.x * C + grp * V + v) * NACC + a] = s;
+          float* dst = partial + ((long long)blockIdx.x * C + grp * V + v) * NACC + a;
+          if constexpr (AGENT) fold_store(dst, s);
+          else *dst = s;
         }
     }
+    __syncthreads();
+  }
+}
+
+template <class Op, int V>
+__global__ void __launch_bounds__(kThreads) colreduce_kernel(Op op, long long rows, int C, float* __restrict__ partial) {
+  __shared__ float red[kThreads * V * Op::NACC];
+  colreduce_body<Op, V, false>(op, rows, C, partial, red);
+}
+
+template <class Op, int V>
+__global__ void __launch_bounds__(kThreads) colreduce_finish_kernel(Op op, long long rows, int C, float* __restrict__ partial, FoldWs ws,
+                                                                    float* __restrict__ out0, float* __restrict__ out1) {
+  static_assert(Op::NACC == 2, "the finish takes pairs");
+  __shared__ float red[kThreads * V * 2];
+  __shared__ double dred[2 * kFoldSlices * 64];
+  __shared__ int last[kFoldCounters];
+  __shared__ int flag;
+  colreduce_body<Op, V, true>(op, rows, C, partial, red);
+  const int prow = (int)gridDim.x, nsl = (C + 63) / 64, tid = (int)threadIdx.x;
+  const int g = prow > kFoldMaxRows ? (int)blockIdx.x / kFoldMaxRows : 0;
+  const int left = prow - g * kFoldMaxRows;
+  const int expected = left < kFoldMaxRows ? left : kFoldMaxRows;
+  asm volatile("s_waitcnt vmcnt(0)" ::: "memory");
+  __syncthreads();
+  if (tid < nsl) {
+    int* counter = prow > kFoldMaxRows ? ws.cnt1 + tid * kFoldMaxGroups + g : ws.cnt + tid;
+    const int prev = __hip_atomic_fetch_add(counter, 1, __ATOMIC_RELAXED, __HIP_MEMORY_SCOPE_AGENT);
+    last[tid] = (prev == expected - 1) ? 1 : 0;
+    if (prev == expected - 1) __hip_atomic_store(counter, 0, __ATOMIC_RELAXED, __HIP_MEMORY_SCOPE_AGENT);
+  }
+  __syncthreads();
+  for (int nb = 0; nb < nsl; ++nb) {
+    if (last[nb] == 0) continue;
+    fold_colsum2_levels<true>(partial, prow, C, 2, 0, nb, g, out0, out1, ws.cnt, ws.rec, dred, &flag, tid);
     __syncthreads();
   }
 }
@@ -75,6 +112,14 @@
   else
     DN_LAUNCH((colreduce_kernel<Op, 1>), dim3(blocks), dim3(kThreads), 0, s, op, rows, C, partial);
   return check_launch(what);
+}
+
+template <class Op>
+static bool launch_colreduce_finish(const Op& op, long long rows, int C, float* partial, const FoldWs& ws, float* out0, float* out1, hipStream_t s) {
+  const int blocks = reduce_blocks(rows, C);
+  if (C % 4 != 0 || !fold_levels_fit(ws, blocks, C) || (reinterpret_cast<uintptr_t>(partial) & 7) != 0) return false;
+  DN_LAUNCH((colreduce_finish_kernel<Op, 4>), dim3(blocks), dim3(kThreads), 0, s, op, rows, C, partial, ws, out0, out1);
+  return true;
 }
 
 template <int V>
diff --git a/supervised_dispnet_amd/csrc/dn_conv.hip b/supervised_dispnet_amd/csrc/dn_conv.hip
--- a/supervised_dispnet_amd/csrc/dn_conv.hip
+++ b/supervised_dispnet_amd/csrc/dn_conv.hip
@@ -19,7 +19,8 @@
               r.stride_h == (int64_t)d->OW * r.C && r.stride_n == (int64_t)d->OH * d->OW * r.C && d->bias == nullptr && d->act == DN_ACT_NONE;
      },
      [](IgemmParams& p) { wino_prepare(p); return wino_folds_bn_finalize(p); }, [](IgemmParams& p) { wino_prepare(p); return wino_folds_bn_sums(p); }},
-    {"stem3", stem3_conv_eligible, nullptr, plan_only<launch_stem3_conv>, nullptr, x3_upper},
+    {"stem3", stem3_conv_eligible, nullptr, plan_only<launch_stem3_conv>, nullptr, x3_upper, nullptr, nullptr,
+     [](IgemmParams& p) { return stem3_folds_bn_finalize(p); }},
     {"stemk", stemk_conv_eligible, nullptr, with_desc<launch_stemk_conv>, nullptr, x3_upper},
     {"stem", stem_eligible, nullptr, plan_only<launch_stem>, nullptr, x3_upper},
     {"lds3", lds3_conv_eligible, nullptr, with_desc<launch_lds3_conv>, nullptr, x3_upper},
diff --git a/supervised_dispnet_amd/csrc/dn_fold.h b/supervised_dispnet_amd/csrc/dn_fold.h
--- a/supervised_dispnet_amd/csrc/dn_fold.h
+++ b/supervised_dispnet_amd/csrc/dn_fold.h
@@ -9,8 +9,48 @@
 constexpr int kFoldMaxRows = 128;
 constexpr int kFoldSlices = 4;
 constexpr int kFoldCounters = 64;
+constexpr int kFoldMaxGroups = 128;
+constexpr int kFoldLevelSlices = 8;
+constexpr size_t kFoldCnt1Bytes = (size_t)kFoldLevelSlices * kFoldMaxGroups * sizeof(int);
+constexpr size_t kFoldRecBytes = (size_t)kFoldLevelSlices * 64 * kFoldMaxGroups * 24;
+constexpr size_t kFoldWsBytes = 256 + kFoldCnt1Bytes + kFoldRecBytes;
+
+static inline size_t fold_ws_of(void* ws, long long bytes, FoldWs* f) {
+  f->cnt = nullptr;
+  f->cnt1 = nullptr;
+  f->rec = nullptr;
+  if (ws == nullptr || bytes < 8192 || (bytes & 3) != 0) return 0;
+  char* end = reinterpret_cast<char*>(ws) + bytes;
+  f->cnt = reinterpret_cast<int*>(end - 256);
+  if ((size_t)bytes < kFoldWsBytes + 8192 || (reinterpret_cast<uintptr_t>(end) & 7) != 0) return 256;
+  f->cnt1 = reinterpret_cast<int*>(end - 256 - kFoldCnt1Bytes);
+  f->rec = reinterpret_cast<double*>(end - kFoldWsBytes);
+  return kFoldWsBytes;
+}
+
+static inline bool fold_levels_fit(const FoldWs& f, int rows, int C) {
+  if (f.cnt == nullptr || rows < 1 || (C + 63) / 64 > kFoldCounters) return false;
+  if (rows <= kFoldMaxRows) return true;
+  return f.rec != nullptr && (rows + kFoldMaxRows - 1) / kFoldMaxRows <= kFoldMaxGroups && (C + 63) / 64 <= kFoldLevelSlices;
+}
+
+#if defined(__HIPCC__)
+__device__ __forceinline__ int* fold_cnt1_of(int* cnt) { return reinterpret_cast<int*>(reinterpret_cast<char*>(cnt) - kFoldCnt1Bytes); }
+__device__ __forceinline__ double* fold_rec_of(int* cnt) {
+  return reinterpret_cast<double*>(reinterpret_cast<char*>(cnt) + 256 - kFoldWsBytes);
+}
 
 __device__ __forceinline__ void fold_store(float* p, float v) { __hip_atomic_store(p, v, __ATOMIC_RELAXED, __HIP_MEMORY_SCOPE_AGENT); }
+__device__ __forceinline__ void fold_store2(float* p, float v0, float v1) {
+  const unsigned long long u = (unsigned long long)__builtin_bit_cast(unsigned, v0) | ((unsigned long long)__builtin_bit_cast(unsigned, v1) << 32);
+  __hip_atomic_store(reinterpret_cast<unsigned long long*>(p), u, __ATOMIC_RELAXED, __HIP_MEMORY_SCOPE_AGENT);
+}
+__device__ __forceinline__ void fold_stored(double* p, double v) {
+  __hip_atomic_store(reinterpret_cast<unsigned long long*>(p), __builtin_bit_cast(unsigned long long, v), __ATOMIC_RELAXED, __HIP_MEMORY_SCOPE_AGENT);
+}
+__device__ __forceinline__ double fold_loadd(const double* p) {
+  return __builtin_bit_cast(double, __hip_atomic_load(reinterpret_cast<const unsigned long long*>(p), __ATOMIC_RELAXED, __HIP_MEMORY_SCOPE_AGENT));
+}
 
 template <bool AGENT>
 __device__ __forceinline__ float2 fold_load2(const float* p) {
@@ -25,32 +65,34 @@
   return r;
 }
 
-__device__ __forceinline__ bool fold_last_arrival(int* counter, int expected, int* flag) {
+__device__ __forceinline__ bool fold_last_arrival(int* counter, int expected, int* flag, int mine = 1) {
   asm volatile("s_waitcnt vmcnt(0)" ::: "memory");
   __syncthreads();
   if (threadIdx.x == 0) {
-    const int prev = __hip_atomic_fetch_add(counter, 1, __ATOMIC_RELAXED, __HIP_MEMORY_SCOPE_AGENT);
-    *flag = (prev == expected - 1) ? 1 : 0;
-    if (prev == expected - 1) __hip_atomic_store(counter, 0, __ATOMIC_RELAXED, __HIP_MEMORY_SCOPE_AGENT);
+    const int prev = __hip_atomic_fetch_add(counter, mine, __ATOMIC_RELAXED, __HIP_MEMORY_SCOPE_AGENT);
+    *flag = (prev == expected - mine) ? 1 : 0;
+    if (prev == expected - mine) __hip_atomic_store(counter, 0, __ATOMIC_RELAXED, __HIP_MEMORY_SCOPE_AGENT);
   }
   __syncthreads();
   return *flag != 0;
 }
 
 template <bool AGENT>
-__device__ __forceinline__ void bn_finalize_sliced(const float* partial, int rows, int C, int c0, int nlive, double count, const BnFinalizeArgs& a,
-                                                   double* red, int tid) {
+__device__ __forceinline__ void bn_group_sliced(const float* partial, int r0, int r1, int C, int c0, int nlive, double count, double* red, int tid,
+                                                double (&rec)[3]) {
   constexpr double kTile = 128.0;
   const int cl = tid & 63, sl = tid >> 6;
   const int c = c0 + cl;
   const bool live = tid < 64 * kFoldSlices && cl < nlive;
   double pivot = 0.0;
+  rec[0] = rec[1] = rec[2] = 0.0;
   if (live) {
     double s1 = 0.0, q = 0.0, pp = 0.0;
-    const double n0 = count < kTile ? count : kTile;
-    pivot = (double)fold_load2<AGENT>(partial + (long long)c * 2).x / n0;
+    const double left0 = count - (double)r0 * kTile;
+    const double n0 = left0 < kTile ? left0 : kTile;
+    pivot = (double)fold_load2<AGENT>(partial + ((long long)r0 * C + c) * 2).x / n0;
 #pragma unroll 8
-    for (int r = sl; r < rows; r += kFoldSlices) {
+    for (int r = r0 + sl; r < r1; r += kFoldSlices) {
       const float2 v = fold_load2<AGENT>(partial + ((long long)r * C + c) * 2);
       const double left = count - (double)r * kTile;
       const double nt = left < kTile ? left : kTile;
@@ -70,36 +112,115 @@
     for (int k = 0; k < 3; ++k)
       t[k] = ((red[(k * kFoldSlices + 0) * 64 + cl] + red[(k * kFoldSlices + 1) * 64 + cl]) + red[(k * kFoldSlices + 2) * 64 + cl]) +
              red[(k * kFoldSlices + 3) * 64 + cl];
-    const double macc = t[0] / count;
-    const double m2tot = t[1] + (t[2] - count * (macc - pivot) * (macc - pivot));
-    double var = m2tot / count;
-    if (var < 0.0) var = 0.0;
-    const float mean = (float)(macc + (a.conv_bias ? (double)a.conv_bias[c] : 0.0));
-    const float invstd = (float)(1.0 / sqrt(var + (double)a.eps));
-    const float sc = a.gamma[c] * invstd;
-    a.mean[c] = mean;
-    a.invstd[c] = invstd;
-    a.scale[c] = sc;
-    a.shift[c] = a.beta[c] - mean * sc;
-    if (a.running_mean) {
-      const double unbiased = count > 1.0 ? var * count / (count - 1.0) : var;
-      a.running_mean[c] = (1.f - a.momentum) * a.running_mean[c] + a.momentum * mean;
-      a.running_var[c] = (1.f - a.momentum) * a.running_var[c] + a.momentum * (float)unbiased;
-    }
-  }
+    const double cap = (double)(r1 - r0) * kTile, left = count - (double)r0 * kTile;
+    const double n = left < cap ? left : cap;
+    const double macc = t[0] / n;
+    rec[0] = n;
+    rec[1] = t[0];
+    rec[2] = t[1] + (t[2] - n * (macc - pivot) * (macc - pivot));
+  }
+}
+
+__device__ __forceinline__ void bn_chan_merge(double (&A)[3], const double (&B)[3]) {
+#pragma clang fp contract(off)
+  if (!(B[0] > 0.0)) return;
+  if (!(A[0] > 0.0)) {
+    A[0] = B[0];
+    A[1] = B[1];
+    A[2] = B[2];
+    return;
+  }
+  const double n = A[0] + B[0];
+  const double d = B[1] / B[0] - A[1] / A[0];
+  A[2] = (A[2] + B[2]) + d * d * (A[0] * B[0] / n);
+  A[1] = A[1] + B[1];
+  A[0] = n;
+}
+
+__device__ __forceinline__ void bn_merge_slices(double (&A)[3], bool live, double* red, int tid) {
+  const int cl = tid & 63, sl = tid >> 6;
+  if (live) {
+#pragma unroll
+    for (int k = 0; k < 3; ++k) red[(k * kFoldSlices + sl) * 64 + cl] = A[k];
+  }
+  __syncthreads();
+  if (live && sl == 0) {
+#pragma unroll
+    for (int s = 1; s < kFoldSlices; ++s) {
+      const double B[3] = {red[(0 * kFoldSlices + s) * 64 + cl], red[(1 * kFoldSlices + s) * 64 + cl], red[(2 * kFoldSlices + s) * 64 + cl]};
+      bn_chan_merge(A, B);
+    }
+  }
+}
+
+__device__ __forceinline__ void bn_merge_sliced(const double* recs, int groups, int C, int c0, int nlive, double* red, int tid, double (&out)[3]) {
+  const int cl = tid & 63, sl = tid >> 6;
+  const bool live = tid < 64 * kFoldSlices && cl < nlive;
+  out[0] = out[1] = out[2] = 0.0;
+  if (live) {
+#pragma unroll 4
+    for (int g = sl; g < groups; g += kFoldSlices) {
+      const double* q = recs + ((long long)g * C + c0 + cl) * 3;
+      const double B[3] = {fold_loadd(q), fold_loadd(q + 1), fold_loadd(q + 2)};
+      bn_chan_merge(out, B);
+    }
+  }
+  bn_merge_slices(out, live, red, tid);
+}
+
+__device__ __forceinline__ void bn_finalize_record(const double (&rec)[3], int c, double count, const BnFinalizeArgs& a) {
+  const double macc = rec[1] / count;
+  double var = rec[2] / count;
+  if (var < 0.0) var = 0.0;
+  const float mean = (float)(macc + (a.conv_bias ? (double)a.conv_bias[c] : 0.0));
+  const float invstd = (float)(1.0 / sqrt(var + (double)a.eps));
+  const float sc = a.gamma[c] * invstd;
+  a.mean[c] = mean;
+  a.invstd[c] = invstd;
+  a.scale[c] = sc;
+  a.shift[c] = a.beta[c] - mean * sc;
+  if (a.running_mean) {
+    const double unbiased = count > 1.0 ? var * count / (count - 1.0) : var;
+    a.running_mean[c] = (1.f - a.momentum) * a.running_mean[c] + a.momentum * mean;
+    a.running_var[c] = (1.f - a.momentum) * a.running_var[c] + a.momentum * (float)unbiased;
+  }
+}
+
+template <bool AGENT>
+__device__ __forceinline__ void fold_bn_levels(const float* partial, int rows, int C, int nb, int g, double count, const BnFinalizeArgs& a, int* cnt2,
+                                               double* recs, double* red, int* flag, int tid) {
+  const int groups = (rows + kFoldMaxRows - 1) / kFoldMaxRows;
+  const int c0 = nb * 64, cl = tid & 63;
+  const int nlive = C - c0 < 64 ? C - c0 : 64;
+  const bool mine = tid < 64 && cl < nlive;
+  const int r0 = g * kFoldMaxRows;
+  double rec[3];
+  bn_group_sliced<AGENT>(partial, r0, r0 + kFoldMaxRows < rows ? r0 + kFoldMaxRows : rows, C, c0, nlive, count, red, tid, rec);
+  if (groups > 1) {
+    if (mine) {
+      double* q = recs + ((long long)g * C + c0 + cl) * 3;
+      fold_stored(q, rec[0]);
+      fold_stored(q + 1, rec[1]);
+      fold_stored(q + 2, rec[2]);
+    }
+    if (!fold_last_arrival(cnt2 + nb, groups, flag)) return;
+    bn_merge_sliced(recs, groups, C, c0, nlive, red, tid, rec);
+  }
+  if (mine) bn_finalize_record(rec, c0 + cl, count, a);
   if (tid == 0 && c0 == 0 && a.num_batches_tracked != nullptr) a.num_batches_tracked[0] += 1;
 }
 
 template <bool AGENT>
-__device__ __forceinline__ void colsum2_sliced(const float* partial, int rows, int C, int stride, int offset, int c0, int nlive, float* out0,
-                                               float* out1, double* red, int tid) {
+__device__ __forceinline__ void colsum2_group_sliced(const float* partial, int r0, int r1, int C, int stride, int offset, int c0, int nlive, double* red,
+                                                     int tid, double (&out)[2]) {
   const int cl = tid & 63, sl = tid >> 6;
   const int c = c0 + cl;
   const bool live = tid < 64 * kFoldSlices && cl < nlive;
+  out[0] = out[1] = 0.0;
   if (live) {
     double s0 = 0.0, s1 = 0.0;
 #pragma unroll 8
-    for (int r = sl; r < rows; r += kFoldSlices) {
+    for (int r = r0 + sl; r < r1; r += kFoldSlices) {
       const float2 v = fold_load2<AGENT>(partial + ((long long)r * C + c) * stride + offset);
       s0 += (double)v.x;
       s1 += (double)v.y;
@@ -109,11 +230,67 @@
   }
   __syncthreads();
   if (live && sl == 0) {
-    out0[c] = (float)(((red[(0 * kFoldSlices + 0) * 64 + cl] + red[(0 * kFoldSlices + 1) * 64 + cl]) + red[(0 * kFoldSlices + 2) * 64 + cl]) +
-                      red[(0 * kFoldSlices + 3) * 64 + cl]);
-    out1[c] = (float)(((red[(1 * kFoldSlices + 0) * 64 + cl] + red[(1 * kFoldSlices + 1) * 64 + cl]) + red[(1 * kFoldSlices + 2) * 64 + cl]) +
-                      red[(1 * kFoldSlices + 3) * 64 + cl]);
-  }
-}
-
-}
+    out[0] = ((red[(0 * kFoldSlices + 0) * 64 + cl] + red[(0 * kFoldSlices + 1) * 64 + cl]) + red[(0 * kFoldSlices + 2) * 64 + cl]) +
+             red[(0 * kFoldSlices + 3) * 64 + cl];
+    out[1] = ((red[(1 * kFoldSlices + 0) * 64 + cl] + red[(1 * kFoldSlices + 1) * 64 + cl]) + red[(1 * kFoldSlices + 2) * 64 + cl]) +
+             red[(1 * kFoldSlices + 3) * 64 + cl];
+  }
+}
+
+__device__ __forceinline__ void colsum2_merge_slices(double (&A)[2], bool live, double* red, int tid) {
+  const int cl = tid & 63, sl = tid >> 6;
+  if (live) {
+    red[(0 * kFoldSlices + sl) * 64 + cl] = A[0];
+    red[(1 * kFoldSlices + sl) * 64 + cl] = A[1];
+  }
+  __syncthreads();
+  if (live && sl == 0) {
+    A[0] = ((red[(0 * kFoldSlices + 0) * 64 + cl] + red[(0 * kFoldSlices + 1) * 64 + cl]) + red[(0 * kFoldSlices + 2) * 64 + cl]) +
+           red[(0 * kFoldSlices + 3) * 64 + cl];
+    A[1] = ((red[(1 * kFoldSlices + 0) * 64 + cl] + red[(1 * kFoldSlices + 1) * 64 + cl]) + red[(1 * kFoldSlices + 2) * 64 + cl]) +
+           red[(1 * kFoldSlices + 3) * 64 + cl];
+  }
+}
+
+__device__ __forceinline__ void colsum2_merge_sliced(const double* recs, int groups, int C, int c0, int nlive, double* red, int tid, double (&out)[2]) {
+  const int cl = tid & 63, sl = tid >> 6;
+  const bool live = tid < 64 * kFoldSlices && cl < nlive;
+  out[0] = out[1] = 0.0;
+  if (live) {
+#pragma unroll 4
+    for (int g = sl; g < groups; g += kFoldSlices) {
+      const double* q = recs + ((long long)g * C + c0 + cl) * 2;
+      out[0] += fold_loadd(q);
+      out[1] += fold_loadd(q + 1);
+    }
+  }
+  colsum2_merge_slices(out, live, red, tid);
+}
+
+template <bool AGENT>
+__device__ __forceinline__ void fold_colsum2_levels(const float* partial, int rows, int C, int stride, int offset, int nb, int g, float* out0, float* out1,
+                                                    int* cnt2, double* recs, double* red, int* flag, int tid) {
+  const int groups = (rows + kFoldMaxRows - 1) / kFoldMaxRows;
+  const int c0 = nb * 64, cl = tid & 63;
+  const int nlive = C - c0 < 64 ? C - c0 : 64;
+  const bool mine = tid < 64 && cl < nlive;
+  const int r0 = g * kFoldMaxRows;
+  double s[2];
+  colsum2_group_sliced<AGENT>(partial, r0, r0 + kFoldMaxRows < rows ? r0 + kFoldMaxRows : rows, C, stride, offset, c0, nlive, red, tid, s);
+  if (groups > 1) {
+    if (mine) {
+      double* q = recs + ((long long)g * C + c0 + cl) * 2;
+      fold_stored(q, s[0]);
+      fold_stored(q + 1, s[1]);
+    }
+    if (!fold_last_arrival(cnt2 + nb, groups, flag)) return;
+    colsum2_merge_sliced(recs, groups, C, c0, nlive, red, tid, s);
+  }
+  if (mine) {
+    out0[c0 + cl] = (float)s[0];
+    out1[c0 + cl] = (float)s[1];
+  }
+}
+#endif
+
+}
diff --git a/supervised_dispnet_amd/csrc/dn_internal.h b/supervised_dispnet_amd/csrc/dn_internal.h
--- a/supervised_dispnet_amd/csrc/dn_internal.h
+++ b/supervised_dispnet_amd/csrc/dn_internal.h
@@ -109,6 +109,12 @@
   int ooy, oox;
   int nchunks;
   long long w_off;
+};
+
+struct FoldWs {
+  int* cnt;
+  int* cnt1;
+  double* rec;
 };
 
 struct BnFinalizeArgs {
@@ -169,6 +175,8 @@
   BnFinalizeArgs bnf;
   float *bnb_dgamma, *bnb_dbeta;
   int* fold_cnt;
+  int* fold_cnt1;
+  double* fold_rec;
   int fold_bn, fold_bnb;
   int nmajor;
 };
@@ -262,6 +270,7 @@
 bool lds3k_conv_eligible(const dn_conv_desc* d, const IgemmParams& p);
 int launch_lds3k_conv(const dn_conv_desc* d, const IgemmParams& p, hipStream_t stream);
 bool stem3_conv_eligible(const dn_conv_desc* d, const IgemmParams& p);
+bool stem3_folds_bn_finalize(const IgemmParams& p);
 bool stemk_conv_eligible(const dn_conv_desc* d, const IgemmParams& p);
 int launch_stemk_conv(const dn_conv_desc* d, const IgemmParams& p, hipStream_t stream);
 bool stemk_wgrad_eligible(const dn_conv_desc* d, const IgemmParams& p);
diff --git a/supervised_dispnet_amd/csrc/dn_lds3.hip b/supervised_dispnet_amd/csrc/dn_lds3.hip
--- a/supervised_dispnet_amd/csrc/dn_lds3.hip
+++ b/supervised_dispnet_amd/csrc/dn_lds3.hip
@@ -1,6 +1,7 @@
 #include <stdlib.h>
 
 #include "dn_device.h"
+#include "dn_fold.h"
 
 namespace dn {
 
@@ -448,7 +449,38 @@
       const int h = tid >> 6, c = tid & 63;
       const f32x2 a = *reinterpret_cast<const f32x2*>(&wstat[2 * h][c][0]), b2 = *reinterpret_cast<const f32x2*>(&wstat[2 * h + 1][c][0]);
       const float dm = (b2[0] - a[0]) * (1.f / 64.f);
-      *reinterpret_cast<f32x2*>(p.bn_partial + ((long long)(2 * t + h) * p.Ntot + c) * 2) = f32x2{a[0] + b2[0], a[1] + b2[1] + dm * dm * 32.f};
+      fold_store2(p.bn_partial + ((long long)(2 * t + h) * p.Ntot + c) * 2, a[0] + b2[0], a[1] + b2[1] + dm * dm * 32.f);
+    }
+  }
+
+  const int t0 = band_lo + local;
+  if (p.fold_bn && t0 < band_hi) {
+    __shared__ double fred[3 * kFoldSlices * 64];
+    __shared__ int flast[32];
+    __shared__ int fflag;
+    const int prow = 2 * geo.ntiles;
+    const int g_lo = t0 >> 6, ng = ((t0 + (band_hi - 1 - t0) / nlocal * nlocal) >> 6) - g_lo + 1;
+    asm volatile("s_waitcnt vmcnt(0)" ::: "memory");
+    __syncthreads();
+    if (tid < ng) {
+      const int gg = g_lo + tid;
+      int mine = 0, last = 0;
+      for (int t = t0; t < band_hi; t += nlocal) mine += ((t >> 6) == gg) ? 1 : 0;
+      if (mine > 0) {
+        const int left = geo.ntiles - 64 * gg;
+        const int expected = left < 64 ? left : 64;
+        int* counter = prow > kFoldMaxRows ? fold_cnt1_of(p.fold_cnt) + gg : p.fold_cnt;
+        const int prev = __hip_atomic_fetch_add(counter, mine, __ATOMIC_RELAXED, __HIP_MEMORY_SCOPE_AGENT);
+        last = (prev + mine == expected) ? 1 : 0;
+        if (last) __hip_atomic_store(counter, 0, __ATOMIC_RELAXED, __HIP_MEMORY_SCOPE_AGENT);
+      }
+      flast[tid] = last;
+    }
+    __syncthreads();
+    for (int i = 0; i < ng; ++i) {
+      if (flast[i] == 0) continue;
+      fold_bn_levels<true>(p.bn_partial, prow, p.Ntot, 0, g_lo + i, (double)p.M, p.bnf, p.fold_cnt, fold_rec_of(p.fold_cnt), fred, &fflag, tid);
+      __syncthreads();
     }
   }
 }
@@ -466,7 +498,15 @@
 
 bool stem3_conv_eligible(const dn_conv_desc* d, const IgemmParams& p) { return stem3_eligible(d, p); }
 
-int launch_stem3_conv(const IgemmParams& p, hipStream_t stream) {
+bool stem3_folds_bn_finalize(const IgemmParams& p) {
+  const FoldWs f{p.fold_cnt, p.fold_cnt1, p.fold_rec};
+  const int ntiles = p.M / (STEM_TH * STEM_TW);
+  return p.bnf.scale != nullptr && p.bn_partial != nullptr && fold_levels_fit(f, 2 * ntiles, p.Ntot) && ((ntiles + 7) / 8 + 63) / 64 + 1 <= 32;
+}
+
+int launch_stem3_conv(const IgemmParams& p0, hipStream_t stream) {
+  IgemmParams p = p0;
+  p.fold_bn = stem3_folds_bn_finalize(p) ? 1 : 0;
   Lds3Geo geo;
   geo.tilesX = p.GW / STEM_TW;
   geo.tilesY = p.GH / STEM_TH;
diff --git a/supervised_dispnet_amd/csrc/dn_plan.hip b/supervised_dispnet_amd/csrc/dn_plan.hip
--- a/supervised_dispnet_amd/csrc/dn_plan.hip
+++ b/supervised_dispnet_amd/csrc/dn_plan.hip
@@ -5,6 +5,7 @@
 #include <atomic>
 #include <mutex>
 
+#include "dn_fold.h"
 #include "dn_internal.h"
 
 namespace dn {
@@ -146,10 +147,11 @@
   if (!for_wgrad && d->splitk_ws != nullptr && d->splitk_ws_bytes > 0) {
     p->ks_ws = reinterpret_cast<float*>(d->splitk_ws);
     p->ks_ws_bytes = (size_t)d->splitk_ws_bytes;
-    if (d->splitk_ws_bytes >= 8192 && (d->splitk_ws_bytes & 3) == 0) {
-      p->ks_ws_bytes -= 256;
-      p->fold_cnt = reinterpret_cast<int*>(reinterpret_cast<char*>(d->splitk_ws) + d->splitk_ws_bytes - 256);
-    }
+    FoldWs f;
+    p->ks_ws_bytes -= fold_ws_of(d->splitk_ws, d->splitk_ws_bytes, &f);
+    p->fold_cnt = f.cnt;
+    p->fold_cnt1 = f.cnt1;
+    p->fold_rec = f.rec;
   }
   if (!for_wgrad && d->kind == DN_CONV_FWD && d->bn_partial != nullptr && d->bnf_scale != nullptr) {
     DN_REQUIRE(d->bnf_gamma && d->bnf_beta && d->bnf_mean && d->bnf_invstd && d->bnf_shift, DN_ERR_BAD_ARG,
@@ -372,7 +374,7 @@
 
 extern "C" {
 
-int dn_version(void) { return 23; }
+int dn_version(void) { return 24; }
 
 void dn_reload_knobs(void) {
   std::lock_guard<std::mutex> lock(dn::g_knobs_mu);
diff --git a/supervised_dispnet_amd/csrc/dn_wino_common.h b/supervised_dispnet_amd/csrc/dn_wino_common.h
--- a/supervised_dispnet_amd/csrc/dn_wino_common.h
+++ b/supervised_dispnet_amd/csrc/dn_wino_common.h
@@ -91,15 +91,31 @@
   }
 }
 
-__device__ __forceinline__ void wino_fold_tail(const IgemmParams& p, int nb, int mblocks, float* lds, int tid) {
+template <int RPB>
+__device__ __forceinline__ void wino_fold_tail(const IgemmParams& p, int nb, int mb, int mblocks, float* lds, int tid) {
+  static_assert(kFoldMaxRows % RPB == 0, "a block's rows lie in one group");
   if (!(p.fold_bn | p.fold_bnb)) return;
   __shared__ int fold_flag;
-  if (!fold_last_arrival(p.fold_cnt + nb, mblocks, &fold_flag)) return;
-  const int rows = (p.T + 31) / 32, c0 = nb * WBN;
-  const int nlive = p.Ntot - c0 < WBN ? p.Ntot - c0 : WBN;
+  const int rows = (p.T + 31) / 32;
+  int g = 0, expected = mblocks;
+  int* cnt = p.fold_cnt + nb;
+  if (rows > kFoldMaxRows) {
+    g = mb / (kFoldMaxRows / RPB);
+    const int left = rows - g * kFoldMaxRows;
+    expected = ((left < kFoldMaxRows ? left : kFoldMaxRows) + RPB - 1) / RPB;
+    cnt = fold_cnt1_of(p.fold_cnt) + nb * kFoldMaxGroups + g;
+  }
+  if (!fold_last_arrival(cnt, expected, &fold_flag)) return;
   double* red = reinterpret_cast<double*>(lds);
-  if (p.fold_bn) bn_finalize_sliced<true>(p.bn_partial, rows, p.Ntot, c0, nlive, (double)p.M, p.bnf, red, tid);
-  if (p.fold_bnb) colsum2_sliced<true>(p.bnb_partial, rows, p.Ntot, 2, 0, c0, nlive, p.bnb_dbeta, p.bnb_dgamma, red, tid);
+  if (p.fold_bn)
+    fold_bn_levels<true>(p.bn_partial, rows, p.Ntot, nb, g, (double)p.M, p.bnf, p.fold_cnt, fold_rec_of(p.fold_cnt), red, &fold_flag, tid);
+  else
+    fold_colsum2_levels<true>(p.bnb_partial, rows, p.Ntot, 2, 0, nb, g, p.bnb_dbeta, p.bnb_dgamma, p.fold_cnt, fold_rec_of(p.fold_cnt), red, &fold_flag, tid);
+}
+
+static inline bool wino_fold_fits(const IgemmParams& p, int rows, int slices) {
+  const FoldWs f{p.fold_cnt, p.fold_cnt1, p.fold_rec};
+  return fold_levels_fit(f, rows, p.Ntot) && slices <= (rows <= kFoldMaxRows ? kFoldCounters : kFoldLevelSlices);
 }
 
 bool wino8_wanted(const IgemmParams& p);
diff --git a/supervised_dispnet_amd/csrc/dn_winograd.hip b/supervised_dispnet_amd/csrc/dn_winograd.hip
--- a/supervised_dispnet_amd/csrc/dn_winograd.hip
+++ b/supervised_dispnet_amd/csrc/dn_winograd.hip
@@ -902,17 +902,15 @@
     const int MT2 = (p.T + BT - 1) / BT, NT2 = p.Npad / WBN;
     const int per2 = (MT2 * NT2 + 7) >> 3;
     const int q2 = (int)(bx & 7u) * per2 + (int)(bx >> 3);
-    wino_fold_tail(p, p.nmajor ? q2 / MT2 : q2 % NT2, MT2, smem, (int)threadIdx.x);
+    wino_fold_tail<MTW>(p, p.nmajor ? q2 / MT2 : q2 % NT2, p.nmajor ? q2 % MT2 : q2 / NT2, MT2, smem, (int)threadIdx.x);
   }
 }
 
 bool wino_folds_bn_finalize(const IgemmParams& p) {
-  return p.bnf.scale != nullptr && p.bn_partial != nullptr && p.fold_cnt != nullptr && (p.T + 31) / 32 <= kFoldMaxRows &&
-         wino_npad(p) / WBN <= kFoldCounters;
+  return p.bnf.scale != nullptr && p.bn_partial != nullptr && wino_fold_fits(p, (p.T + 31) / 32, wino_npad(p) / WBN);
 }
 bool wino_folds_bn_sums(const IgemmParams& p) {
-  return p.bnb_dgamma != nullptr && p.bnb_dbeta != nullptr && p.bnb_partial != nullptr && p.fold_cnt != nullptr && (p.T + 31) / 32 <= kFoldMaxRows &&
-         wino_npad(p) / WBN <= kFoldCounters;
+  return p.bnb_dgamma != nullptr && p.bnb_dbeta != nullptr && p.bnb_partial != nullptr && wino_fold_fits(p, (p.T + 31) / 32, wino_npad(p) / WBN);
 }
 
 template <int MTW, bool HA, int PREC = 0>
diff --git a/supervised_dispnet_amd/csrc/dn_winograd8.hip b/supervised_dispnet_amd/csrc/dn_winograd8.hip
--- a/supervised_dispnet_amd/csrc/dn_winograd8.hip
+++ b/supervised_dispnet_amd/csrc/dn_winograd8.hip
@@ -531,7 +531,7 @@
     }
   }
   __syncthreads();
-  wino_fold_tail(p, nb, MT, smem, tid);
+  wino_fold_tail<2>(p, nb, mb, MT, smem, tid);
 }
 
 template <bool HA>
diff --git a/supervised_dispnet_amd/engine.py b/supervised_dispnet_amd/engine.py
--- a/supervised_dispnet_amd/engine.py
+++ b/supervised_dispnet_amd/engine.py
@@ -222,6 +222,16 @@
         return
     d.splitk_ws = cur[3]
     d.splitk_ws_bytes = cur[1]
+
+
+class _Ws:
+    splitk_ws, splitk_ws_bytes = None, 0
+
+
+def _fold_workspace(device):
+    w = _Ws()
+    _splitk_workspace(w, device)
+    return w.splitk_ws, w.splitk_ws_bytes
 
 
 def _pick_bn(ntot):
@@ -971,21 +981,22 @@
     elif sums is None:
         raise RuntimeError("bn_backward: the column sums of this dz are gone (a second consumer added to the gradient after they were taken)")
     dgamma, dbeta = sums.final if sums.final is not None else (sink.dest_or_new(bn.weight), sink.dest_or_new(bn.bias))
+    part = None if sums.final is not None else sums.partial.data_ptr()
     if y.pool_src is not None:
         dpooled, pidx = y.pool_src
         hbm_call("dn::bn_bwd_apply_pool_kernel", y.rows * Cn * 8 + y.rows * Cn * 5 // 4, "dn_bn_bwd_apply_pool", dpooled.data_ptr(),
-                 pidx.data_ptr(), y_t.data_ptr(), y.mean.data_ptr(), y.invstd.data_ptr(), bn.weight.data_ptr(), sums.partial.data_ptr(),
+                 pidx.data_ptr(), y_t.data_ptr(), y.mean.data_ptr(), y.invstd.data_ptr(), bn.weight.data_ptr(), part,
                  sums.rows, sums.stride, sums.offset, y.N, y.H, y.W, Cn, g.data_ptr(), dgamma.data_ptr(),
                  dbeta.data_ptr(), _stream())
         y.pool_src = None
     elif relu_pending and not BN_MATERIALIZE_DZ:
         hbm_call(None, y.rows * Cn * 12, "dn_bn_bwd_apply_relu", g.data_ptr(), y_t.data_ptr(),
                  y.scale.data_ptr(), y.shift.data_ptr(), y.mean.data_ptr(), y.invstd.data_ptr(), bn.weight.data_ptr(),
-                 None if sums.final is not None else sums.partial.data_ptr(), sums.rows, sums.stride, sums.offset, y.rows, Cn,
+                 part, sums.rows, sums.stride, sums.offset, y.rows, Cn,
                  dgamma.data_ptr(), dbeta.data_ptr(), _stream())
     else:
         hbm_call(None, y.rows * Cn * 12, "dn_bn_bwd_apply", g.data_ptr(), y_t.data_ptr(), y.mean.data_ptr(),
-                 y.invstd.data_ptr(), bn.weight.data_ptr(), sums.partial.data_ptr(), sums.rows, sums.stride,
+                 y.invstd.data_ptr(), bn.weight.data_ptr(), part, sums.rows, sums.stride,
                  sums.offset, y.rows, Cn, dgamma.data_ptr(), dbeta.data_ptr(), _stream())
     y.bn_sums = None
     sink.put(bn.weight, dgamma)
@@ -1089,9 +1100,18 @@
                      p.grad.data_ptr(), idx.data_ptr(), y.t.data_ptr(), y.mean.data_ptr(), y.invstd.data_ptr(), y.N, y.H, y.W, y.C,
                      y.grad.data_ptr(), sums.partial.data_ptr(), _stream())
         else:
-            hbm_call("dn::colreduce_kernel<dn::PoolBwdOp, 4>", y.rows * y.C * 4 * 1.25 + y.rows * y.C // 4, "dn_bn_relu_pool_bwd_sums",
-                     p.grad.data_ptr(), idx.data_ptr(), y.t.data_ptr(), y.mean.data_ptr(), y.invstd.data_ptr(), y.N, y.H, y.W, y.C,
-                     sums.partial.data_ptr(), _stream())
+            ws, wsb = _fold_workspace(dev) if FOLD_FINALIZE and y.bn_owner is not None else (None, 0)
+            if ws:
+                obn, osink = y.bn_owner
+                dg, db = osink.dest_or_new(obn.weight), osink.dest_or_new(obn.bias)
+                hbm_call("dn::colreduce_finish_kernel<dn::PoolBwdOp, 4>", y.rows * y.C * 4 * 1.25 + y.rows * y.C // 4,
+                         "dn_bn_relu_pool_bwd_sums_finish", p.grad.data_ptr(), idx.data_ptr(), y.t.data_ptr(), y.mean.data_ptr(),
+                         y.invstd.data_ptr(), y.N, y.H, y.W, y.C, sums.partial.data_ptr(), dg.data_ptr(), db.data_ptr(), ws, wsb, _stream())
+                sums.final = (dg, db)
+            else:
+                hbm_call("dn::colreduce_kernel<dn::PoolBwdOp, 4>", y.rows * y.C * 4 * 1.25 + y.rows * y.C // 4, "dn_bn_relu_pool_bwd_sums",
+                         p.grad.data_ptr(), idx.data_ptr(), y.t.data_ptr(), y.mean.data_ptr(), y.invstd.data_ptr(), y.N, y.H, y.W, y.C,
+                         sums.partial.data_ptr(), _stream())
             y.pool_src = (p.grad, idx)
         p.grad = None
 
```

Result: no change. 1986 (-0.9%).
